# hahnicity/deepards

Measured on AMD Instinct MI355X. Metric: breath-sequences/sec (train step) cnn_linear nb20 seq224, higher is better.
Workload: dtype f32; 1 GPU; cnn_linear+resnet18, synthetic (B=64 per GPU, 20, 1, 224) fp32 train step (BASELINE configs[1]); backbone=resnet18, batch_per_gpu=64, global_batch=64, batch_rule=--batch 64 per rank (weak scaling: the global batch grows with the ranks), n_sub_batches=20, seq_len=224, optimizer=sgd-nesterov+clamp, parallelism=dp1, hipgraph=True

## Files before the change

deepards_amd/_lib.py:

```python
import ctypes
import os
import re
import subprocess

_HERE = os.path.dirname(os.path.abspath(__file__))
CSRC = os.path.join(_HERE, 'csrc')
LIB_PATH = os.environ.get('DA_LIB_PATH') or os.path.join(_HERE, 'libdeepards_hip.so')
HEADER = os.path.join(os.path.dirname(_HERE), 'include', 'deepards_hip.h')
SOURCES = ['conv_gemm.hip', 'conv_wino.hip', 'conv_bf16.hip', 'conv_x3p.hip', 'bn.hip', 'stem_pool.hip', 'head_optim.hip', 'transformer.hip',
           'filters.hip', 'se.hip', 'se_wide.hip', 'vgg.hip', 'gradcam.hip', 'protopnet.hip', 'lstm_seq.hip',
           'siamese.hip']

_P, _I, _F, _Z, _U, _D = ctypes.c_void_p, ctypes.c_int, ctypes.c_float, ctypes.c_size_t, ctypes.c_uint, ctypes.c_double
_IP = ctypes.POINTER(ctypes.c_int)


class BnRunningDesc(ctypes.Structure):
    _fields_ = [('mean', _P), ('invstd', _P), ('running_mean', _P), ('running_var', _P), ('num_batches_tracked', _P),
                ('W', _I), ('C', _I), ('Wn', _I), ('eps', _F), ('momentum', _F)]


class BnFwdDesc(ctypes.Structure):
    _fields_ = [('x', ctypes.c_void_p), ('ldx', ctypes.c_int), ('res', ctypes.c_void_p), ('ldr', ctypes.c_int),
                ('out', ctypes.c_void_p), ('ldo', ctypes.c_int), ('mean', ctypes.c_void_p), ('invstd', ctypes.c_void_p),
                ('gamma', ctypes.c_void_p), ('beta', ctypes.c_void_p), ('relu', ctypes.c_int), ('mask', ctypes.c_void_p)]


class BnBwdDesc(ctypes.Structure):
    _fields_ = [('x', ctypes.c_void_p), ('ldx', ctypes.c_int), ('dx', ctypes.c_void_p), ('lddx', ctypes.c_int),
                ('mean', ctypes.c_void_p), ('invstd', ctypes.c_void_p), ('gamma', ctypes.c_void_p), ('beta', ctypes.c_void_p),
                ('ds', ctypes.c_void_p)]


class BnPgradDesc(ctypes.Structure):
    _fields_ = [('s1', _P), ('s2', _P), ('dgamma', _P), ('dbeta', _P), ('W', _I), ('C', _I)]


class WgradReduceDesc(ctypes.Structure):
    _fields_ = [('slab', _P), ('dw', _P), ('splits', _I), ('ntaps', _I), ('N', _I), ('C', _I)]


class WgradJob(ctypes.Structure):
    _fields_ = [('dy', _P), ('x', _P), ('workspace', _P)] + [(n, _I) for n in
               ('rows', 'Lm', 'Ldy', 'lddy', 'N', 'Lx', 'ldx', 'C', 'dy_stride', 'dy_off', 'src_stride', 'ntaps')] + \
               [('src_off', _I * 3), ('winograd', _I), ('xform', _I), ('dy_half', _I), ('Wn', _I), ('ldstat', _I),
                ('mean', _P), ('invstd', _P), ('gamma', _P), ('beta', _P)]


class ConvJob(ctypes.Structure):
    _fields_ = [('x', _P), ('w', _P), ('y', _P)] + [(n, _I) for n in
               ('rows', 'Lm', 'Lsrc', 'ldx', 'C', 'Ldst', 'ldy', 'N', 'dst_stride', 'dst_off', 'src_stride', 'ntaps')] + \
               [('src_off', _I * 3), ('wtap', _I * 3), ('accumulate', _I), ('x2', _P), ('w2', _P), ('tap_split', _I)]


class RepackDesc(ctypes.Structure):
    _fields_ = [('W', _P), ('Wf', _P), ('Wd', _P), ('Uf', _P), ('Ud', _P), ('Co', _I), ('Ci', _I), ('K', _I),
                ('points', _I)]


SIGNATURES = {
    'da_version': (_I, []),
    'da_set_act_dtype': (_I, [_I]),
    'da_get_act_dtype': (_I, []),
    'da_abi_sizes': (None, [ctypes.POINTER(_I)]),
    'da_sizeof_wgrad_reduce_desc': (_I, []),
    'da_sizeof_bn_running_desc': (_I, []),
    'da_sizeof_bn_pgrad_desc': (_I, []),
    'da_hip_runtime_symbol': (_P, []),
    'da_conv_gemm': (_I, [_P, _P, _P] + [_I] * 12 + [_IP, _IP, _I, _P]),
    'da_conv_wgrad_workspace': (_Z, [_I] * 5),
    'da_conv_wgrad': (_I, [_P, _P, _P, _P] + [_I] * 12 + [_IP, _I, _P]),
    'da_debug_set': (_I, [_I, _I]),
    'da_repack_conv_weight': (_I, [_P, _P, _P, _I, _I, _I, _P]),
    'da_stem_conv_fwd': (_I, [_P, _P, _P, _I, _I, _I, _I, _P]),
    'da_stem_wgrad_workspace': (_Z, [_I, _I]),
    'da_stem_conv_wgrad': (_I, [_P, _I, _P, _P, _P, _I, _I, _I, _I, _P]),
    'da_stem_conv_fwd_g': (_I, [_P, _P, _P] + [_I] * 7 + [_P]),
    'da_stem_wgrad_workspace_g': (_Z, [_I] * 4),
    'da_stem_conv_wgrad_g': (_I, [_P, _I, _P, _P, _P] + [_I] * 7 + [_P]),
    'da_bn_chunks': (None, [_I, _I, _I, _IP, _IP]),
    'da_bn_workspace': (_Z, [_I, _I, _I]),
    'da_bn_stats_partial': (_I, [_P, _I, _I, _I, _I, _P, _P]),
    'da_stem_stats_partial': (_I, [_P, _P, _I, _I, _I, _I, _P, _P]),
    'da_stem_bn_relu_pool_fwd': (_I, [_P, _P, _P, _I, _I, _I, _I, _I, _P, _P, _P, _P, _I, _I, _P]),
    'da_stem_bwd_workspace': (_Z, [_I, _I]),
    'da_stem_bwd': (_I, [_P, _I, _P, _P, _I, _I, _I, _I, _P, _P, _P, _P, _I, _P, _P, _I, _P, _P]),
    'da_bn_stats_merge': (_I, [_P, _I, _I, _I, _F, _P, _P, _P]),
    'da_bn_running_multi': (_I, [ctypes.POINTER(BnRunningDesc), _I, _P]),
    'da_bn_apply': (_I, [_P, _I, _P, _I, _P, _I, _I, _I, _I, _P, _P, _P, _P, _I, _P, _F, _P]),
    'da_bn_fwd_x': (_I, [_P, _I, _P, _I, _P, _I, _I, _I, _I, _P, _P, _P, _P, _I, _F, _P, _I, _I, _P]),
    'da_bn_bwd_x': (_I, [_P, _I, _P, _I, _P, _I, _P, _I, _I, _I, _I, _P, _P, _P, _P, _I, _P, _P, _I, _P]),
    'da_bn_relu_pool_fwd_x': (_I, [_P, _I, _P, _I, _I, _I, _I, _P, _P, _P, _P, _I, _P]),
    'da_bn_fwd': (_I, [_P, _I, _P, _I, _P, _I, _I, _I, _I, _P, _P, _P, _P, _I, _F, _P, _P]),
    'da_bn_debug_two_stage': (_I, [_I]),
    'da_bn_debug_target_blocks': (_I, [_I]),
    'da_bn_bwd': (_I, [_P, _I, _P, _I, _P, _I, _P, _I, _P, _I, _I, _I, _I, _P, _P, _P, _P, _I, _P, _P, _P, _P, _I, _P]),
    'da_bn_mask_words': (_Z, [_I, _I, _I]),
    'da_bn_fwd_mask': (_I, [_P, _I, _P, _I, _P, _I, _I, _I, _I, _P, _P, _P, _P, _F, _P, _P, _P]),
    'da_bn_bwd_mask': (_I, [_P, _I, _P, _I, _P, _I, _P, _I, _I, _I, _I, _P, _P, _P, _P, _P, _P, _P, _P, _I, _P, _P]),
    'da_bn_pool_ok': (_I, [_I, _I, _I, _I]),
    'da_bn_fwd_pool': (_I, [_P, _I, _P, _I, _P, _I, _I, _I, _I, _P, _P, _P, _P, _F, _P, _P]),
    'da_bn_bwd_pool': (_I, [_P, _I, _P, _I, _P, _I, _P, _I, _I, _I, _I, _I, _P, _P, _P, _P, _P, _P, _P]),
    'da_bn_bwd_add': (_I, [_P, _I, _P, _I, _P, _I, _P, _I, _P, _I, _I, _I, _I, _P, _P, _P, _P, _I, _P, _P, _P, _P, _I, _P, _I, _P]),
    'da_bn_param_grad_multi': (_I, [ctypes.POINTER(BnPgradDesc), _I, _I, _P]),
    'da_bn_fwd_pair': (_I, [ctypes.POINTER(BnFwdDesc), _I, _I, _I, _F, _P]),
    'da_bn_bwd_pair': (_I, [_P, _I, ctypes.POINTER(BnBwdDesc), _I, _I, _I, _P, _P]),
    'da_bn_bwd_pair2': (_I, [_P, _I, _P, _I, ctypes.POINTER(BnBwdDesc), _I, _I, _I, _P, _P]),
    'da_bn_two_ok': (_I, [_I, _I, _I]),
    'da_bn_bwd_mask2': (_I, [_P, _I, _P, _I, _P, _I, _P, _I, _P, _I, _I, _I, _I, _P, _P, _P, _P, _P, _P, _P]),
    'da_bn_stats_fused': (_I, [_P, _I, _I, _I, _I, _P, _P, _I, _F, _P]),
    'da_bn_relu_ss': (_I, [_P, _I, _P, _I, _I, _I, _I, _P, _P, _I, _P, _P, _P]),
    'da_bn_bwd_ss': (_I, [_P, _I, _P, _I, _P, _I, _P, _I, _P, _I, _I, _I, _I, _P, _P, _I, _P, _P, _I, _I, _P, _U, _F, _I, _P, _P, _I, _P]),
    'da_conv1x1_bn': (_I, [_P, _I, _P, _P, _I, _I, _I, _I, _I, _I, _I, _P, _P, _I, _P, _P, _P, _I, ctypes.c_long, _I, _F, _P, _P]),
    'da_conv3_winograd_drop': (_I, [_P, _P, _P, _I, _I, _I, _I, _I, _I, _P, _U, _F, _P, _I, _P]),
    'da_stat_records_floats': (_Z, [ctypes.c_long, _I]),
    'da_conv3_winograd_bn': (_I, [_P, _P, _P, _I, _I, _I, _I, _I, _I, _P, _P, _P, _P, _P, _F, _P, _U, _F, _P, _P]),
    'da_conv_wgrad_splits': (_I, [_I] * 5),
    'da_conv_wgrad_padded_n': (_I, [_I, _I]),
    'da_conv_gemm_multi': (_I, [ctypes.POINTER(ConvJob), _I, _P]),
    'da_conv3_winograd': (_I, [_P, _P, _P, _I, _I, _I, _I, _I, _I, _I, _P]),
    'da_conv3_winograd4': (_I, [_P, _P, _P, _I, _I, _I, _I, _I, _I, _I, _P]),
    'da_conv3_bf16': (_I, [_P, _P, _P, _I, _I, _I, _I, _I, _I, _I, _P]),
    'da_conv3_bf16_bn': (_I, [_P, _P, _P, _I, _I, _I, _I, _I, _I, _I, _P, _P, _P, _P, _P, _F, _P, _P]),
    'da_pack_conv3_bf16': (_I, [_P, _P, _P, _I, _I, _P]),
    'da_conv3_x3p': (_I, [_P, _P, _P] + [_I] * 6 + [_P]),
    'da_conv_x3p_s2_fwd': (_I, [_P] * 5 + [_I] * 4 + [_P]),
    'da_conv_x3p_s2_dgrad': (_I, [_P] * 5 + [_I] * 4 + [_P]),
    'da_x3_split': (_I, [_P, _I, _P, _Z, _I, _P]),
    'da_x3_merge': (_I, [_P, _P, _I, _Z, _I, _P]),
    'da_conv_bf16_multi': (_I, [ctypes.POINTER(ConvJob), _I, _P]),
    'da_wino_debug_tail': (_I, [_I]),
    'da_wino_weights': (_I, [_P, _P, _I, _I, _I, _P]),
    'da_wino4_weights': (_I, [_P, _P, _I, _I, _I, _P]),
    'da_conv_wgrad_multi': (_I, [ctypes.POINTER(WgradJob), _I, _P]),
    'da_conv_wgrad_multi_reduce': (_I, [ctypes.POINTER(WgradJob), _I, ctypes.POINTER(ctypes.c_void_p), _I, _IP, _P]),
    'da_conv_wgrad_plan': (_I, [ctypes.POINTER(WgradJob), _I, _I, _IP]),
    'da_wgrad_reduce_multi': (_I, [ctypes.POINTER(WgradReduceDesc), _I, _I, _P]),
    'da_step_tail_multi': (_I, [ctypes.POINTER(WgradReduceDesc), _I, ctypes.POINTER(BnPgradDesc), _I, ctypes.POINTER(BnRunningDesc), _I, _P, _I, _I, _P, _I, _P]),
    'da_stem_bwd_partials': (_I, [_I, _I, _I, ctypes.POINTER(ctypes.c_size_t), ctypes.POINTER(_I)]),
    'da_stem_wgrad_reduce': (_I, [_P, _I, _I, _P, _I, _P]),
    'da_repack_multi': (_I, [ctypes.POINTER(RepackDesc), _I, _P]),
    'da_bn_relu_pool_fwd': (_I, [_P, _I, _P, _I, _I, _I, _I, _I, _P, _P, _P, _P, _I, _P]),
    'da_pool_bwd': (_I, [_P, _I, _P, _I, _P, _I, _I, _I, _I, _I, _P, _P, _P, _P, _I, _P]),
    'da_avgpool_fwd': (_I, [_P, _I, _P, _I, _I, _I, _I, _I, _P]),
    'da_avgpool_bwd': (_I, [_P, _I, _P, _I, _I, _I, _I, _I, _P]),
    'da_avgpool_slide_fwd': (_I, [_P, _I, _P, _I, _I, _I, _I, _P]),
    'da_avgpool_slide_bwd': (_I, [_P, _P, _I, _I, _I, _I, _I, _P]),
    'da_global_avgpool_fwd': (_I, [_P, _I, _P, _I, _I, _I, _P]),
    'da_global_avgpool_bwd': (_I, [_P, _P, _I, _I, _I, _I, _P]),
    'da_linear2_fwd': (_I, [_P, _P, _P, _P, _I, _I, _P]),
    'da_bce_logits': (_I, [_P, _P, _I, _F, _P, _P, _P]),
    'da_confidence_loss': (_I, [_P, _P, _I, _I, _F, _F, _P, _P, _P]),
    'da_vacillating_loss': (_I, [_P, _P, _I, _I, _F, _F, _P, _P, _P]),
    'da_linear2_bwd': (_I, [_P, _P, _P, _P, _P, _P, _I, _I, _I, _P]),
    'da_head_groups': (_I, [_I, _I]),
    'da_head_fwd': (_I, [_P, _I, _P, _P, _P, _P, _P, _P, _P, _I, _I, _I, _I, _I, _P]),
    'da_head_bwd': (_I, [_P, _P, _P, _P, _P, _P, _I, _P, _P, _P, _P, _P, _P, _I, _I, _I, _I, _F, _I, _P]),
    'da_head_flat_fwd': (_I, [_P, _P, _P, _P, _P, _P, _P, _P, _I, _I, _I, _I, _P]),
    'da_head_flat_bwd': (_I, [_P, _P, _P, _P, _P, _P, _P, _P, _P, _P, _P, _P, _I, _I, _I, _F, _I, _P]),
    'da_clamp_sgd_nesterov': (_I, [_P, _P, _P, _Z, _F, _F, _F, _F, _F, _I, _P]),
    'da_clamp_adam': (_I, [_P, _P, _P, _P, _Z, _F, _D, _D, _F, _I, _F, _F, _P]),
    'da_clamp_adam_dev': (_I, [_P, _P, _P, _P, _Z, _F, _D, _D, _F, _P, _F, _F, _P]),
    'da_gather_normalize': (_I, [_P, _P, ctypes.c_double, ctypes.c_double, _P, _I, _I, _P]),
    'da_gather_normalize_ch': (_I, [_P, _P, ctypes.POINTER(ctypes.c_double), ctypes.POINTER(ctypes.c_double), _P, _I, _I, _I, _I, _P]),
    'da_gather_normalize_filter': (_I, [_P, _P, ctypes.POINTER(ctypes.c_double), ctypes.POINTER(ctypes.c_double), _P, _P, _P, _I, _I, _I, _I, _P]),
    'da_gather_normalize_chain': (_I, [_P, _P, ctypes.POINTER(ctypes.c_double), ctypes.POINTER(ctypes.c_double), _I, _P, _P, _I, _P, _P,
                                       _I, _I, _I, _I, _P]),
    'da_window_median_fwd': (_I, [_P, _I, _I, _I, _I, _P, _P, _P]),
    'da_window_median_bwd': (_I, [_P, _P, _I, _I, _I, _P, _I, _P]),
    'da_lstm_fwd': (_I, [_P] * 11 + [_I, _I, _I, _P]),
    'da_lstm_bwd': (_I, [_P] * 9 + [_I, _I, _I, _P]),
    'da_lstm_seq_block_seqs': (_I, [_I]),
    'da_lstm_seq_fwd': (_I, [_P] * 5 + [_I] + [_P] * 3 + [_I, _I, _I, _P]),
    'da_lstm_seq_bwd_workspace': (_Z, [_I, _I]),
    'da_lstm_seq_bwd': (_I, [_P] * 14 + [_I] * 4 + [_P]),
    'da_lstm_seq_proj_fwd': (_I, [_P] * 4 + [_I] * 3 + [_P]),
    'da_lstm_seq_proj_bwd_workspace': (_Z, [_I] * 3),
    'da_lstm_seq_proj_bwd': (_I, [_P] * 7 + [_I] * 4 + [_P]),
    'da_tfm_block_form': (_I, [_I, _I, _I, _IP, _IP, ctypes.POINTER(_Z), ctypes.POINTER(_Z)]),
    'da_tfm_block_fwd': (_I, [_P] * 9 + [_I] * 4 + [_P, _U, _U, _F, _P]),
    'da_tfm_block_bwd': (_I, [_P] * 17 + [_I] * 4 + [_P, _U, _U, _F, _P]),
    'da_tfm_block_pgrad': (_I, [_P] * 13 + [_I] * 5 + [_P, _U, _U, _F, _P]),
    'da_reduce_rows': (_I, [_P, _I, _I, _P, _I, _P]),
    'da_se_gate_fwd': (_I, [_P] + [_I] * 5 + [_P] * 12),
    'da_se_scale_fwd': (_I, [_P] * 4 + [_I] * 4 + [_P] * 6),
    'da_se_bwd_reduce': (_I, [_P] * 5 + [_I] * 4 + [_P] * 5),
    'da_se_gate_bwd_workspace': (_Z, [_I] * 3),
    'da_se_gate_bwd': (_I, [_P] * 11 + [_I, _P, _I, _I, _I, _P]),
    'da_se_bwd_scale': (_I, [_P] * 4 + [_I] * 3 + [_P]),
    'da_se_wide_shape_ok': (_I, [_I, _I]),
    'da_se_wide_stats': (_I, [_P] + [_I] * 4 + [_F] + [_P] * 5),
    'da_se_wide_gate_fwd': (_I, [_P] + [_I] * 5 + [_P] * 12),
    'da_se_wide_scale_fwd': (_I, [_P] * 4 + [_I] * 4 + [_P] * 6),
    'da_se_wide_bwd_reduce': (_I, [_P] * 5 + [_I] * 4 + [_P] * 5),
    'da_se_wide_chunk_rows': (_I, []),
    'da_se_wide_gate_bwd_workspace': (_Z, [_I] * 3),
    'da_se_wide_gate_bwd': (_I, [_P] * 11 + [_I, _P, _I, _I, _I, _P]),
    'da_se_wide_bwd_scale': (_I, [_P] * 4 + [_I] * 3 + [_P]),
    'da_bn_relu_maxpool2_fwd': (_I, [_P, _I, _P] + [_I] * 4 + [_P] * 5),
    'da_bn_relu_maxpool2_bwd_workspace': (_Z, [_I] * 4),
    'da_bn_relu_maxpool2_bwd': (_I, [_P, _P, _I, _P, _P, _P] + [_I] * 4 + [_P] * 5),
    'da_bn_mean_bias': (_I, [_P, _P, _P, _I, _I, _P, _P]),
    'da_adaptive_avgpool_flat_fwd': (_I, [_P, _P] + [_I] * 4 + [_P]),
    'da_adaptive_avgpool_flat_bwd': (_I, [_P, _P] + [_I] * 4 + [_P]),
    'da_gather_rows': (_I, [_P, _P, _P, _I, _I, _P]),
    'da_gradcam_shape_ok': (_I, [_I] * 3),
    'da_gradcam_workspace': (_Z, [_I] * 3),
    'da_gradcam': (_I, [_P] * 4 + [_I] * 4 + [_P] * 12),
    'da_bias_act_fwd': (_I, [_P, _P, _P, _I, _I, _I, _P]),
    'da_bias_act_bwd_workspace': (_Z, [_I, _I]),
    'da_bias_act_bwd': (_I, [_P, _P, _P, _P, _I, _P, _I, _I, _I, _P]),
    'da_proto_shape_ok': (_I, [_I] * 4),
    'da_proto_row_tile': (_I, [_I, _I]),
    'da_proto_fwd': (_I, [_P] * 6 + [_I] * 4 + [_P]),
    'da_proto_bwd_workspace': (_Z, [_I] * 3),
    'da_proto_bwd': (_I, [_P] * 8 + [_I, _P] + [_I] * 4 + [_P]),
    'da_ppnet_loss': (_I, [_P] * 3 + [_I] * 3 + [_F] * 4 + [_P] * 4),
    'da_grad_add_decay': (_I, [_P, _P, _Z, _F, _P]),
    'da_vote_counts': (_I, [_P, _P, _I, _I, _P, _P, _P]),
    'da_concat2': (_I, [_P, _I, _I, _P, _I, _I, _P, _I, _Z, _P]),
    'da_slice_copy': (_I, [_P, _I, _I, _P, _I, _I, _Z, _I, _P]),
    'da_dropout': (_I, [_P, _P, _Z, _P, _U, _F, _P]),
    'da_concat2_dropout': (_I, [_P, _I, _I, _P, _I, _I, _P, _I, _Z, _P, _U, _F, _P]),
    'da_slice_dropout': (_I, [_P, _I, _I, _P, _I, _I, _Z, _P, _U, _F, _P]),
    'da_siamese_draw': (_I, [_P] * 4 + [_I, _I, _U, _U, _I, _P]),
    'da_siamese_head_rows_per_block': (_I, []),
    'da_siamese_head_fwd': (_I, [_P] * 4 + [_I] + [_P] * 7 + [_I] * 3 + [_P]),
    'da_siamese_head_bwd_workspace': (_Z, [_I] * 3),
    'da_siamese_head_bwd': (_I, [_P] * 4 + [_I] + [_P] * 8 + [_I] + [_P] * 5 + [_F] + [_I] * 4 + [_P]),
}


def header_symbols():
    txt = open(HEADER).read()
    txt = re.sub(r'/\*.*?\*/', '', txt, flags=re.S)
    return sorted(set(re.findall(r'\b(da_[a-z0-9_]+)\s*\(', txt)))


def build(force=False, verbose=False):
    srcs = [os.path.join(CSRC, s) for s in SOURCES]
    deps = srcs + [os.path.join(CSRC, h) for h in ('common.h', 'se_tail.h')]
    if not force and os.path.exists(LIB_PATH) and all(os.path.getmtime(LIB_PATH) >= os.path.getmtime(d) for d in deps):
        return LIB_PATH
    hipcc = os.environ.get('HIPCC', '/opt/rocm/bin/hipcc')
    if not os.path.exists(hipcc):
        hipcc = 'hipcc'
    cmd = [hipcc, '-O3', '--offload-arch=gfx950', '-fPIC', '-shared', '-std=c++17', '-o', LIB_PATH] + srcs
    if verbose:
        print(' '.join(cmd))
    subprocess.check_call(cmd)
    return LIB_PATH


_lib = None


def lib():
    global _lib
    if _lib is None:
        if not os.path.exists(LIB_PATH):
            raise RuntimeError('libdeepards_hip.so is not built: run `python -c "import __graft_entry__ as g; '
                               'g.build()"` (hipcc --offload-arch=gfx950).  There is no CPU fallback.')
        import torch
        l = ctypes.CDLL(LIB_PATH)
        for name, (res, args) in SIGNATURES.items():
            fn = getattr(l, name)
            fn.restype = res
            fn.argtypes = args
        _check_same_runtime(l)
        _lib = l
    return _lib


def _check_same_runtime(l):
    import sys
    torch = sys.modules.get('torch')
    if torch is None:
        return
    tlib = os.path.join(os.path.dirname(torch.__file__), 'lib', 'libamdhip64.so')
    if not os.path.exists(tlib):
        return
    theirs = ctypes.cast(ctypes.CDLL(tlib).hipGetLastError, ctypes.c_void_p).value
    ours = l.da_hip_runtime_symbol()
    if ours != theirs:
        raise RuntimeError('libdeepards_hip.so is bound to a different HIP runtime (%#x) than PyTorch (%#x): '
                           'import torch before deepards_amd' % (ours or 0, theirs or 0))
```

deepards_amd/csrc/common.h:

```cpp
#pragma once
#include <hip/hip_runtime.h>
#include <stdint.h>

typedef float f32x4 __attribute__((ext_vector_type(4)));
typedef float f32x16 __attribute__((ext_vector_type(16)));

typedef float f32x2v __attribute__((ext_vector_type(2)));
typedef __bf16 bf16x2v __attribute__((ext_vector_type(2)));

#define DA_OK 0
#define DA_EINVAL (-1)

__device__ __forceinline__ int xcd_chunked(int id, int total) {
  const int q = total >> 3, r = total & 7;
  const int xcd = id & 7, s = id >> 3;
  return (xcd < r ? xcd * (q + 1) : r * (q + 1) + (xcd - r) * q) + s;
}

__device__ __forceinline__ uint32_t mix32(uint32_t a, uint32_t b) {
  uint32_t h = a * 0x9E3779B1u ^ (b + 0x7F4A7C15u);
  h ^= h >> 16; h *= 0x85EBCA6Bu;
  h ^= h >> 13; h *= 0xC2B2AE35u;
  h ^= h >> 16;
  return h;
// ... 277 lines not shown
  const float* mean;
  const float* invstd;
  const float* gamma;
  const float* beta;
} da_wgrad_job;

struct WgradReduceDesc {
  const float* slab;
  float* dw;
  int splits, ntaps, N, C;
};

__device__ __forceinline__ void wgrad_reduce_block(const WgradReduceDesc& d, int blk, int accumulate) {
  const int total = d.ntaps * d.N * d.C;
  const int i = blk * 1024 + threadIdx.x * 4;
  if (i >= total) return;
  const float* p = d.slab + i;
  f32x4 s = {0.f, 0.f, 0.f, 0.f};
  int sp = 0;
  for (; sp + 8 <= d.splits; sp += 8) {
    f32x4 v[8];
#pragma unroll
    for (int j = 0; j < 8; ++j) v[j] = *reinterpret_cast<const f32x4*>(p + (size_t)(sp + j) * total);
#pragma unroll
    for (int e = 0; e < 4; ++e) s[e] += ((v[0][e] + v[1][e]) + (v[2][e] + v[3][e])) + ((v[4][e] + v[5][e]) + (v[6][e] + v[7][e]));
  }
  if (sp + 4 <= d.splits) {
    f32x4 v[4];
#pragma unroll
    for (int j = 0; j < 4; ++j) v[j] = *reinterpret_cast<const f32x4*>(p + (size_t)(sp + j) * total);
#pragma unroll
    for (int e = 0; e < 4; ++e) s[e] += (v[0][e] + v[1][e]) + (v[2][e] + v[3][e]);
    sp += 4;
  }
  for (; sp < d.splits; ++sp) {
    const f32x4 v = *reinterpret_cast<const f32x4*>(p + (size_t)sp * total);
#pragma unroll
    for (int e = 0; e < 4; ++e) s[e] += v[e];
  }
  const int nc = d.N * d.C;
  const int tap = i / nc, rem = i - tap * nc;
  float* o = d.dw + (size_t)rem * d.ntaps + tap;
#pragma unroll
  for (int e = 0; e < 4; ++e) {
    float* q = o + (size_t)e * d.ntaps;
    *q = accumulate ? *q + s[e] : s[e];
  }
}

#define WGRAD_PRE_MAX 14
struct WgradPreTable {
  WgradReduceDesc d[WGRAD_PRE_MAX];
  int first_block[WGRAD_PRE_MAX + 1];
  int n, nblocks, accumulate;
  int own;
};
__device__ __forceinline__ int wgrad_pre_dispatch(const WgradPreTable& p) {
  const int bid = blockIdx.x;
  if (p.nblocks == 0) return bid;
  if (p.own < 0) {
    if (bid >= p.nblocks) return bid - p.nblocks;
  } else if (bid < p.own) {
    return bid;
  }
  const int pb = p.own < 0 ? bid : bid - p.own;
  if (pb < p.first_block[p.n]) {
    int i = 0;
    while (i + 1 < p.n && pb >= p.first_block[i + 1]) ++i;
    wgrad_reduce_block(p.d[i], pb - p.first_block[i], p.accumulate);
  }
  return -1;
}
static inline int wgrad_pre_grid(WgradPreTable& pre, int blocks, bool front = false) {
  if (pre.nblocks == 0) return blocks;
  pre.own = front ? -1 : (blocks + 7) & ~7;
  return (front ? blocks : pre.own) + pre.nblocks;
}

struct WgradChain {
  WgradPreTable pre, next;
  int pre_job[WGRAD_PRE_MAX], next_job[WGRAD_PRE_MAX];
  float* const* dws;
  int* reduced;
};
static inline void wgrad_chain_init(WgradChain* c, float* const* dws, int accumulate, int* reduced) {
  c->pre.n = c->pre.nblocks = c->pre.own = 0;
  c->pre.first_block[0] = 0;
  c->pre.accumulate = accumulate;
  c->next = c->pre;
  c->dws = dws;
  c->reduced = reduced;
}
static inline void wgrad_chain_offer(WgradChain* c, int job, const da_wgrad_job& j, int splits) {
  if (!c || !c->dws || !c->dws[job] || c->next.n >= WGRAD_PRE_MAX) return;
  WgradPreTable& t = c->next;
  t.d[t.n] = {j.workspace, c->dws[job], splits, j.ntaps, j.N, j.C};
  c->next_job[t.n] = job;
  t.first_block[t.n + 1] = t.first_block[t.n] + (j.ntaps * j.N * j.C + 1023) / 1024;
  ++t.n;
  t.nblocks = (t.first_block[t.n] + 7) & ~7;
}
static inline WgradPreTable wgrad_chain_take(WgradChain* c) {
  WgradPreTable t;
  t.n = t.nblocks = t.accumulate = t.own = 0;
  t.first_block[0] = 0;
  if (!c) return t;
  t = c->pre;
  for (int i = 0; i < t.n; ++i) c->reduced[c->pre_job[i]] = 1;
  c->pre = c->next;
  for (int i = 0; i < c->next.n; ++i) c->pre_job[i] = c->next_job[i];
  c->next.n = c->next.nblocks = 0;
  return t;
}

struct WgradPlan {
  int tn, tc;
  int splits;
  int kchunk;
};
int wgrad_plan_jobs(const da_wgrad_job* jobs, int n, int chained, WgradPlan* plan);

bool wino_wgrad_eligible(const da_wgrad_job& j);
void wino_wgrad_plan_jobs(const da_wgrad_job* jobs, int n, int chained, WgradPlan* plan);
int wino_wgrad_launch(const da_wgrad_job* jobs, const WgradPlan* plan, int n, hipStream_t stream, WgradChain* chain);
void wino4_wgrad_plan(int rows, int L, int* splits, int* qchunk);
extern int g_wino4_skip5;
int wino4_wgrad_launch(const da_wgrad_job* jobs, const WgradPlan* plan, int n, hipStream_t stream, WgradChain* chain);

bool bf16_wgrad_eligible(const da_wgrad_job& j);
void bf16_wgrad_plan(int rows, int L, int* splits, int* pchunk);
int bf16_wgrad_launch(const da_wgrad_job* jobs, const WgradPlan* plan, int n, int code, hipStream_t stream);

typedef struct {
  const float* x;
  const float* w;
  float* y;
  int rows, Lm, Lsrc, ldx, C, Ldst, ldy, N, dst_stride, dst_off, src_stride, ntaps;
  int src_off[3];
  int wtap[3];
  int accumulate;
  const float* x2;
  const float* w2;
  int tap_split;
} da_conv_job;

extern "C" int da_sizeof_wgrad_reduce_desc(void);
extern "C" int da_sizeof_bn_running_desc(void);
extern "C" int da_sizeof_bn_pgrad_desc(void);
```

deepards_amd/csrc/conv_gemm.hip:

```cpp
#include "common.h"
#include <algorithm>
#include <utility>
#include <vector>

#ifndef WGRAD_GLOAD_AT
#define WGRAD_GLOAD_AT 8
#endif
#ifndef GLOAD_AT
#define GLOAD_AT 3
#endif

struct ConvGemmArgs {
  const float* x;
  const float* w;
  const float* x2;
  const float* w2;
  int tap_split;
  float* y;
  int M, Lsrc, ldx, C;
  int Ldst, ldy, N;
  int dst_stride, dst_off, src_stride;
  int ntaps, so0, so1, so2, wt0, wt1, wt2;
  int accumulate;
  FastDiv divLm;
};

template <int TM, int TN, int WGM, int WGN>
__device__ __forceinline__ void conv_gemm_body(const ConvGemmArgs& a, const int lin, float* lds) {
  constexpr int BM = TM * WGM * 32, BN = TN * WGN * 32, PITCH = 36;
  static_assert(WGM * WGN == 4, "4 waves");
  float* As = lds;
  float* Bs = lds + BM * PITCH;

  const int tid = threadIdx.x, lane = tid & 63, wave = tid >> 6;
  const int wm = wave / WGN, wn = wave % WGN;
  const int ntn = a.N / BN;
  const int m_blk = (lin / ntn) * BM, n_blk = (lin % ntn) * BN;
  const int lr = tid >> 3, lq = tid & 7;
  const int Lm = (int)a.divLm.d;

  constexpr int AP = BM / 32, BP = BN / 32;
  int a_rowoff[AP], a_j[AP];
  bool a_ok[AP];
#pragma unroll
  for (int p = 0; p < AP; ++p) {
    int m = m_blk + lr + 32 * p;
    a_ok[p] = m < a.M;
    uint32_t row = fdiv((uint32_t)(a_ok[p] ? m : 0), a.divLm);
    int j = (a_ok[p] ? m : 0) - (int)row * Lm;
    a_rowoff[p] = (int)row * a.Lsrc;
    a_j[p] = j * a.src_stride;
  }

  const int kc = a.C >> 5;
  const int nk = a.ntaps * kc;
  f32x4 ra[AP], rb[BP];

  auto gload = [&](int it) {
    int t = it / kc;
    int c0 = (it - t * kc) << 5;
    int so = t == 0 ? a.so0 : (t == 1 ? a.so1 : a.so2);
    int wt = t == 0 ? a.wt0 : (t == 1 ? a.wt1 : a.wt2);
#pragma unroll
    for (int p = 0; p < AP; ++p) {
      int ls = a_j[p] + so;
      bool ok = a_ok[p] && ls >= 0 && ls < a.Lsrc;
      const float* src = (t < a.tap_split ? a.x : a.x2) + (size_t)(a_rowoff[p] + (ok ? ls : 0)) * a.ldx + c0 + lq * 4;
      f32x4 v = {0.f, 0.f, 0.f, 0.f};
      if (ok) v = *reinterpret_cast<const f32x4*>(src);
      ra[p] = v;
    }
    const float* wtp = (t < a.tap_split ? a.w : a.w2) + (size_t)wt * a.N * a.C;
#pragma unroll
    for (int p = 0; p < BP; ++p) {
      int n = n_blk + lr + 32 * p;
      rb[p] = *reinterpret_cast<const f32x4*>(wtp + (size_t)n * a.C + c0 + lq * 4);
    }
  };

  f32x16 acc[TM][TN];
#pragma unroll
  for (int i = 0; i < TM; ++i)
#pragma unroll
// ... 1103 lines not shown
  if (key == 3) g_use_tail = value;
  else if (key == 7) g_wgrad_any = value;
  else if (key == 11) g_wino4_skip5 = value;
  else return DA_EINVAL;
  return DA_OK;
}

int da_conv_gemm(const float* x, const float* w, float* y, int rows, int Lm, int Lsrc, int ldx, int C, int Ldst,
                 int ldy, int N, int dst_stride, int dst_off, int src_stride, int ntaps, const int* src_off,
                 const int* wtap, int accumulate, hipStream_t stream) {
  DA_ENTER();
  if (g_act_bf16) return DA_EINVAL;
  if (!x || !w || !y || rows < 0 || Lm < 1 || ntaps < 1 || ntaps > 3) return DA_EINVAL;
  da_conv_job j = {};
  j.x = x; j.w = w; j.y = y;
  j.rows = rows; j.Lm = Lm; j.Lsrc = Lsrc; j.ldx = ldx; j.C = C; j.Ldst = Ldst; j.ldy = ldy; j.N = N;
  j.dst_stride = dst_stride; j.dst_off = dst_off; j.src_stride = src_stride; j.ntaps = ntaps; j.accumulate = accumulate;
  for (int t = 0; t < ntaps; ++t) {
    j.src_off[t] = src_off[t];
    j.wtap[t] = wtap[t];
  }
  ConvGemmArgs a;
  conv_gemm_fill(a, j);
  return conv_gemm_dispatch(a, stream);
}

int da_conv_gemm_multi(const da_conv_job* jobs, int n, hipStream_t stream) {
  DA_ENTER();
  if (g_act_bf16) return DA_EINVAL;
  if (n < 1 || n > 4 || !jobs) return DA_EINVAL;
  ConvGemmArgs a[4];
  for (int i = 0; i < n; ++i) {
    const da_conv_job& j = jobs[i];
    if (!j.x || !j.w || !j.y || j.rows < 0 || j.Lm < 1 || j.ntaps < 1 || j.ntaps > 3 || j.C % 32 || j.N % 64 || j.ldx % 4)
      return DA_EINVAL;
    if ((uint64_t)j.rows * j.Lm * (uint64_t)j.Lm >= 0xffffffffull) return DA_EINVAL;
    if (j.x2 && (!j.w2 || j.tap_split < 1 || j.tap_split >= j.ntaps)) return DA_EINVAL;
    conv_gemm_fill(a[i], j);
  }
  return launch_conv_multi(a, n, stream);
}

int da_conv1x1_bn(const float* x, int ldx, const float* w, float* y, int ldy, int rows, int R, int Lin, int C, int N, int pool,
                  float* mean, float* invstd, int ldstat, const float* gamma, const float* beta, const float* pend, int pend_c0,
                  long pend_units, int pend_Wu, float eps, float* out_part, hipStream_t stream) {
  DA_ENTER();
  if (g_act_bf16) return DA_EINVAL;
  if (!x || !w || !y || !mean || !invstd || !gamma || !beta || rows < 0 || R < 1 || rows % R || Lin < 1) return DA_EINVAL;
  if (C % 32 || C < 32 || C > 2048 || N % 64 || N < 64 || ldx % 4 || ldx < C || ldy < N || ldstat % 4 || ldstat < C) return DA_EINVAL;
  if (pool && (Lin & 1)) return DA_EINVAL;
  if (rows == 0) return DA_OK;
  const int Lout = pool ? Lin / 2 : Lin;
  const long M = (long)rows * Lout;
  if ((long)R * Lout < 64) return DA_EINVAL;
  if ((uint64_t)rows * Lin * (uint64_t)(ldx > ldy ? ldx : ldy) >= 0x7fffffffull) return DA_EINVAL;
  if ((uint64_t)M * (uint64_t)(R * Lout) >= 0xffffffffull) return DA_EINVAL;
  Conv1x1BnArgs a;
  a.x = x; a.w = w; a.y = y;
  a.M = (int)M; a.ldx = ldx; a.C = C; a.ldy = ldy; a.N = N; a.W = rows / R; a.Wn = R * Lout; a.ldstat = ldstat;
  a.mean = mean; a.invstd = invstd; a.gamma = gamma; a.beta = beta;
  a.divWn = make_fastdiv((uint32_t)a.Wn);
  a.pend = pend; a.pend_c0 = C; a.pend_nc = 0; a.pend_Wu = 1; a.pend_tiles = 0; a.eps = eps; a.out_part = out_part;
  if (pend) {
    if (pend_c0 < 0 || pend_c0 >= C || pend_units < 1 || pend_Wu < 64 || pend_units % pend_Wu || pend_units / pend_Wu != rows / R)
      return DA_EINVAL;
    a.pend_c0 = pend_c0; a.pend_nc = C - pend_c0; a.pend_Wu = pend_Wu; a.pend_tiles = (int)((pend_units + 63) / 64);
  }
  const unsigned blocks = (unsigned)(((M + 63) / 64) * (N / 64));
  const size_t shm = (size_t)(128 * 36 + 4 * C) * sizeof(float);
  if (out_part) {
    if (pool) hipLaunchKernelGGL((conv1x1_bn_kernel<1, 1>), dim3(blocks), dim3(256), shm, stream, a);
    else hipLaunchKernelGGL((conv1x1_bn_kernel<0, 1>), dim3(blocks), dim3(256), shm, stream, a);
  } else if (pool) hipLaunchKernelGGL((conv1x1_bn_kernel<1, 0>), dim3(blocks), dim3(256), shm, stream, a);
  else hipLaunchKernelGGL((conv1x1_bn_kernel<0, 0>), dim3(blocks), dim3(256), shm, stream, a);
  DA_CHECK_LAUNCH();
  return DA_OK;
}

size_t da_conv_wgrad_workspace(int rows, int Lm, int N, int C, int ntaps) {
  WgradPlan p = wgrad_plan(rows * Lm, N, C, ntaps);
  return (size_t)p.splits * ntaps * N * C * sizeof(float);
}

static int conv_wgrad_multi_impl(const da_wgrad_job* jobs, int n, int chained, float* const* dws, int accumulate, int* reduced,
                                 hipStream_t stream) {
  DA_ENTER();
  std::vector<WgradPlan> plan_(n > 0 ? n : 0);
  WgradPlan* const plan = plan_.data();
  int rc = wgrad_plan_jobs(jobs, n, chained, plan);
  if (rc) return rc;
  for (int i = 0; i < n; ++i)
    if (!jobs[i].workspace) return DA_EINVAL;
  WgradChain chain_, *chain = nullptr;
  if (dws) {
    if (!reduced) return DA_EINVAL;
    for (int i = 0; i < n; ++i) reduced[i] = 0;
    wgrad_chain_init(&chain_, dws, accumulate, reduced);
    chain = &chain_;
  }
  if ((rc = wino4_wgrad_launch(jobs, plan, n, stream, chain))) return rc;
  if ((rc = wino_wgrad_launch(jobs, plan, n, stream, chain))) return rc;
  if ((rc = bf16_wgrad_launch(jobs, plan, n, 49, stream))) return rc;
  if ((rc = bf16_wgrad_launch(jobs, plan, n, 16, stream))) return rc;
  if ((rc = launch_wgrad_group<2, 2, 2, 2>(jobs, plan, n, 128, 128, stream, chain))) return rc;
  if ((rc = launch_wgrad_group<2, 1, 2, 2>(jobs, plan, n, 128, 64, stream, chain))) return rc;
  if ((rc = launch_wgrad_group<1, 2, 2, 2>(jobs, plan, n, 64, 128, stream, chain))) return rc;
  if ((rc = launch_wgrad_group<1, 1, 2, 2>(jobs, plan, n, 64, 64, stream, chain))) return rc;
  if ((rc = launch_wgrad_group<1, 1, 4, 1>(jobs, plan, n, 128, 32, stream, chain))) return rc;
  if ((rc = launch_wgrad_group<1, 1, 1, 4>(jobs, plan, n, 32, 128, stream, chain))) return rc;
  if ((rc = launch_wgrad_group<2, 2, 2, 2, 1>(jobs, plan, n, 128, 128, stream, chain))) return rc;
  if (g_wgrad_any) return launch_wgrad_any<1>(jobs, plan, n, stream, chain);
  if ((rc = launch_wgrad_group<2, 1, 2, 2, 1>(jobs, plan, n, 128, 64, stream, chain))) return rc;
  if ((rc = launch_wgrad_group<1, 2, 2, 2, 1>(jobs, plan, n, 64, 128, stream, chain))) return rc;
  if ((rc = launch_wgrad_group<1, 1, 2, 2, 1>(jobs, plan, n, 64, 64, stream, chain))) return rc;
  if ((rc = launch_wgrad_group<1, 1, 4, 1, 1>(jobs, plan, n, 128, 32, stream, chain))) return rc;
  return launch_wgrad_group<1, 1, 1, 4, 1>(jobs, plan, n, 32, 128, stream, chain);
}

int da_conv_wgrad_multi(const da_wgrad_job* jobs, int n, hipStream_t stream) {
  return conv_wgrad_multi_impl(jobs, n, 0, nullptr, 0, nullptr, stream);
}

int da_conv_wgrad_multi_reduce(const da_wgrad_job* jobs, int n, float* const* dws, int accumulate, int* reduced,
                               hipStream_t stream) {
  if (n && (!dws || !reduced)) return DA_EINVAL;
  return conv_wgrad_multi_impl(jobs, n, 1, dws, accumulate, reduced, stream);
}

int da_conv_wgrad_plan(const da_wgrad_job* jobs, int n, int chained, int* slabs) {
  if (n > 0 && !slabs) return DA_EINVAL;
  std::vector<WgradPlan> plan(n > 0 ? n : 0);
  const int rc = wgrad_plan_jobs(jobs, n, chained, plan.data());
  for (int i = 0; !rc && i < n; ++i) slabs[i] = plan[i].splits;
  return rc;
}

int da_conv_wgrad_padded_n(int N, int C) {
  if (N < 32 || N % 32 || C < 32 || C % 32) return -1;
  for (int n = N; n < N + 128; n += 32)
    if (wgrad_plan(128, n, C, 1).tn) return n;
  return -1;
}

int da_conv_wgrad_splits(int rows, int Lm, int N, int C, int ntaps) {
  return wgrad_plan(rows * Lm, N, C, ntaps).splits;
}

typedef struct {
  const float* slab;
  float* dw;
  int splits, ntaps, N, C;
} da_wgrad_reduce_desc;

int da_sizeof_wgrad_reduce_desc(void) { return (int)sizeof(da_wgrad_reduce_desc); }

typedef struct {
  const float* s1;
  const float* s2;
  float* dgamma;
  float* dbeta;
  int W, C;
} da_bn_pgrad_desc;
typedef struct {
  const float* mean;
  const float* invstd;
  float* running_mean;
  float* running_var;
  long long* num_batches_tracked;
  int W, C, Wn;
  float eps, momentum;
} da_bn_running_desc;
int da_bn_param_grad_multi(const da_bn_pgrad_desc* descs, int n, int accumulate, hipStream_t stream);
int da_bn_running_multi(const da_bn_running_desc* descs, int n, hipStream_t stream);
int da_wgrad_reduce_multi(const da_wgrad_reduce_desc* descs, int n, int accumulate, hipStream_t stream);

int da_stem_wgrad_reduce(const float* partial, int nblk, int n, float* dw, int accumulate, hipStream_t stream);
int da_step_tail_multi(const da_wgrad_reduce_desc* descs, int n, const da_bn_pgrad_desc* pg, int npg,
                       const da_bn_running_desc* run, int nrun, const float* stem_partial, int stem_nblk, int stem_n,
                       float* stem_dw, int accumulate, hipStream_t stream) {
  DA_ENTER();
  if (n < 0 || npg < 0 || nrun < 0 || (n && !descs) || (npg && !pg) || (nrun && !run)) return DA_EINVAL;
  if (stem_partial && (!stem_dw || stem_nblk < 1 || stem_n < 1)) return DA_EINVAL;
  if (n == 0 || n > 32 || npg > REDUCE_MAX_BN || nrun > REDUCE_MAX_BN || (npg + nrun == 0 && !stem_partial)) {
    int rc = nrun ? da_bn_running_multi(run, nrun, stream) : DA_OK;
    if (!rc && stem_partial) rc = da_stem_wgrad_reduce(stem_partial, stem_nblk, stem_n, stem_dw, accumulate, stream);
    if (!rc && npg) rc = da_bn_param_grad_multi(pg, npg, accumulate, stream);
    if (!rc && n) rc = da_wgrad_reduce_multi(descs, n, accumulate, stream);
    return rc;
  }
  WgradReduceTable t;
  ReducePgradTable g;
  int maxc = 0, nred = 0;
  for (int i = 0; i < n; ++i) {
    const da_wgrad_reduce_desc& s = descs[i];
    if (!s.slab || !s.dw || s.splits < 1) return DA_EINVAL;
    if (s.ntaps < 1 || s.N < 1 || s.C < 1 || (s.N * s.C) % 4) return DA_EINVAL;
    t.d[i] = {s.slab, s.dw, s.splits, s.ntaps, s.N, s.C};
    t.first_block[i] = nred;
    nred += (s.ntaps * s.N * s.C + 1023) / 1024;
  }
  t.first_block[n] = nred;
  t.n = n;
  for (int i = 0; i < npg; ++i) {
    const da_bn_pgrad_desc& s = pg[i];
    if (!s.s1 || !s.s2 || !s.dgamma || !s.dbeta) return DA_EINVAL;
    g.p[i] = {s.s1, s.s2, s.dgamma, s.dbeta, s.W, s.C};
    if (s.C > maxc) maxc = s.C;
  }
  for (int i = 0; i < nrun; ++i) {
// ... 80 lines not shown
```

deepards_amd/csrc/conv_wino.hip:

```cpp
#include "common.h"
#include <type_traits>

struct WinoArgs {
  const float* x;
  const float* u;
  float* y;
  int MP, L, PL, ldx, C, ldy, N, accumulate;
  FastDiv divPL;
  const long long* drop_seed;
  uint32_t drop_salt;
  float drop_p;
  float* stat_part;
  int stat_Wu;
  const float* in_pend;
  float* in_mean;
  float* in_invstd;
  const float* in_gamma;
  const float* in_beta;
  int in_tiles, in_Wu;
  float in_eps;
};

__device__ __forceinline__ int wino_row(int i) {
  return (i >= 4 && i < 12) ? 2 * (i - 4) : (i < 4 ? 2 * i + 1 : 2 * (i - 12) + 9);
}

#define WINO_PITCH 36
#define WINO_AROWS 66
#define WINO_LDS_FLOATS (2 * WINO_AROWS * WINO_PITCH + 4 * 32 * WINO_PITCH)

#define WINO_STAT_FLOATS (4 * 2 * 2 * 32 + 8)
#define WINO_XF_FLOATS (2 * 2 * 128)
template <bool MINI, bool STATS = false, bool XFW = false, bool DROP = false>
__device__ __forceinline__ void conv3_wino_body(const WinoArgs& a, const int tile, const int sub, float* lds) {
  constexpr int PITCH = WINO_PITCH, PAIRS = MINI ? 32 : 64, AR = PAIRS + 2;
  float* Es = lds;
  float* Os = lds + AR * PITCH;
  float* Us = lds + 2 * AR * PITCH;

  const int tid = threadIdx.x, lane = tid & 63, wave = tid >> 6;
  const int ntn = a.N >> 5;
  const int P0 = (tile / ntn) * 64 + (MINI ? 32 * sub : 0), n_blk = (tile % ntn) * 32;
  const int lr = tid >> 3, lq = tid & 7;
  const int PL = a.PL;

  constexpr int NA = MINI ? 3 : 5;
  int aoff[NA], aslot[NA];
  bool aok[NA];
#pragma unroll
  for (int p = 0; p < NA; ++p) {
    const bool extra = p == NA - 1;
    const int e = extra ? PAIRS + (tid >> 4) : (MINI ? lr : lr + 32 * (p & 1));
    const int odd = extra ? ((tid >> 3) & 1) : (MINI ? p : (p >> 1));
    const int P = P0 - 1 + e;
    aslot[p] = 0;
    bool ok = P >= 0 && P < a.MP && (!extra || tid < 32);
    const uint32_t r = fdiv((uint32_t)(ok ? P : 0), a.divPL);
    const int i = (ok ? P : 0) - (int)r * PL;
    const int pos = 2 * i + odd;
    ok = ok && pos < a.L;
    aoff[p] = ((int)r * a.L + (ok ? pos : 0)) * a.ldx + lq * 4;
    aok[p] = ok;
    if (XFW) {
      const int sl = (P >= 0 ? P : 0) / a.stat_Wu - P0 / a.stat_Wu;
      aslot[p] = (sl < 0 ? 0 : (sl > 1 ? 1 : sl)) * 2 * a.C + lq * 4;
    }
  }
  const float* ub = a.u + (size_t)(n_blk + lr) * a.C + lq * 4;
  const size_t ustride = (size_t)a.N * a.C;
  float* xtab = lds + WINO_LDS_FLOATS + WINO_STAT_FLOATS;

  f32x4 ra[NA], rb[4];
  auto gload_a = [&](int ks) {
    const int c0 = ks << 5;
#pragma unroll
    for (int p = 0; p < NA; ++p) {
      f32x4 v = {0.f, 0.f, 0.f, 0.f};
      if (aok[p]) v = *reinterpret_cast<const f32x4*>(a.x + aoff[p] + c0);
      ra[p] = v;
    }
  };
  auto gload_b = [&](int ks) {
    const int c0 = ks << 5;
// ... 846 lines not shown
      ry[2 * rb] = okk ? *reinterpret_cast<const f32x4*>(a.dy + pos * a.lddy + n_blk + lq * 4) : z;
      ry[2 * rb + 1] = (okk && ok1) ? *reinterpret_cast<const f32x4*>(a.dy + (pos + 1) * a.lddy + n_blk + lq * 4) : z;
      rx[2 * rb] = ok ? *reinterpret_cast<const f32x4*>(a.x + pos * a.ldx + c_blk + lq * 4) : z;
      rx[2 * rb + 1] = ok1 ? *reinterpret_cast<const f32x4*>(a.x + (pos + 1) * a.ldx + c_blk + lq * 4) : z;
    }
    if (tid < 32) {
      const int P = tid < 16 ? k0 - 1 : k0 + KP;
      const bool ok = P >= 0 && P < a.MP;
      const uint32_t r = fdiv((uint32_t)(ok ? P : 0), a.divPL);
      const int i = (ok ? P : 0) - (int)r * PL;
      const int pp = 2 * i + (tid < 16 ? 1 : 0);
      f32x4 v = {0.f, 0.f, 0.f, 0.f};
      if (ok && pp < a.L) v = *reinterpret_cast<const f32x4*>(a.x + ((size_t)r * a.L + pp) * a.ldx + c_blk + lq * 4);
      rx[2 * NRB] = v;
    }
  };

  f32x16 acc[4];
#pragma unroll
  for (int j = 0; j < 4; ++j)
#pragma unroll
    for (int r = 0; r < 16; ++r) acc[j][r] = 0.f;

  const int frow = lane & 31, fh = lane >> 5;
  if (k_beg < k_end) gload(k_beg);
  for (int k0 = k_beg; k0 < k_end; k0 += KP) {
    __syncthreads();
#pragma unroll
    for (int rb = 0; rb < NRB; ++rb) {
      const int row = lrow + 16 * rb;
      *reinterpret_cast<f32x4*>(&YE[row * 64 + lq * 4]) = ry[2 * rb];
      *reinterpret_cast<f32x4*>(&YO[row * 64 + lq * 4]) = ry[2 * rb + 1];
      *reinterpret_cast<f32x4*>(&XE[(row + 1) * 64 + lq * 4]) = rx[2 * rb];
      *reinterpret_cast<f32x4*>(&XO[(row + 1) * 64 + lq * 4]) = rx[2 * rb + 1];
    }
    if (tid < 16) *reinterpret_cast<f32x4*>(&XO[lq * 4]) = rx[2 * NRB];
    else if (tid < 32) *reinterpret_cast<f32x4*>(&XE[(KP + 1) * 64 + lq * 4]) = rx[2 * NRB];
    const int Pm = k0 + (lane & 31);
    const int im = Pm - (int)fdiv((uint32_t)(Pm < a.MP ? Pm : 0), a.divPL) * PL;
    const uint32_t fmask = (uint32_t)__ballot(Pm < a.MP && im == 0);
    const uint32_t lmask = (uint32_t)__ballot(Pm < a.MP && im == PL - 1);
    __syncthreads();
#pragma unroll WW_UNROLL
    for (int kk = 0; kk < KP / 2; ++kk) {
      if (kk == KP / 4) {
        __builtin_amdgcn_sched_barrier(0);
        if (k0 + KP < k_end) gload(k0 + KP);
        __builtin_amdgcn_sched_barrier(0);
      }
      const int p = 2 * kk + fh;
      const float y0 = YE[p * 64 + wm * 32 + frow], y1 = YO[p * 64 + wm * 32 + frow];
      float d0 = XO[p * 64 + wn * 32 + frow];
      const float d1 = XE[(p + 1) * 64 + wn * 32 + frow], d2 = XO[(p + 1) * 64 + wn * 32 + frow];
      float d3 = XE[(p + 2) * 64 + wn * 32 + frow];
      if ((fmask >> p) & 1) d0 = 0.f;
      if ((lmask >> p) & 1) d3 = 0.f;
      acc[0] = __builtin_amdgcn_mfma_f32_32x32x2f32(y0, d0 - d2, acc[0], 0, 0, 0);
      acc[1] = __builtin_amdgcn_mfma_f32_32x32x2f32(y0 + y1, d1 + d2, acc[1], 0, 0, 0);
      acc[2] = __builtin_amdgcn_mfma_f32_32x32x2f32(y0 - y1, d2 - d1, acc[2], 0, 0, 0);
      acc[3] = __builtin_amdgcn_mfma_f32_32x32x2f32(y1, d1 - d3, acc[3], 0, 0, 0);
    }
  }

  float* out = a.slab + (size_t)split * 3 * a.N * a.C;
  const size_t plane = (size_t)a.N * a.C;
#pragma unroll
  for (int r = 0; r < 16; ++r) {
    const int n = n_blk + wm * 32 + (r & 3) + 8 * (r >> 2) + 4 * fh;
    const int c = c_blk + wn * 32 + frow;
    const float h = 0.5f * (acc[1][r] + acc[2][r]);
    float* o = out + (size_t)n * a.C + c;
    o[0] = acc[0][r] + h;
    o[plane] = 0.5f * (acc[1][r] - acc[2][r]);
    o[2 * plane] = h - acc[3][r];
  }
}

struct WinoWgradTable {
  WinoWgradArgs d[24];
  int first_block[25];
  int n;
  int skip5;
};
static_assert(sizeof(WinoWgradTable) + sizeof(WgradPreTable) <= 4096, "kernel arguments: 4 KB");

__global__ __launch_bounds__(256, WW_MIN_WAVES) void wino_wgrad_multi_kernel(WinoWgradTable t, WgradPreTable pre) {
  __shared__ float lds[WW_LDS_FLOATS];
  const int b = wgrad_pre_dispatch(pre);
  if (b < 0 || b >= t.first_block[t.n]) return;
  int i = 0;
  while (i + 1 < t.n && b >= t.first_block[i + 1]) ++i;
  wino_wgrad_body(t.d[i], b - t.first_block[i], t.first_block[i + 1] - t.first_block[i], lds);
}

bool wino_wgrad_eligible(const da_wgrad_job& j) {
  return j.ntaps == 3 && j.dy_stride == 1 && j.dy_off == 0 && j.src_stride == 1 && j.src_off[0] == -1 &&
         j.src_off[1] == 0 && j.src_off[2] == 1 && j.Lm == j.Ldy && j.Lm == j.Lx && j.N % 64 == 0 && j.C % 64 == 0 &&
         j.N >= 64 && j.C >= 64;
}

#ifndef WW_PCHUNK
#define WW_PCHUNK 640
#endif

static void wino_wgrad_plan(int rows, int L, int* splits, int* pchunk, int f) {
  const int MP = rows * ((L + 1) / 2);
  const int base = WW_PCHUNK / (f > 1 ? f : 1) >= 32 ? WW_PCHUNK / (f > 1 ? f : 1) : 32;
  int sp = (MP + base - 1) / base;
  if (sp < 1) sp = 1;
  int pc = ((MP + sp - 1) / sp + 31) / 32 * 32;
  if (pc < 32) pc = 32;
  *splits = (MP + pc - 1) / pc > 0 ? (MP + pc - 1) / pc : 1;
  *pchunk = pc;
}

void wino_wgrad_plan_jobs(const da_wgrad_job* jobs, int n, int chained, WgradPlan* plan) {
  constexpr int SLOTS = 1024;
  long total = 0;
  int njobs = 0;
  for (int i = 0; i < n; ++i) {
    if (jobs[i].winograd != 1) continue;
    plan[i].tn = plan[i].tc = 64;
    wino_wgrad_plan(jobs[i].rows, jobs[i].Lm, &plan[i].splits, &plan[i].kchunk, 1);
    total += (long)(jobs[i].N / 64) * (jobs[i].C / 64) * plan[i].splits;
    ++njobs;
  }
  if (!chained || njobs > 24 || total <= SLOTS || total % SLOTS == 0) return;
  const long full = total / SLOTS * SLOTS;
  long cum = 0;
  for (int i = 0; i < n; ++i) {
    if (jobs[i].winograd != 1) continue;
    cum += (long)(jobs[i].N / 64) * (jobs[i].C / 64) * plan[i].splits;
    if (cum > full) wino_wgrad_plan(jobs[i].rows, jobs[i].Lm, &plan[i].splits, &plan[i].kchunk, 2);
  }
}

int wino_wgrad_launch(const da_wgrad_job* jobs, const WgradPlan* plan, int n, hipStream_t s, WgradChain* chain) {
  WinoWgradTable t;
  int cnt = 0, blocks = 0;
  auto flush = [&]() -> int {
    if (!cnt) return DA_OK;
    t.n = cnt;
    t.skip5 = 0;
    t.first_block[cnt] = blocks;
    WgradPreTable pre = wgrad_chain_take(chain);
    hipLaunchKernelGGL(wino_wgrad_multi_kernel, dim3(wgrad_pre_grid(pre, blocks)), dim3(256), 0, s, t, pre);
    DA_CHECK_LAUNCH();
    cnt = 0;
    blocks = 0;
    return DA_OK;
  };
  for (int i = 0; i < n; ++i) {
    const da_wgrad_job& j = jobs[i];
    if (j.winograd != 1) continue;
    WinoWgradArgs& a = t.d[cnt];
    a.dy = j.dy; a.x = j.x; a.slab = j.workspace;
    a.L = j.Lm; a.PL = (j.Lm + 1) / 2; a.MP = j.rows * a.PL;
    a.lddy = j.lddy; a.N = j.N; a.ldx = j.ldx; a.C = j.C; a.pchunk = plan[i].kchunk;
    a.divPL = make_fastdiv((uint32_t)a.PL);
    t.first_block[cnt] = blocks;
    blocks += (j.N / 64) * (j.C / 64) * plan[i].splits;
    wgrad_chain_offer(chain, i, j, plan[i].splits);
    if (++cnt == 24) {
      int rc = flush();
      if (rc) return rc;
    }
  }
// ... 63 lines not shown
    }
  };

  f32x16 acc[6];
#pragma unroll
  for (int j = 0; j < 6; ++j)
#pragma unroll
    for (int r = 0; r < 16; ++r) acc[j][r] = 0.f;

  const int frow = lane & 31, fh = lane >> 5;
  if (k_beg < k_end) gload(k_beg);
  for (int k0 = k_beg; k0 < k_end; k0 += KQ) {
    __syncthreads();
#pragma unroll
    for (int rb = 0; rb < NRB; ++rb) {
      const int row = lrow + 16 * rb;
#pragma unroll
      for (int ph = 0; ph < 4; ++ph) *reinterpret_cast<f32x4*>(&Y[(ph * KQ + row) * 64 + lq * 4]) = ry[4 * rb + ph];
      *reinterpret_cast<f32x4*>(&X0[row * 64 + lq * 4]) = rx[4 * rb];
      *reinterpret_cast<f32x4*>(&X1[row * 64 + lq * 4]) = rx[4 * rb + 1];
      *reinterpret_cast<f32x4*>(&X2[row * 64 + lq * 4]) = rx[4 * rb + 2];
      *reinterpret_cast<f32x4*>(&X3[(row + 1) * 64 + lq * 4]) = rx[4 * rb + 3];
    }
    if (tid < 16) *reinterpret_cast<f32x4*>(&X3[lq * 4]) = rx[4 * NRB];
    else if (tid < 32) *reinterpret_cast<f32x4*>(&X0[KQ * 64 + lq * 4]) = rx[4 * NRB];
    const int Qm = k0 + (lane & (KQ - 1));
    const int im = Qm - (int)fdiv((uint32_t)(Qm < a.MP ? Qm : 0), a.divPL) * QL;
    const uint32_t fmask = (uint32_t)__ballot(Qm < a.MP && im == 0);
    const uint32_t lmask = (uint32_t)__ballot(Qm < a.MP && im == QL - 1);
    __syncthreads();
    constexpr int UNR = SKIP5 ? WW4_SKIP5_UNROLL : WW4_UNROLL, UNR2 = UNR / 2;
    static_assert(UNR % 2 == 0 && KQ % 8 == 0, "the K loop is unrolled in whole pairs of kk");
#pragma unroll UNR2
    for (int k2 = 0; k2 < KQ / 4; ++k2)
#pragma unroll
    for (int u = 0; u < 2; ++u) {
      const int kk = 2 * k2 + u;
      if (u == 0 && k2 == KQ / 8) {
        __builtin_amdgcn_sched_barrier(0);
        if (k0 + KQ < k_end) gload(k0 + KQ);
        __builtin_amdgcn_sched_barrier(0);
      }
      const int p = 2 * kk + fh;
      const int yo = p * 64 + wm * 32 + frow, xo = p * 64 + wn * 32 + frow;
      const float y0 = Y[yo], y1 = Y[KQ * 64 + yo], y2 = Y[2 * KQ * 64 + yo], y3 = Y[3 * KQ * 64 + yo];
      float d0 = X3[xo];
      const float d1 = X0[xo], d2 = X1[xo], d3 = X2[xo], d4 = X3[xo + 64];
      float d5 = X0[xo + 64];
      if ((fmask >> p) & 1) d0 = 0.f;
      if ((lmask >> p) & 1) d5 = 0.f;
      const float ya = y0 + y2, yb = y1 + y3, yc = fmaf(4.f, y2, y0), yd = 2.f * fmaf(4.f, y3, y1);
      const float e1 = fmaf(-4.f, d2, d4), e2 = fmaf(-4.f, d1, d3), f1 = d4 - d2, f2 = d3 - d1;
      acc[0] = __builtin_amdgcn_mfma_f32_32x32x2f32(y0, fmaf(4.f, d0, fmaf(-5.f, d2, d4)), acc[0], 0, 0, 0);
      acc[1] = __builtin_amdgcn_mfma_f32_32x32x2f32(ya + yb, e1 + e2, acc[1], 0, 0, 0);
      acc[2] = __builtin_amdgcn_mfma_f32_32x32x2f32(ya - yb, e1 - e2, acc[2], 0, 0, 0);
      acc[3] = __builtin_amdgcn_mfma_f32_32x32x2f32(yc + yd, fmaf(2.f, f2, f1), acc[3], 0, 0, 0);
      acc[4] = __builtin_amdgcn_mfma_f32_32x32x2f32(yc - yd, fmaf(-2.f, f2, f1), acc[4], 0, 0, 0);
      if (!SKIP5) {
        acc[5] = __builtin_amdgcn_mfma_f32_32x32x2f32(y3, fmaf(4.f, d1, fmaf(-5.f, d3, d5)), acc[5], 0, 0, 0);
      } else if (u == 0) {
        const int p5 = 2 * kk + 2 * fh;
        const int y5o = p5 * 64 + wm * 32 + frow, x5o = p5 * 64 + wn * 32 + frow;
        const float g3 = Y[3 * KQ * 64 + y5o];
        const float g1 = X0[x5o], g2 = X2[x5o], g5 = X0[x5o + 64];
        acc[5] = __builtin_amdgcn_mfma_f32_32x32x2f32(g3, fmaf(4.f, g1, fmaf(-5.f, g2, g5)), acc[5], 0, 0, 0);
      }
    }
  }

  float* out = a.slab + (size_t)split * 3 * a.N * a.C;
  const size_t plane = (size_t)a.N * a.C;
#pragma unroll
  for (int r = 0; r < 16; ++r) {
    const int n = n_blk + wm * 32 + (r & 3) + 8 * (r >> 2) + 4 * fh;
    const int c = c_blk + wn * 32 + frow;
    const float s12 = acc[1][r] + acc[2][r], s34 = acc[3][r] + acc[4][r];
    float* o = out + (size_t)n * a.C + c;
    o[0] = fmaf(0.25f, acc[0][r], fmaf(1.0f / 24.0f, s34, -(1.0f / 6.0f) * s12));
    o[plane] = fmaf(1.0f / 6.0f, acc[2][r] - acc[1][r], (1.0f / 12.0f) * (acc[3][r] - acc[4][r]));
    o[2 * plane] = fmaf(1.0f / 6.0f, s34 - s12, acc[5][r]);
  }
}

__global__ __launch_bounds__(256, WW4_MIN_WAVES) void wino4_wgrad_multi_kernel(WinoWgradTable t, WgradPreTable pre) {
  __shared__ float lds[WW4_LDS_FLOATS];
  const int b = wgrad_pre_dispatch(pre);
  if (b < 0 || b >= t.first_block[t.n]) return;
  int i = 0;
  while (i + 1 < t.n && b >= t.first_block[i + 1]) ++i;
  const bool skip5 = t.skip5 && t.d[i].PL == 2 && (t.d[i].L & 3) != 0;
  if (skip5) wino4_wgrad_body<true>(t.d[i], b - t.first_block[i], t.first_block[i + 1] - t.first_block[i], lds);
  else wino4_wgrad_body<false>(t.d[i], b - t.first_block[i], t.first_block[i + 1] - t.first_block[i], lds);
}

#ifndef WW4_QCHUNK
#define WW4_QCHUNK 320
#endif

void wino4_wgrad_plan(int rows, int L, int* splits, int* qchunk) {
  const int MQ = rows * ((L + 3) / 4);
  int sp = (MQ + WW4_QCHUNK - 1) / WW4_QCHUNK;
  if (sp < 1) sp = 1;
  int qc = ((MQ + sp - 1) / sp + WW4_KQ - 1) / WW4_KQ * WW4_KQ;
  if (qc < WW4_KQ) qc = WW4_KQ;
  *splits = (MQ + qc - 1) / qc > 0 ? (MQ + qc - 1) / qc : 1;
  *qchunk = qc;
}

int wino4_wgrad_launch(const da_wgrad_job* jobs, const WgradPlan* plan, int n, hipStream_t s, WgradChain* chain) {
  WinoWgradTable t;
  int cnt = 0, blocks = 0;
  auto flush = [&]() -> int {
    if (!cnt) return DA_OK;
    t.n = cnt;
    t.first_block[cnt] = blocks;
    WgradPreTable pre = wgrad_chain_take(chain);
    t.skip5 = g_wino4_skip5 != 0;
    hipLaunchKernelGGL(wino4_wgrad_multi_kernel, dim3(wgrad_pre_grid(pre, blocks)), dim3(256), 0, s, t, pre);
    DA_CHECK_LAUNCH();
    cnt = 0;
    blocks = 0;
    return DA_OK;
  };
  for (int i = 0; i < n; ++i) {
    const da_wgrad_job& j = jobs[i];
    if (j.winograd != 6) continue;
    WinoWgradArgs& a = t.d[cnt];
    a.dy = j.dy; a.x = j.x; a.slab = j.workspace;
    a.L = j.Lm; a.PL = (j.Lm + 3) / 4; a.MP = j.rows * a.PL;
    a.lddy = j.lddy; a.N = j.N; a.ldx = j.ldx; a.C = j.C; a.pchunk = plan[i].kchunk;
    static_assert(WW4_KQ % 8 == 0, "skip5: K steps start at even quads");
    if (a.pchunk % WW4_KQ) return DA_EINVAL;
    a.divPL = make_fastdiv((uint32_t)a.PL);
    t.first_block[cnt] = blocks;
    blocks += (j.N / 64) * (j.C / 64) * plan[i].splits;
    wgrad_chain_offer(chain, i, j, plan[i].splits);
    if (++cnt == 24) {
      int rc = flush();
      if (rc) return rc;
    }
  }
  return flush();
}

__global__ __launch_bounds__(256) void wino_weight_kernel(const float* __restrict__ w, float* __restrict__ u, int co,
                                                          int ci, int transpose) {
  const int N = transpose ? ci : co, C = transpose ? co : ci;
  const size_t total = (size_t)N * C;
  const size_t idx = (size_t)blockIdx.x * blockDim.x + threadIdx.x;
  if (idx >= total) return;
  const int n = (int)(idx / C), c = (int)(idx - (size_t)n * C);
  const float* src = transpose ? w + ((size_t)c * ci + n) * 3 : w + ((size_t)n * ci + c) * 3;
  const float g0 = transpose ? src[2] : src[0], g1 = src[1], g2 = transpose ? src[0] : src[2];
  u[idx] = g0;
  u[total + idx] = (g0 + g1 + g2) * 0.5f;
  u[2 * total + idx] = (g0 - g1 + g2) * 0.5f;
  u[3 * total + idx] = g2;
}

__global__ __launch_bounds__(256) void wino4_weight_kernel(const float* __restrict__ w, float* __restrict__ u, int co,
                                                           int ci, int transpose) {
  const int N = transpose ? ci : co, C = transpose ? co : ci;
  const size_t total = (size_t)N * C;
  const size_t idx = (size_t)blockIdx.x * blockDim.x + threadIdx.x;
  if (idx >= total) return;
  const int n = (int)(idx / C), c = (int)(idx - (size_t)n * C);
  const float* src = transpose ? w + ((size_t)c * ci + n) * 3 : w + ((size_t)n * ci + c) * 3;
  const float g0 = transpose ? src[2] : src[0], g1 = src[1], g2 = transpose ? src[0] : src[2];
  wino4_taps(g0, g1, g2, u + idx, total);
}

extern "C" {

int da_wino4_weights(const float* w, float* u, int co, int ci, int transpose, hipStream_t stream) {
  DA_ENTER();
  if (!w || !u || co < 1 || ci < 1) return DA_EINVAL;
  const size_t total = (size_t)co * ci;
  hipLaunchKernelGGL(wino4_weight_kernel, dim3((unsigned)((total + 255) / 256)), dim3(256), 0, stream, w, u, co, ci,
                     transpose);
  DA_CHECK_LAUNCH();
  return DA_OK;
}

struct WinoBnIn {
  const float* pend; float* mean; float* invstd; const float* gamma; const float* beta; float eps;
};

static int conv3_winograd_impl(const float* x, const float* u, float* y, int rows, int L, int ldx, int C, int ldy, int N,
                               int accumulate, const long long* drop_seed, unsigned drop_salt, float drop_p, float* stat_part,
                               int stat_R, hipStream_t stream, const WinoBnIn* bn = nullptr, int outs = 2) {
  DA_ENTER();
  if (g_act_bf16) return DA_EINVAL;
  if (outs == 4 && (stat_part || bn || drop_p > 0.f)) return DA_EINVAL;
  if (!x || !u || !y || rows < 0 || L < 1 || C % 32 || N % 32 || C < 32 || N < 32 || ldx % 4 || ldx < C || ldy < N)
    return DA_EINVAL;
  if (rows == 0) return DA_OK;
  if ((uint64_t)rows * L * (uint64_t)(ldx > ldy ? ldx : ldy) >= 0x7fffffffull) return DA_EINVAL;
  WinoArgs a;
  a.x = x; a.u = u; a.y = y;
  a.L = L; a.PL = (L + outs - 1) / outs; a.MP = rows * a.PL;
  a.ldx = ldx; a.C = C; a.ldy = ldy; a.N = N; a.accumulate = accumulate;
// ... 89 lines not shown
```

deepards_amd/csrc/stem_pool.hip:

```cpp
#include "common.h"

template <typename AT, int CIN, int K, int S>
__global__ __launch_bounds__(256) void stem_conv_fwd_kernel(const float* __restrict__ x, const float* __restrict__ w,
                                                            AT* __restrict__ y, int Lin, int Lout, int C0, int ldy) {
  extern __shared__ float xs[];
  constexpr int PAD = K / 2;
  const int row = blockIdx.x, LP = Lin + K - 1;
  for (int i = threadIdx.x; i < CIN * LP; i += blockDim.x) {
    const int ci = i / LP, s = i - ci * LP - PAD;
    xs[i] = (s >= 0 && s < Lin) ? x[((size_t)row * CIN + ci) * Lin + s] : 0.f;
  }
  __syncthreads();
  const int co = threadIdx.x % C0, slot = threadIdx.x / C0, nslots = blockDim.x / C0;
  if (slot >= nslots) return;
  float wk[CIN * K];
#pragma unroll
  for (int k = 0; k < CIN * K; ++k) wk[k] = w[co * CIN * K + k];
  for (int l = slot; l < Lout; l += nslots) {
    float acc = 0.f;
#pragma unroll
    for (int ci = 0; ci < CIN; ++ci)
#pragma unroll
      for (int k = 0; k < K; ++k) acc = fmaf(wk[ci * K + k], xs[ci * LP + S * l + k], acc);
    Act<AT>::st1(y + ((size_t)row * Lout + l) * ldy + co, acc);
  }
}

template <typename AT, int CIN, int K, int S>
__global__ __launch_bounds__(256) void stem_wgrad_kernel(const AT* __restrict__ dy, int lddy,
                                                         const float* __restrict__ x, float* __restrict__ partial,
                                                         int rows, int Lin, int Lout, int C0) {
  extern __shared__ float sm[];
  constexpr int PAD = K / 2, KK = CIN * K;
  const int LP = Lin + K - 1;
  float* xs = sm;
  float* red = sm + CIN * LP;
  const int co = threadIdx.x % C0, slot = threadIdx.x / C0, nslots = blockDim.x / C0;
  float acc[KK];
#pragma unroll
  for (int k = 0; k < KK; ++k) acc[k] = 0.f;
  for (int row = blockIdx.x; row < rows; row += gridDim.x) {
    __syncthreads();
    for (int i = threadIdx.x; i < CIN * LP; i += blockDim.x) {
      const int ci = i / LP, s = i - ci * LP - PAD;
      xs[i] = (s >= 0 && s < Lin) ? x[((size_t)row * CIN + ci) * Lin + s] : 0.f;
    }
    __syncthreads();
    if (slot < nslots) {
      for (int l = slot; l < Lout; l += nslots) {
        float g = Act<AT>::ld1(dy + ((size_t)row * Lout + l) * lddy + co);
#pragma unroll
        for (int ci = 0; ci < CIN; ++ci)
#pragma unroll
          for (int k = 0; k < K; ++k) acc[ci * K + k] = fmaf(g, xs[ci * LP + S * l + k], acc[ci * K + k]);
      }
    }
  }
  __syncthreads();
  if (slot < nslots) {
#pragma unroll
    for (int k = 0; k < KK; ++k) red[(slot * C0 + co) * KK + k] = acc[k];
  }
  __syncthreads();
  for (int i = threadIdx.x; i < C0 * KK; i += blockDim.x) {
    float s = 0.f;
    for (int sl = 0; sl < nslots; ++sl) s += red[sl * C0 * KK + i];
    partial[(size_t)blockIdx.x * C0 * KK + i] = s;
  }
}

__global__ __launch_bounds__(256) void stem_wgrad_reduce_kernel(const float* __restrict__ partial, int nblk, int n,
                                                                float* __restrict__ dw, int accumulate) {
  __shared__ float red[32][8];
  stem_wgrad_reduce_block(partial, nblk, n, dw, accumulate, blockIdx.x, red);
}

template <typename AT, int OX3 = 0>
__global__ __launch_bounds__(256) void bn_relu_pool_fwd_kernel(const AT* __restrict__ y, int ldy,
                                                               AT* __restrict__ out, int ldo, int rows, int R,
                                                               int Lin, int Lout, int C, const float* __restrict__ mean,
                                                               const float* __restrict__ invstd,
                                                               const float* __restrict__ gamma,
                                                               const float* __restrict__ beta, int pool_mode) {
  const int nq = C >> 2;
  size_t idx = (size_t)blockIdx.x * blockDim.x + threadIdx.x;
  size_t total = (size_t)rows * Lout * nq;
  if (idx >= total) return;
  int q = (int)(idx % nq);
  size_t po = idx / nq;
  int j = (int)(po % Lout);
  int row = (int)(po / Lout);
  int w = row / R;
  int c0 = q * 4;
  f32x4 mu = *reinterpret_cast<const f32x4*>(mean + (size_t)w * C + c0);
  f32x4 is = *reinterpret_cast<const f32x4*>(invstd + (size_t)w * C + c0);
  f32x4 ga = *reinterpret_cast<const f32x4*>(gamma + c0);
  f32x4 be = *reinterpret_cast<const f32x4*>(beta + c0);
  f32x4 o;
  if (pool_mode != 1) o = f32x4{-INFINITY, -INFINITY, -INFINITY, -INFINITY};
  else o = f32x4{0.f, 0.f, 0.f, 0.f};
  const int sh = pool_mode == 2 ? 1 : 0;
#pragma unroll
  for (int t = 0; t < 3; ++t) {
    int l = 2 * j - 1 + sh + t;
    if (l < 0 || l >= Lin) continue;
    f32x4 v = Act<AT>::ld4(y + ((size_t)row * Lin + l) * ldy + c0);
#pragma unroll
    for (int e = 0; e < 4; ++e) {
      float z = fmaxf((v[e] - mu[e]) * is[e] * ga[e] + be[e], 0.f);
      o[e] = pool_mode != 1 ? fmaxf(o[e], z) : o[e] + z;
    }
  }
  if (pool_mode == 1) {
#pragma unroll
    for (int e = 0; e < 4; ++e) o[e] *= (1.0f / 3.0f);
  }
  if constexpr (OX3) X3::st4(reinterpret_cast<__bf16*>(out) + po * (size_t)(3 * C), c0, o);
  else Act<AT>::st4(out + po * ldo + c0, o);
}

#define STEM_XPAD 8

__device__ __forceinline__ f32x4 stem_y4(const StemW4& sw, const float (&xw)[16], int o) {
  f32x4 y;
#pragma unroll
  for (int e = 0; e < 4; ++e) {
    float acc = 0.f;
#pragma unroll
    for (int k = 0; k < 7; ++k) acc = fmaf(sw.w[e][k], xw[o + k], acc);
    y[e] = acc;
  }
  return y;
}
__device__ __forceinline__ void stem_xw_fill(float (&xw)[16], const float* xs, int j) {
#pragma unroll
  for (int i = 0; i < 16; i += 4) {
    const f32x4 v = *reinterpret_cast<const f32x4*>(xs + 4 * j + i);
    xw[i] = v[0]; xw[i + 1] = v[1]; xw[i + 2] = v[2]; xw[i + 3] = v[3];
  }
}
__device__ __forceinline__ void stem_xw_next(float (&xw)[16], const float* xs, int j) {
#pragma unroll
  for (int i = 0; i < 12; ++i) xw[i] = xw[i + 4];
  const f32x4 v = *reinterpret_cast<const f32x4*>(xs + 4 * j + 12);
  xw[12] = v[0]; xw[13] = v[1]; xw[14] = v[2]; xw[15] = v[3];
}
__host__ __device__ __forceinline__ int stem_xs_floats(int Lin) { return (STEM_XPAD + Lin + 16 + 3) & ~3; }

struct StemBn4 {
  f32x4 mu, is, ga, be;
  __device__ __forceinline__ f32x4 z(const f32x4& y) const {
    f32x4 r;
#pragma unroll
    for (int e = 0; e < 4; ++e) r[e] = fmaxf((y[e] - mu[e]) * is[e] * ga[e] + be[e], 0.f);
    return r;
  }
};

template <typename AT, int OX3, int SH>
__global__ __launch_bounds__(256) void stem_bn_relu_pool_fwd_kernel(const float* __restrict__ xrows, const float* __restrict__ wt,
                                                                    AT* __restrict__ out, int ldo, int rows, int R, int Lin,
                                                                    int Lc, int Lp, int C, const float* __restrict__ mean,
                                                                    const float* __restrict__ invstd,
                                                                    const float* __restrict__ gamma,
                                                                    const float* __restrict__ beta, int pool_mode) {
  extern __shared__ __attribute__((aligned(16))) float sm[];
  const int nq = C >> 2, nruns = blockDim.x / nq, RJ = (Lp + nruns - 1) / nruns;
  const int XS = stem_xs_floats(Lin);
  float* xs = sm;
  const int q = threadIdx.x % nq, run = threadIdx.x / nq, c0 = q * 4;
  StemW4 sw;
  sw.load(wt, c0);
  StemBn4 bn;
  bn.ga = *reinterpret_cast<const f32x4*>(gamma + c0);
  bn.be = *reinterpret_cast<const f32x4*>(beta + c0);
  constexpr int sh = SH;
  const int j0 = sh + run * RJ, j1 = min(Lp + sh, j0 + RJ);
  for (int row = blockIdx.x; row < rows; row += gridDim.x) {
    const int w = row / R;
    __syncthreads();
    for (int i = threadIdx.x; i < XS; i += blockDim.x) {
      const int sx = i - STEM_XPAD - 2 * sh;
      xs[i] = (sx >= 0 && sx < Lin) ? xrows[(size_t)row * Lin + sx] : 0.f;
    }
    __syncthreads();
    if (j0 >= j1) continue;
    bn.mu = *reinterpret_cast<const f32x4*>(mean + (size_t)w * C + c0);
    bn.is = *reinterpret_cast<const f32x4*>(invstd + (size_t)w * C + c0);
    float xw[16];
    stem_xw_fill(xw, xs, j0);
    f32x4 zm = {0.f, 0.f, 0.f, 0.f};
    if (j0 > 0) zm = bn.z(stem_y4(sw, xw, 3));
    for (int j = j0; j < j1; ++j) {
      if (j > j0) stem_xw_next(xw, xs, j);
      const bool vm = j > 0, vp = 2 * j + 1 < Lc + sh;
      const f32x4 z0 = bn.z(stem_y4(sw, xw, 5)), zp = bn.z(stem_y4(sw, xw, 7));
      f32x4 o;
#pragma unroll
      for (int e = 0; e < 4; ++e) {
        if (pool_mode != 1) {
          float m = vm ? fmaxf(-INFINITY, zm[e]) : -INFINITY;
          m = fmaxf(m, z0[e]);
          o[e] = vp ? fmaxf(m, zp[e]) : m;
        } else {
          float a = vm ? 0.f + zm[e] : 0.f;
          a += z0[e];
          if (vp) a += zp[e];
          o[e] = a * (1.0f / 3.0f);
        }
      }
      const size_t po = (size_t)row * Lp + (j - sh);
      if constexpr (OX3) X3::st4(reinterpret_cast<__bf16*>(out) + po * (size_t)(3 * C), c0, o);
      else Act<AT>::st4(out + po * ldo + c0, o);
      zm = zp;
    }
  }
}

template <typename AT>
__global__ __launch_bounds__(256) void pool_bwd_kernel(const AT* __restrict__ dout, int ldd,
                                                       const AT* __restrict__ y, int ldy, AT* __restrict__ dz,
                                                       int lddz, int rows, int R, int Lin, int Lout, int C,
                                                       const float* __restrict__ mean, const float* __restrict__ invstd,
                                                       const float* __restrict__ gamma, const float* __restrict__ beta,
                                                       int pool_mode) {
  const int nq = C >> 2;
  size_t idx = (size_t)blockIdx.x * blockDim.x + threadIdx.x;
  size_t total = (size_t)rows * Lin * nq;
  if (idx >= total) return;
  int q = (int)(idx % nq);
  size_t pi = idx / nq;
  int l = (int)(pi % Lin);
  int row = (int)(pi / Lin);
  int w = row / R;
  int c0 = q * 4;
  f32x4 acc = {0.f, 0.f, 0.f, 0.f};
  const int sh = pool_mode == 2 ? 1 : 0;
  int j_lo = (l + sh) / 2 - sh;
  int j_hi = (l + sh + 1) / 2 - sh;
  if (pool_mode == 1) {
    for (int j = j_lo; j <= j_hi; ++j) {
      if (j >= Lout) continue;
      f32x4 g = Act<AT>::ld4(dout + ((size_t)row * Lout + j) * ldd + c0);
#pragma unroll
      for (int e = 0; e < 4; ++e) acc[e] += g[e] * (1.0f / 3.0f);
    }
  } else {
    f32x4 mu = *reinterpret_cast<const f32x4*>(mean + (size_t)w * C + c0);
    f32x4 is = *reinterpret_cast<const f32x4*>(invstd + (size_t)w * C + c0);
    f32x4 ga = *reinterpret_cast<const f32x4*>(gamma + c0);
    f32x4 be = *reinterpret_cast<const f32x4*>(beta + c0);
    for (int j = j_lo; j <= j_hi; ++j) {
      if (j < 0 || j >= Lout) continue;
      float best[4] = {-INFINITY, -INFINITY, -INFINITY, -INFINITY};
      int barg[4] = {-1, -1, -1, -1};
#pragma unroll
      for (int t = 0; t < 3; ++t) {
        int ll = 2 * j - 1 + sh + t;
        if (ll < 0 || ll >= Lin) continue;
        f32x4 v = Act<AT>::ld4(y + ((size_t)row * Lin + ll) * ldy + c0);
#pragma unroll
        for (int e = 0; e < 4; ++e) {
          float z = fmaxf((v[e] - mu[e]) * is[e] * ga[e] + be[e], 0.f);
          if (z > best[e]) {
            best[e] = z;
            barg[e] = ll;
          }
        }
      }
      f32x4 g = Act<AT>::ld4(dout + ((size_t)row * Lout + j) * ldd + c0);
#pragma unroll
      for (int e = 0; e < 4; ++e)
        if (barg[e] == l) acc[e] += g[e];
    }
  }
  Act<AT>::st4(dz + pi * lddz + c0, acc);
}

template <typename AT, bool APPLY, int SH>
__global__ __launch_bounds__(256) void stem_bwd_kernel(const AT* __restrict__ dout, int ldd, const float* __restrict__ xrows,
                                                       const float* __restrict__ wt, int rows, int R, int Lin, int Lc, int Lp,
                                                       int C, const float* __restrict__ mean, const float* __restrict__ invstd,
                                                       const float* __restrict__ gamma, const float* __restrict__ beta,
                                                       int pool_mode, int RPB, float* __restrict__ rowpart,
                                                       float* __restrict__ ds, float* __restrict__ partial) {
  extern __shared__ __attribute__((aligned(16))) float sm[];
  const int nq = C >> 2, slots = blockDim.x / nq, NRUN = slots < 8 ? slots : 8, RS = slots / NRUN, RJ = (Lp + NRUN - 1) / NRUN;
  const int XS = stem_xs_floats(Lin);
  float* tot = sm + RS * XS;
  float* red = tot + 2 * C;
  const int q = threadIdx.x % nq, slot = threadIdx.x / nq, rs = slot / NRUN, run = slot - rs * NRUN, c0 = q * 4;
  float* xs = sm + rs * XS;
  StemW4 sw;
  sw.load(wt, c0);
  StemBn4 bn;
  bn.ga = *reinterpret_cast<const f32x4*>(gamma + c0);
  bn.be = *reinterpret_cast<const f32x4*>(beta + c0);
  float wacc[4][7];
#pragma unroll
  for (int e = 0; e < 4; ++e)
#pragma unroll
    for (int k = 0; k < 7; ++k) wacc[e][k] = 0.f;
  const float inv_n = 1.0f / (float)(R * Lc);
  constexpr int sh = SH;
  const int jend = Lp + sh;
  const int j0 = sh + run * RJ, j1 = min(jend, j0 + RJ);
  const int row_beg = blockIdx.x * RPB, w = row_beg / R;
  if (APPLY && (int)threadIdx.x < 2 * C) {
    const int which = threadIdx.x / C, c = threadIdx.x - which * C;
    float t = 0.f;
    for (int r = 0; r < R; ++r) t += rowpart[((size_t)(w * R + r) * 2 + which) * C + c];
    tot[which * C + c] = t;
    if (ds && row_beg == w * R) ds[((size_t)which * (rows / R) + w) * C + c] = t;
  }
  bn.mu = *reinterpret_cast<const f32x4*>(mean + (size_t)w * C + c0);
  bn.is = *reinterpret_cast<const f32x4*>(invstd + (size_t)w * C + c0);
  f32x4 t1n = {0.f, 0.f, 0.f, 0.f}, t2n = t1n;
  for (int rb = row_beg; rb < row_beg + RPB; rb += RS) {
    const int row = rb + rs;
    __syncthreads();
    for (int i = threadIdx.x; i < RS * XS; i += blockDim.x) {
      const int r = i / XS, sx = i - r * XS - STEM_XPAD - 2 * sh;
      sm[i] = (sx >= 0 && sx < Lin) ? xrows[(size_t)(rb + r) * Lin + sx] : 0.f;
    }
    __syncthreads();
    if (APPLY && rb == row_beg) {
#pragma unroll
      for (int e = 0; e < 4; ++e) {
        t1n[e] = tot[c0 + e] * inv_n;
        t2n[e] = tot[C + c0 + e] * inv_n;
      }
    }
    const AT* drow = dout + (size_t)row * Lp * ldd + c0;
    float s1[4] = {0.f, 0.f, 0.f, 0.f}, s2[4] = {0.f, 0.f, 0.f, 0.f};
    float xw[16];
    auto finish = [&](const f32x4& gsum, const f32x4& y, int o) {
      f32x4 g, xh;
#pragma unroll
      for (int e = 0; e < 4; ++e) {
        xh[e] = (y[e] - bn.mu[e]) * bn.is[e];
        g[e] = (xh[e] * bn.ga[e] + bn.be[e] > 0.f) ? gsum[e] : 0.f;
      }
      if (!APPLY) {
#pragma unroll
        for (int e = 0; e < 4; ++e) {
          s1[e] += g[e];
          s2[e] += g[e] * xh[e];
        }
      } else {
#pragma unroll
        for (int e = 0; e < 4; ++e) {
          const float d = bn.ga[e] * bn.is[e] * (g[e] - t1n[e] - xh[e] * t2n[e]);
#pragma unroll
          for (int k = 0; k < 7; ++k) wacc[e][k] = fmaf(d, xw[o + k], wacc[e][k]);
        }
      }
    };
    auto choose = [&](const f32x4& zm, const f32x4& z0, const f32x4& zp, bool vm, bool vp, const f32x4& d, f32x4& gm, f32x4& g0,
                      f32x4& gp) {
      if (pool_mode == 1) {
#pragma unroll
        for (int e = 0; e < 4; ++e) {
          const float t = d[e] * (1.0f / 3.0f);
          gm[e] = vm ? t : 0.f; g0[e] = t; gp[e] = vp ? t : 0.f;
        }
        return;
      }
#pragma unroll
      for (int e = 0; e < 4; ++e) {
        float best = -INFINITY;
        int arg = -1;
        if (vm && zm[e] > best) { best = zm[e]; arg = 0; }
        if (z0[e] > best) { best = z0[e]; arg = 1; }
        if (vp && zp[e] > best) { best = zp[e]; arg = 2; }
        gm[e] = arg == 0 ? d[e] : 0.f;
        g0[e] = arg == 1 ? d[e] : 0.f;
        gp[e] = arg == 2 ? d[e] : 0.f;
      }
    };
    if (j0 < j1) {
      const int js = j0 > sh ? j0 - 1 : j0;
      stem_xw_fill(xw, xs, js);
      f32x4 carry = {0.f, 0.f, 0.f, 0.f}, ym = carry, zm = carry;
      if (js > 0) {
        ym = stem_y4(sw, xw, 3);
        zm = bn.z(ym);
      }
      for (int j = js; j < j1; ++j) {
        if (j > js) stem_xw_next(xw, xs, j);
        const bool vm = j > 0, vp = 2 * j + 1 < Lc + sh;
        const f32x4 y0 = stem_y4(sw, xw, 5), yp = stem_y4(sw, xw, 7);
        const f32x4 z0 = bn.z(y0), zp = bn.z(yp);
        const f32x4 d = Act<AT>::ld4(drow + (size_t)(j - sh) * ldd);
        f32x4 gm, g0, gp;
        choose(zm, z0, zp, vm, vp, d, gm, g0, gp);
        if (j >= j0) {
          if (vm) {
#pragma unroll
            for (int e = 0; e < 4; ++e) gm[e] += carry[e];
            finish(gm, ym, 3);
          }
          finish(g0, y0, 5);
          if (j == jend - 1 && vp) finish(gp, yp, 7);
        }
        carry = gp; ym = yp; zm = zp;
      }
    }
    if (!APPLY) {
      __syncthreads();
#pragma unroll
      for (int e = 0; e < 4; ++e) {
        red[(slot * 2 + 0) * C + c0 + e] = s1[e];
        red[(slot * 2 + 1) * C + c0 + e] = s2[e];
      }
      __syncthreads();
      for (int i = threadIdx.x; i < RS * 2 * C; i += blockDim.x) {
        const int r = i / (2 * C), t_ = i - r * 2 * C;
        float t = 0.f;
        for (int u = 0; u < NRUN; ++u) t += red[(r * NRUN + u) * 2 * C + t_];
        rowpart[(size_t)(rb + r) * 2 * C + t_] = t;
      }
    }
  }
  if (APPLY) {
    __syncthreads();
#pragma unroll
    for (int e = 0; e < 4; ++e)
#pragma unroll
      for (int k = 0; k < 7; ++k) red[(slot * C + c0 + e) * 7 + k] = wacc[e][k];
    __syncthreads();
    for (int i = threadIdx.x; i < C * 7; i += blockDim.x) {
      float t = 0.f;
      for (int r = 0; r < slots; ++r) t += red[r * C * 7 + i];
      partial[(size_t)blockIdx.x * C * 7 + i] = t;
    }
  }
}

template <typename IT, typename OT>
__global__ __launch_bounds__(256) void avgpool_fwd_kernel(const IT* __restrict__ x, int ldx, OT* __restrict__ out,
                                                          int ldo, int rows, int Lin, int Lout, int k, int C) {
  const int nq = C >> 2;
  size_t idx = (size_t)blockIdx.x * blockDim.x + threadIdx.x;
  size_t total = (size_t)rows * Lout * nq;
  if (idx >= total) return;
  int q = (int)(idx % nq);
  size_t po = idx / nq;
  int j = (int)(po % Lout);
  int row = (int)(po / Lout);
  f32x4 acc = {0.f, 0.f, 0.f, 0.f};
  for (int t = 0; t < k; ++t) {
    f32x4 v = Act<IT>::ld4(x + ((size_t)row * Lin + j * k + t) * ldx + q * 4);
#pragma unroll
    for (int e = 0; e < 4; ++e) acc[e] += v[e];
  }
  const float inv = 1.0f / (float)k;
#pragma unroll
  for (int e = 0; e < 4; ++e) acc[e] *= inv;
  Act<OT>::st4(out + po * ldo + q * 4, acc);
}

template <typename IT, typename OT>
__global__ __launch_bounds__(256) void avgpool_bwd_kernel(const IT* __restrict__ dout, int ldd, OT* __restrict__ dx,
                                                          int lddx, int rows, int Lin, int Lout, int k, int C) {
  const int nq = C >> 2;
  size_t idx = (size_t)blockIdx.x * blockDim.x + threadIdx.x;
  size_t total = (size_t)rows * Lin * nq;
  if (idx >= total) return;
  int q = (int)(idx % nq);
  size_t pi = idx / nq;
  int l = (int)(pi % Lin);
  int row = (int)(pi / Lin);
  int j = l / k;
  f32x4 g = {0.f, 0.f, 0.f, 0.f};
  if (j < Lout) {
    g = Act<IT>::ld4(dout + ((size_t)row * Lout + j) * ldd + q * 4);
    const float inv = 1.0f / (float)k;
#pragma unroll
    for (int e = 0; e < 4; ++e) g[e] *= inv;
  }
  Act<OT>::st4(dx + pi * lddx + q * 4, g);
}

template <typename AT>
__global__ __launch_bounds__(256) void avgpool_slide_fwd_kernel(const AT* __restrict__ x, int ldx,
                                                                float* __restrict__ feat, int rows, int Lin, int Lout,
                                                                int k, int C) {
  const int nq = C >> 2;
  size_t idx = (size_t)blockIdx.x * blockDim.x + threadIdx.x;
  size_t total = (size_t)rows * Lout * nq;
  if (idx >= total) return;
  int q = (int)(idx % nq);
  size_t po = idx / nq;
  int j = (int)(po % Lout);
  int row = (int)(po / Lout);
  f32x4 acc = {0.f, 0.f, 0.f, 0.f};
  for (int t = 0; t < k; ++t) {
    f32x4 v = Act<AT>::ld4(x + ((size_t)row * Lin + j + t) * ldx + q * 4);
#pragma unroll
    for (int e = 0; e < 4; ++e) acc[e] += v[e];
  }
  const float inv = 1.0f / (float)k;
  float* o = feat + (size_t)row * C * Lout + (size_t)(q * 4) * Lout + j;
#pragma unroll
  for (int e = 0; e < 4; ++e) o[(size_t)e * Lout] = acc[e] * inv;
}

template <typename AT>
__global__ __launch_bounds__(256) void avgpool_slide_bwd_kernel(const float* __restrict__ dfeat, AT* __restrict__ dx,
                                                                int lddx, int rows, int Lin, int Lout, int k, int C) {
  const int nq = C >> 2;
  size_t idx = (size_t)blockIdx.x * blockDim.x + threadIdx.x;
  size_t total = (size_t)rows * Lin * nq;
  if (idx >= total) return;
  int q = (int)(idx % nq);
  size_t pi = idx / nq;
  int l = (int)(pi % Lin);
  int row = (int)(pi / Lin);
  int j0 = l - k + 1 > 0 ? l - k + 1 : 0;
// ... 116 lines not shown
  if (256 % (C / 4)) return DA_EINVAL;
  const size_t shm = (size_t)stem_xs_floats(Lin) * sizeof(float);
  const int nblk = rows < 1024 ? rows : 1024;
#define DA_STEM_FWD(SH_)                                                                                                      \
  do {                                                                                                                        \
    if (out_x3)                                                                                                               \
      hipLaunchKernelGGL((stem_bn_relu_pool_fwd_kernel<float, 1, SH_>), dim3(nblk), dim3(256), shm, stream, xrows, wt,        \
                         (float*)out, ldo, rows, R, Lin, Lc, Lp, C, mean, invstd, gamma, beta, pool_mode);                     \
    else                                                                                                                      \
      DA_ACT_DISPATCH(hipLaunchKernelGGL((stem_bn_relu_pool_fwd_kernel<AT, 0, SH_>), dim3(nblk), dim3(256), shm, stream,      \
                                         xrows, wt, (AT*)out, ldo, rows, R, Lin, Lc, Lp, C, mean, invstd, gamma, beta,        \
                                         pool_mode));                                                                         \
  } while (0)
  if (pool_mode == 2) DA_STEM_FWD(1);
  else DA_STEM_FWD(0);
#undef DA_STEM_FWD
  DA_CHECK_LAUNCH();
  return DA_OK;
}

int da_stem_bwd_partials(int rows, int R, int C, size_t* offset, int* nblk) {
  if (!offset || !nblk || C % 4 || C < 4 || 256 % (C / 4) || R < 1 || rows % R) return DA_EINVAL;
  const int nruns = 256 / (C / 4), NRUN = nruns < 8 ? nruns : 8, RS = nruns / NRUN;
  if (R % RS) return DA_EINVAL;
  int RPB = RS;
  for (int d = RS; d <= 5; d += RS)
    if (R % d == 0) RPB = d;
  *offset = (size_t)rows * 2 * C;
  *nblk = rows / RPB;
  return DA_OK;
}

size_t da_stem_bwd_workspace(int rows, int C) {
  return ((size_t)rows * 2 * C + (size_t)rows * 7 * C) * sizeof(float);
}

int da_stem_wgrad_reduce(const float* partial, int nblk, int n, float* dw, int accumulate, hipStream_t stream) {
  DA_ENTER();
  if (!partial || !dw || nblk < 1 || n < 1) return DA_EINVAL;
  hipLaunchKernelGGL(stem_wgrad_reduce_kernel, dim3((n + 7) / 8), dim3(256), 0, stream, partial, nblk, n, dw, accumulate);
  DA_CHECK_LAUNCH();
  return DA_OK;
}

int da_stem_bwd(const void* dout, int ldd, const float* xrows, const float* wt, int rows, int R, int Lin, int C,
                const float* mean, const float* invstd, const float* gamma, const float* beta, int pool_mode, float* ds,
                float* dw, int accumulate, float* workspace, hipStream_t stream) {
  DA_ENTER();
  if (!dout || !xrows || !wt || !mean || !invstd || !gamma || !beta || !ds || !workspace || C % 4 || C < 4 ||
      256 % (C / 4) || 2 * C > 256 || ldd % 4 || R < 1 || rows % R || Lin < 2 || (Lin & 1) || pool_mode < 0 || pool_mode > 2)
    return DA_EINVAL;
  if (rows == 0) return DA_OK;
  const int Lc = Lin / 2, Lp = pool_out_len(Lc, pool_mode), nruns = 256 / (C / 4);
  float* rowpart = workspace;
  float* partial = workspace + (size_t)rows * 2 * C;
  const int NRUN = nruns < 8 ? nruns : 8, RS = nruns / NRUN;
  if (R % RS) return DA_EINVAL;
  int RPB = RS;
  for (int d = RS; d <= 5; d += RS)
    if (R % d == 0) RPB = d;
  const int nblk = rows / RPB;
  const size_t xsn = (size_t)RS * stem_xs_floats(Lin);
  const size_t shm1 = (xsn + 2 * C + (size_t)nruns * 2 * C) * sizeof(float);
  const size_t shm2 = (xsn + 2 * C + (size_t)nruns * 7 * C) * sizeof(float);
  if (shm2 > 64 * 1024) return DA_EINVAL;
#define DA_STEM_BWD(APPLY_, SH_, SHM_, DS_, PART_)                                                                             \
  DA_ACT_DISPATCH(hipLaunchKernelGGL((stem_bwd_kernel<AT, APPLY_, SH_>), dim3(nblk), dim3(256), SHM_, stream, (const AT*)dout, \
                                     ldd, xrows, wt, rows, R, Lin, Lc, Lp, C, mean, invstd, gamma, beta, pool_mode, RPB,       \
                                     rowpart, DS_, PART_))
  if (pool_mode == 2) DA_STEM_BWD(false, 1, shm1, (float*)nullptr, (float*)nullptr);
  else DA_STEM_BWD(false, 0, shm1, (float*)nullptr, (float*)nullptr);
  DA_CHECK_LAUNCH();
  if (pool_mode == 2) DA_STEM_BWD(true, 1, shm2, ds, partial);
  else DA_STEM_BWD(true, 0, shm2, ds, partial);
#undef DA_STEM_BWD
  DA_CHECK_LAUNCH();
  if (!dw) return DA_OK;
  const int n = C * 7;
  hipLaunchKernelGGL(stem_wgrad_reduce_kernel, dim3((n + 7) / 8), dim3(256), 0, stream, partial, nblk, n, dw, accumulate);
  DA_CHECK_LAUNCH();
  return DA_OK;
}

int da_pool_bwd(const void* dout, int ldd, const void* y, int ldy, void* dz, int lddz, int rows, int R, int Lin,
                int C, const float* mean, const float* invstd, const float* gamma, const float* beta, int pool_mode,
                hipStream_t stream) {
  DA_ENTER();
  if (!dout || !y || !dz || C % 4 || ldd % 4 || ldy % 4 || lddz % 4 || R < 1 || rows % R || pool_mode < 0 || pool_mode > 2)
    return DA_EINVAL;
  if (rows == 0) return DA_OK;
  int Lout = pool_out_len(Lin, pool_mode);
  size_t total = (size_t)rows * Lin * (C / 4);
  DA_ACT_DISPATCH(hipLaunchKernelGGL(pool_bwd_kernel<AT>, dim3(grid1d(total, 256)), dim3(256), 0, stream, (const AT*)dout, ldd,
                                     (const AT*)y, ldy, (AT*)dz, lddz, rows, R, Lin, Lout, C, mean, invstd, gamma, beta,
                                     pool_mode));
  DA_CHECK_LAUNCH();
  return DA_OK;
}

int da_avgpool_fwd(const float* x, int ldx, float* out, int ldo, int rows, int Lin, int k, int C,
                   hipStream_t stream) {
  DA_ENTER();
  if (!x || !out || C % 4 || ldx % 4 || ldo % 4 || k < 1 || k > Lin) return DA_EINVAL;
  if (rows == 0) return DA_OK;
  int Lout = Lin / k;
  size_t total = (size_t)rows * Lout * (C / 4);
  hipLaunchKernelGGL((avgpool_fwd_kernel<float, float>), dim3(grid1d(total, 256)), dim3(256), 0, stream, x, ldx, out, ldo,
                     rows, Lin, Lout, k, C);
  DA_CHECK_LAUNCH();
  return DA_OK;
}

int da_avgpool_slide_fwd(const void* x, int ldx, float* feat, int rows, int Lin, int k, int C, hipStream_t stream) {
  DA_ENTER();
  if (!x || !feat || C % 4 || ldx % 4 || k < 1 || k > Lin) return DA_EINVAL;
  if (rows == 0) return DA_OK;
  int Lout = Lin - k + 1;
  size_t total = (size_t)rows * Lout * (C / 4);
  DA_ACT_DISPATCH(hipLaunchKernelGGL(avgpool_slide_fwd_kernel<AT>, dim3(grid1d(total, 256)), dim3(256), 0, stream, (const AT*)x,
                                     ldx, feat, rows, Lin, Lout, k, C));
  DA_CHECK_LAUNCH();
  return DA_OK;
}

int da_avgpool_slide_bwd(const float* dfeat, void* dx, int lddx, int rows, int Lin, int k, int C,
                         hipStream_t stream) {
  DA_ENTER();
  if (!dfeat || !dx || C % 4 || lddx % 4 || k < 1 || k > Lin) return DA_EINVAL;
  if (rows == 0) return DA_OK;
  int Lout = Lin - k + 1;
  size_t total = (size_t)rows * Lin * (C / 4);
  DA_ACT_DISPATCH(hipLaunchKernelGGL(avgpool_slide_bwd_kernel<AT>, dim3(grid1d(total, 256)), dim3(256), 0, stream, dfeat,
                                     (AT*)dx, lddx, rows, Lin, Lout, k, C));
  DA_CHECK_LAUNCH();
  return DA_OK;
}

int da_avgpool_bwd(const float* dout, int ldd, float* dx, int lddx, int rows, int Lin, int k, int C,
                   hipStream_t stream) {
  DA_ENTER();
  if (!dout || !dx || C % 4 || ldd % 4 || lddx % 4 || k < 1 || k > Lin) return DA_EINVAL;
  if (rows == 0) return DA_OK;
  int Lout = Lin / k;
  size_t total = (size_t)rows * Lin * (C / 4);
  hipLaunchKernelGGL((avgpool_bwd_kernel<float, float>), dim3(grid1d(total, 256)), dim3(256), 0, stream, dout, ldd, dx, lddx,
                     rows, Lin, Lout, k, C);
  DA_CHECK_LAUNCH();
  return DA_OK;
}

int da_global_avgpool_fwd(const void* x, int ldx, float* feat, int rows, int L, int C, hipStream_t stream) {
  DA_ENTER();
  if (!x || !feat || C % 4 || ldx % 4 || L < 1) return DA_EINVAL;
  if (rows == 0) return DA_OK;
  size_t total = (size_t)rows * (C / 4);
  DA_ACT_DISPATCH(hipLaunchKernelGGL((avgpool_fwd_kernel<AT, float>), dim3(grid1d(total, 256)), dim3(256), 0, stream,
                                     (const AT*)x, ldx, feat, C, rows, L, 1, L, C));
  DA_CHECK_LAUNCH();
  return DA_OK;
}

int da_global_avgpool_bwd(const float* dfeat, void* dx, int lddx, int rows, int L, int C, hipStream_t stream) {
  DA_ENTER();
  if (!dfeat || !dx || C % 4 || lddx % 4 || L < 1) return DA_EINVAL;
  if (rows == 0) return DA_OK;
  size_t total = (size_t)rows * L * (C / 4);
// ... 8 lines not shown
```

deepards_amd/functional.py:

```python
import contextlib
import os

import torch
from torch.autograd import Function

from . import hip_ops as H

POOL_MAX, POOL_AVG = 0, 1
POOL_MAX_CEIL = 2


class BNState(object):
    __slots__ = ('running_mean', 'running_var', 'num_batches_tracked', 'momentum', 'eps')

    def __init__(self, bn):
        self.running_mean = bn.running_mean if bn.track_running_stats else None
        self.running_var = bn.running_var if bn.track_running_stats else None
        self.num_batches_tracked = bn.num_batches_tracked if bn.track_running_stats else None
        self.momentum = 0.1 if bn.momentum is None else bn.momentum
        self.eps = bn.eps


_STEP = {'on': False, 'pack': {}, 'running': [], 'running_early': [], 'groups': 1, 'pgrad': [], 'wgrad': [], 'wslab': [],
         'stemred': None}


@contextlib.contextmanager
def training_step(model=None):
    _STEP.update(on=True, pack={}, running=[], running_early=[], pgrad=[], wgrad=[], wslab=[], stemred=None, dout2={})
    try:
        if model is not None:
            precise = {id(c) for b in model.modules() if getattr(b, 'precise_convs', False) for c in b.children()}
            ms = [m for m in model.modules()
                  if isinstance(m, torch.nn.Conv1d) and m.kernel_size[0] <= 3 and m.in_channels % 32 == 0
                  and m.weight.is_cuda and (m.bias is None or m.kernel_size[0] == 3)]
            ws = [m.weight for m in ms]
            forms = [H.step_pack_form(*m.weight.shape, m.stride[0], m.padding[0], id(m) in precise or getattr(m, 'precise_conv', False))
                     for m in ms]
            for w, c, e in zip(ws, forms, H.repack_multi(ws, forms)):
                _STEP['pack'][(w.data_ptr(), int(c))] = e
        yield
    finally:
        _STEP.update(on=False, pack={}, running=[], running_early=[], pgrad=[], wgrad=[], wslab=[], stemred=None, dout2={})


def flush_forward(defer=False):
    if defer:
        return
    _flush_early_running()
    H.bn_running_multi(_STEP['running'])
    _STEP['running'] = []


@contextlib.contextmanager
def running_update_groups(groups):
    old = _STEP['groups']
    _STEP['groups'] = int(groups)
    try:
        yield
    finally:
        _STEP['groups'] = old


def _flush_early_running():
    for items in _STEP['running_early']:
        H.bn_running_multi(items)
    _STEP['running_early'] = []


def flush_backward():
    if _STEP.get('dout2'):
        raise RuntimeError('a two-term input gradient (BasicBlockFunction split_dx) was not picked up by the block in front')
    _launch_wgrads()
    _flush_early_running()
    dst = [dw.data_ptr() for _, dw in _STEP['wslab']] + [t.data_ptr() for _, tg, tb in _STEP['pgrad'] for t in (tg, tb)]
    if len(set(dst)) != len(dst):
        _plain_writer()
    H.step_tail_multi(_STEP['wslab'], _STEP['pgrad'], _STEP['running'], accumulate=_acc(), stem=_STEP.get('stemred'))
    _STEP['pgrad'], _STEP['wslab'], _STEP['running'], _STEP['stemred'] = [], [], [], None


def _launch_wgrads():
    jobs = _STEP['wgrad']
    if not jobs:
        return
    specs = [j[:5] + (j[6], j[7]) for j in jobs]
    if _WGRAD_CHAIN:
        if len({j[5].data_ptr() for j in jobs}) != len(jobs):
            _plain_writer()
        slabs, reduced = H.conv_wgrad_multi(specs, dws=[j[5] for j in jobs], accumulate=_acc())
    else:
        slabs, reduced = H.conv_wgrad_multi(specs), [False] * len(jobs)
    _STEP['wslab'] += [(sl, j[5]) for sl, j, r in zip(slabs, jobs, reduced) if not r]
    _STEP['wgrad'] = []


_WGRAD_CHAIN = True


_STEM_FUSED = os.environ.get('DA_STEM_FUSED', '1') != '0'
CONV_DTYPES = ('f32', 'bf16', 'f32x3p')


def set_conv_dtype(name):
    if name not in CONV_DTYPES:
        raise ValueError('conv dtype must be one of %s' % (CONV_DTYPES,))
    if name != 'bf16' and H.act_dtype() == 'bf16':
        H.set_act_dtype('f32')
    H.CONV_DTYPE = name
    H.WGRAD_BF16 = name == 'bf16'


def conv_dtype():
    return H.CONV_DTYPE


def set_storage_dtype(name):
    if name == 'bf16' and H.CONV_DTYPE != 'bf16':
        raise ValueError("bf16 storage needs conv dtype 'bf16' (set_conv_dtype('bf16') first)")
    H.set_act_dtype(name)


def storage_dtype():
    return H.act_dtype()


set_conv_dtype(os.environ.get('DA_CONV_DTYPE', 'f32'))


def _pack(w, code):
    key = (w.data_ptr(), int(code))
    e = _STEP['pack'].get(key) if _STEP['on'] else None
    if e is None:
        e = H.repack_multi([w], [code])[0]
        if _STEP['on']:
            _STEP['pack'][key] = e
    return e


def _conv_fwd(x, w, stride, pad, precise=False):
    kern = H.conv_kernel(*w.shape, stride, pad, H.is_x3(x), x.shape[1], precise)
    if kern == H.DIRECT:
        return H.conv_fwd(x, _pack(w, kern)[0], stride, pad)
    pk = _pack(w, kern)[2]
    if kern == H.BF16 and stride == 2:
        return H.conv_fwd_bf16_s2(x, pk)
    fn = H.conv3_x3p if kern == H.X3 else H.conv3_bf16 if kern == H.BF16 else H.conv3_winograd
    return fn(x, pk)


def _conv_dgrad(dy, w, stride, pad, l_in, out=None, accumulate=False, precise=False):
    kern = H.conv_kernel(*w.shape, stride, pad, H.is_x3(dy), l_in, precise)
    if kern == H.DIRECT:
        return H.conv_dgrad(dy, _pack(w, kern)[1], stride, pad, l_in, out=out, accumulate=accumulate)
    pk = _pack(w, kern)[3]
    if kern == H.BF16 and stride == 2:
        return H.conv_dgrad_bf16_s2(dy, pk, l_in, out=out, accumulate=accumulate)
    fn = H.conv3_x3p if kern == H.X3 else H.conv3_bf16 if kern == H.BF16 else H.conv3_winograd
    return fn(dy, pk, out=out, accumulate=accumulate)


def _entry_fwd(entry, x, x3, w1, wd, stride):
    if entry == H.X3:
        return H.conv_x3p_s2_fwd(x3, _pack(w1, H.X3)[2], _pack(wd, H.X3)[2])
    if entry == H.BF16:
        return H.conv_fwd_bf16_s2(x, _pack(w1, H.BF16)[2], _pack(wd, H.BF16)[2])
    return H.conv_fwd_multi([(x, _pack(w1, H.DIRECT)[0], stride, 1), (x, _pack(wd, H.DIRECT)[0], stride, 0)])


def _entry_dgrad(entry, dy1, w1, dyd, wd, stride, lin, precise=False):
    if entry == H.X3:
        return H.conv_x3p_s2_dgrad(dy1, _pack(w1, H.X3)[3], dyd, _pack(wd, H.X3)[3])
    if entry == H.DIRECT:
        return H.conv_dgrad_s2_pair(dy1, _pack(w1, H.DIRECT)[1], dyd, _pack(wd, H.DIRECT)[1], lin)
    if entry == H.BF16 and _BF16_DGRAD_PAIR:
        return H.conv_dgrad_bf16_s2_pair(dy1, _pack(w1, H.BF16)[3], dyd, _pack(wd, H.BF16)[3], lin)
    dx = _conv_dgrad(dy1, w1, stride, 1, lin, precise=precise)
    return _conv_dgrad(dyd, wd, stride, 0, lin, out=dx, accumulate=True)


# ... 48 lines not shown

def _tap(t):
    if DECISION_TAP is not None:
        DECISION_TAP.append(t)


class _Stats(object):
    __slots__ = ('mean', 'invstd', 'mask')


def _bn_apply(x, R, s, st, gamma, beta, relu, res=None, want_mask=False):
    if want_mask:
        out, s.mean, s.invstd, s.mask = H.bn_fwd(x, R, gamma, beta, relu=relu, res=res, eps=st.eps, want_mask=True)
    else:
        out, s.mean, s.invstd = H.bn_fwd(x, R, gamma, beta, relu=relu, res=res, eps=st.eps)
    _running(s.mean, s.invstd, R * x.shape[1], st)
    return out


def _running(mean, invstd, wn, st):
    if st.running_mean is None:
        return
    tail = (wn, st.running_mean, st.running_var, st.num_batches_tracked, st.momentum, st.eps)
    g, w = _STEP['groups'], mean.shape[0]
    if g > 1 and w % g == 0:
        k = w // g
        items = [(mean[i * k:(i + 1) * k], invstd[i * k:(i + 1) * k]) + tail for i in range(g)]
    else:
        items = [(mean, invstd) + tail]
    if _STEP['on']:
        early = _STEP['running_early']
        while len(early) < len(items) - 1:
            early.append([])
        for lst, item in zip(early, items[:-1]):
            lst.append(item)
        _STEP['running'].append(items[-1])
    else:
        for item in items:
            H.bn_running_multi([item])


class StemFunction(Function):

    @staticmethod
    def forward(ctx, x2d, w, gamma, beta, R, pool_mode, st, want_out3=False, out_cb=0):
        ctx.fused = _STEM_FUSED and H.stem_fused_ok(x2d, w, R)
        c0 = w.shape[0]
        buf = view = None
        if out_cb > c0:
            lc = (x2d.shape[-1] + 2 * (w.shape[2] // 2) - w.shape[2]) // 2 + 1
            buf = torch.empty((x2d.shape[0], (lc - 1) // 2 + 1, out_cb), device=x2d.device, dtype=torch.float32)
            view = buf[:, :, :c0]
        ctx.c0 = c0 if buf is not None else 0
        if ctx.fused:
            out, mean, invstd = H.stem_fused_fwd(x2d, w, R, gamma, beta, pool_mode, st.eps, out_x3=want_out3, out=view)
            y0 = w
            wn = R * (x2d.shape[-1] // 2)
        else:
            y0 = H.stem_conv_fwd(x2d, w)
            mean, invstd = H.bn_stats(y0, R, st.eps)
            out = H.bn_relu_pool_fwd(y0, R, mean, invstd, gamma, beta, pool_mode, out_x3=want_out3, out=view)
            wn = R * y0.shape[1]
        if buf is not None:
            out = buf
        _running(mean, invstd, wn, st)
        ctx.save_for_backward(x2d, y0, mean, invstd, gamma, beta)
        ctx.R, ctx.pool_mode = R, pool_mode
        ctx.gt = _tgt(w, gamma, beta)
        if want_out3:
            ctx.mark_non_differentiable(out)
            ctx.set_materialize_grads(False)
            return x3_handle(out), out
        return out

    @staticmethod
    def backward(ctx, dout, _d3=None):
        x2d, y0, mean, invstd, gamma, beta = ctx.saved_tensors
        tw, tg, tb = ctx.gt
        dout = dout.contiguous()
        if ctx.c0:
            dout = dout[:, :, :ctx.c0]
        if ctx.fused:
            if _STEM_TAIL and tw is not None and _STEP['on'] and _STEP.get('stemred') is None:
                (part, nblk, n), ds = H.stem_fused_bwd(dout, x2d, y0, ctx.R, mean, invstd, gamma, beta, ctx.pool_mode, defer=True)
                _STEP['stemred'] = (part, nblk, n, tw)
                dw = None
            else:
                if tw is not None:
                    _plain_writer()
                dw, ds = H.stem_fused_bwd(dout, x2d, y0, ctx.R, mean, invstd, gamma, beta, ctx.pool_mode, dw=tw,
                                          accumulate=tw is not None)
            dgamma, dbeta = _bn_pgrad(ds, gamma, beta, tg, tb)
            return None, None if tw is not None else dw, dgamma, dbeta, None, None, None, None, None
        dz = H.pool_bwd(dout, y0, ctx.R, mean, invstd, gamma, beta, ctx.pool_mode)
        dy0, dgamma, dbeta = _bn_bwd(dz, y0, ctx.R, mean, invstd, gamma, beta, 1, tg, tb, dx=dz)
        if tw is not None:
            _plain_writer()
        dw = H.stem_conv_wgrad(dy0, x2d, out=tw, accumulate=tw is not None)
        return None, None if tw is not None else dw, dgamma, dbeta, None, None, None, None, None


class DoubleStemFunction(Function):

    @staticmethod
    def forward(ctx, x2d, wa, g1, b1, w2, g2, b2, R, pool_mode, st1, st2, want_out3=False):
        if H.act_dtype() != 'f32':
            raise NotImplementedError('double_conv_first runs with fp32 activation storage only')
        ya = H.stem_conv_fwd(x2d, wa, stride=1)
        s1 = _Stats()
        h = _bn_apply(ya, R, s1, st1, g1, b1, False)
        wf, wd = H.repack_weight(w2, True, True)
        y2 = H.conv_fwd(h, wf, 2, 3)
        m2, i2 = H.bn_stats(y2, R, st2.eps)
        out = H.bn_relu_pool_fwd(y2, R, m2, i2, g2, b2, pool_mode, out_x3=want_out3)
        _running(m2, i2, R * y2.shape[1], st2)
        ctx.save_for_backward(x2d, ya, s1.mean, s1.invstd, g1, b1, h, wd, y2, m2, i2, g2, b2)
        ctx.R, ctx.pool_mode = R, pool_mode
        ctx.gt = _tgt(wa, g1, b1, w2, g2, b2)
        if want_out3:
            ctx.mark_non_differentiable(out)
            ctx.set_materialize_grads(False)
            return x3_handle(out), out
        return out

    @staticmethod
    def backward(ctx, dout, _d3=None):
        x2d, ya, m1, i1, g1, b1, h, wd, y2, m2, i2, g2, b2 = ctx.saved_tensors
        twa, tg1, tb1, tw2, tg2, tb2 = ctx.gt
        R = ctx.R
        if twa is not None or tw2 is not None:
            _plain_writer()
        dz = H.pool_bwd(dout.contiguous(), y2, R, m2, i2, g2, b2, ctx.pool_mode)
        dy2, dg2, db2 = _bn_bwd(dz, y2, R, m2, i2, g2, b2, 1, tg2, tb2, dx=dz)
        dw2 = H.conv_wgrad(dy2, h, 7, 2, 3, out=tw2, accumulate=tw2 is not None)
        dh = H.conv_dgrad(dy2, wd, 2, 3, h.shape[1])
        dya, dg1, db1 = _bn_bwd(dh, ya, R, m1, i1, g1, b1, 0, tg1, tb1, dx=dh)
        dwa = H.stem_conv_wgrad(dya, x2d, out=twa, accumulate=twa is not None, k=3, stride=1)
        return (None, None if twa is not None else dwa, dg1, db1, None if tw2 is not None else dw2, dg2, db2,
                None, None, None, None, None)


def _bn_bwd(dout, x, R, mean, invstd, gamma, beta, mode, tg, tb, out=None, dx=None, want_g=False, add=None, mask=None):
    dx, _, _, g, ds = H.bn_bwd(dout, x, R, mean, invstd, gamma, beta, mode, out=out, want_g=want_g, dx=dx,
                               defer_param_grads=True, add=add, mask=mask)
    res = (dx,) + _bn_pgrad(ds, gamma, beta, tg, tb)
    return res + (g,) if want_g else res


def _bn_pgrad(ds, gamma, beta, tg, tb):
    if tg is not None and tb is not None:
        if _STEP['on']:
            _STEP['pgrad'].append((ds, tg, tb))
        else:
            _plain_writer()
            H.bn_param_grad_multi([(ds, tg, tb)], accumulate=True)
        return None, None
    dg, db = torch.empty_like(gamma), torch.empty_like(beta)
    H.bn_param_grad_multi([(ds, dg, db)], accumulate=False)
    return dg, db


def _wgrad(dy, x, k, stride, pad, tw, extra=None, precise=False):
    if tw is not None and _STEP['on']:
        _STEP['wgrad'].append((dy, x, k, stride, pad, tw, extra, precise))
        return None
    if tw is not None:
        _plain_writer()
# ... 815 lines not shown
```

deepards_amd/hip_ops.py:

```python
import ctypes
import os

import torch

from . import _lib

_DEBUG_SYNC = os.environ.get('DEEPARDS_DEBUG_SYNC') == '1'


class HipError(RuntimeError):
    pass


def _stream():
    return ctypes.c_void_p(torch.cuda.current_stream().cuda_stream)


def _p(t):
    return None if t is None else ctypes.c_void_p(t.data_ptr())


def _chk(rc, name):
    if rc != 0:
        raise HipError('%s failed with code %d' % (name, rc))
# ... 459 lines not shown


DIRECT = 0
WINO2 = 4
WINO4 = 6
BF16 = 16
X3 = 49
WINOGRAD_WGRAD = os.environ.get('DA_WINOGRAD', '1') != '0'
CONV_DTYPE = 'f32'
WGRAD_BF16 = False
WINO4_WGRAD_MIN_C = 512


def _s2_entry(k, stride, pad):
    return stride == 2 and (k, pad) in ((3, 1), (1, 0))


def _mult(n, co, ci):
    return co % n == 0 and ci % n == 0


def _x3_flow():
    return CONV_DTYPE == 'f32x3p' and ACT == torch.float32


def _wino(co, ci, precise=False):
    return DIRECT if not WINOGRAD_WGRAD else WINO4 if min(co, ci) >= WINO4_WGRAD_MIN_C and not precise else WINO2


def conv_kernel_wanted(co, ci, k, stride, pad, precise=False):
    if CONV_DTYPE == 'bf16' and _mult(64, co, ci) and ((k, stride, pad) == (3, 1, 1) or _s2_entry(k, stride, pad)):
        return BF16
    if not ((k, stride, pad) == (3, 1, 1) and _mult(32, co, ci)):
        return DIRECT
    return X3 if CONV_DTYPE == 'f32x3p' and _mult(64, co, ci) else _wino(co, ci, precise)


def conv_kernel(co, ci, k, stride, pad, x3, l_in, precise=False):
    kern = conv_kernel_wanted(co, ci, k, stride, pad, precise)
    if kern == X3 and not x3:
        kern = _wino(co, ci, precise)
    if kern == BF16 and stride == 2 and l_in % 2:
        kern = DIRECT
    if kern not in (BF16, X3) and ACT == torch.bfloat16:
        raise NotImplementedError('bf16 activation storage: the conv %s stride %d pad %d has no bf16 kernel (channel counts '
                                  'must be multiples of 64, stride-2 inputs of even length)' % ((co, ci, k), stride, pad))
    return kern


def step_pack_form(co, ci, k, stride, pad, precise=False):
    if _x3_flow() and _s2_entry(k, stride, pad) and _mult(64, co, ci):
        return X3
    return conv_kernel_wanted(co, ci, k, stride, pad, precise)


def wgrad_kernel(co, ci, k, stride, pad, l, x3=False, operand_form=False, precise=False):
    fits = _mult(64, co, ci) and ((k, stride, pad) == (3, 1, 1) or (_s2_entry(k, stride, pad) and l % 2 == 0))
    if x3 and not fits:
        raise ValueError('conv_wgrad_multi: x3 operands belong to k3 s1 p1 / k3 s2 p1 / k1 s2 p0 (even length) jobs, channels % 64')
    if operand_form:
        return DIRECT
    if x3:
        return X3
    if WGRAD_BF16 and fits:
        return BF16
    return _wino(co, ci, precise) if fits and stride == 1 else DIRECT


def s2_entry_kernel(w1, wd, stride, l_in, x3):
    if wd is None or stride != 2:
        return None
    if x3:
        fits = l_in % 2 == 0 and w1[2] == 3 and tuple(wd) == (w1[0], w1[1], 1) and _mult(64, w1[0], w1[1])
        return X3 if _x3_flow() and fits else None
    if conv_kernel_wanted(*w1, 2, 1) != BF16:
        return DIRECT
    return BF16 if l_in % 2 == 0 and conv_kernel_wanted(*wd, 2, 0) == BF16 else None


def x3_block_ok(rows, l, c, R):
    return _x3_flow() and c % 64 == 0 and bn_x3_ok(rows, l, c, R)


def conv_wgrad_multi(jobs, dws=None, accumulate=True):
    if not jobs:
        return [] if dws is None else ([], [])
    L = _lib.lib()
    arr = (_lib.WgradJob * len(jobs))()
    shapes = []
    for d, job in zip(arr, jobs):
        dy, x, k, stride, pad = job[:5]
        extra = job[5] if len(job) > 5 and job[5] else {}
        both_x3 = is_x3(dy) and is_x3(x)
        if both_x3:
            if not (dy.is_cuda and dy.is_contiguous() and x.is_contiguous()):
                raise ValueError('conv_wgrad_multi: x3 operands must be contiguous CUDA tensors')
            rows, lo, co = dy.shape[0], dy.shape[1], dy.shape[2] * 16
            rows2, l, ci = x.shape[0], x.shape[1], x.shape[2] * 16
            lddy, ldx = co, ci
        elif ACT == torch.float32:
            lddy, ldx = _pv(dy, 'dy'), _pv(x, 'x')
            rows, lo, co = dy.shape
            rows2, l, ci = x.shape
        else:
            _rlc(dy, 'dy')
            _rlc(x, 'x')
            rows, lo, co = dy.shape
            rows2, l, ci = x.shape
            lddy, ldx = co, ci
        ldy_len = lo
        if extra.get('dy_half'):
            if k != 1 or stride != 1 or pad != 0 or l % 2 or lo * 2 != l:
                raise ValueError('conv_wgrad_multi: dy_half belongs to a 1x1 job whose dy has half the positions of x')
            lo = l
        if rows != rows2 or lo != conv_out_len(l, k, stride, pad) or k > 3 or ci % 32 or co % 32:
            raise ValueError('conv_wgrad_multi: unsupported shape')
        kern = wgrad_kernel(co, ci, k, stride, pad, l, both_x3, bool(extra), len(job) > 6 and bool(job[6]))
        d.dy, d.x = dy.data_ptr(), x.data_ptr()
        d.rows, d.Lm, d.Ldy, d.lddy, d.N, d.Lx, d.ldx, d.C = rows, lo, ldy_len, lddy, co, l, ldx, ci
        d.dy_stride, d.dy_off, d.src_stride, d.ntaps = 1, 0, stride, k
        d.winograd = 1 if kern == WINO2 else kern
        if extra:
            if stride != 1:
                raise ValueError('conv_wgrad_multi: the dense-block operand forms belong to stride-1 jobs')
            d.dy_half = 1 if extra.get('dy_half') else 0
            if extra.get('xform') is not None:
                mean_v, invstd_v, gamma, beta, R = extra['xform']
                if rows % R:
                    raise ValueError('conv_wgrad_multi: rows not a multiple of rows_per_window')
                d.xform, d.Wn = 1, R * l
                d.ldstat = _sv(mean_v, rows // R, ci, 'mean')
                if _sv(invstd_v, rows // R, ci, 'invstd') != d.ldstat:
                    raise ValueError('conv_wgrad_multi: mean / invstd must be slices of tables with one pitch')
                d.mean, d.invstd, d.gamma, d.beta = mean_v.data_ptr(), invstd_v.data_ptr(), _f32(gamma).data_ptr(), _f32(beta).data_ptr()
        for t in range(3):
            d.src_off[t] = t - pad if t < k else 0
        shapes.append((x.device, k, co, ci))
    slabs = (ctypes.c_int * len(jobs))()
    _chk(L.da_conv_wgrad_plan(arr, len(jobs), 0 if dws is None else 1, slabs), 'da_conv_wgrad_plan')
    outs = []
    for d, sp, (dev, k, co, ci) in zip(arr, slabs, shapes):
        ws = torch.empty((sp * k * co * ci,), device=dev, dtype=torch.float32)
        d.workspace = ws.data_ptr()
        outs.append((ws, sp, k, co, ci))
    if dws is not None:
        if len(dws) != len(jobs):
            raise ValueError('conv_wgrad_multi: one destination (or None) per job')
        ptrs = (ctypes.c_void_p * len(jobs))()
        for i, (dw, (_, _, k, co, ci)) in enumerate(zip(dws, outs)):
            if dw is not None:
                if tuple(dw.shape) != (co, ci, k) or not dw.is_contiguous():
                    raise ValueError('conv_wgrad_multi: bad dw shape')
                ptrs[i] = _f32(dw, 'dw').data_ptr()
        red = (ctypes.c_int * len(jobs))()
        _chk(L.da_conv_wgrad_multi_reduce(arr, len(jobs), ptrs, 1 if accumulate else 0, red, _stream()), 'da_conv_wgrad_multi_reduce')
        return outs, [bool(r) for r in red]
    _chk(L.da_conv_wgrad_multi(arr, len(jobs), _stream()), 'da_conv_wgrad_multi')
    return outs


def _reduce_descs(items, who):
    arr = (_lib.WgradReduceDesc * len(items))()
    for d, ((slab, splits, k, co, ci), dw) in zip(arr, items):
        if tuple(dw.shape) != (co, ci, k):
            raise ValueError('%s: bad dw shape' % who)
        d.slab, d.dw, d.splits, d.ntaps, d.N, d.C = slab.data_ptr(), dw.data_ptr(), splits, k, co, ci
    return arr


def wgrad_reduce_multi(items, accumulate=True):
    if not items:
        return
    arr = _reduce_descs(items, 'wgrad_reduce_multi')
    _chk(_lib.lib().da_wgrad_reduce_multi(arr, len(items), 1 if accumulate else 0, _stream()), 'da_wgrad_reduce_multi')


def _running_descs(items):
    arr = (_lib.BnRunningDesc * len(items))()
    for d, (mean, invstd, wn, rm, rv, nbt, mom, eps) in zip(arr, items):
        if nbt is not None and nbt.dtype != torch.int64:
            raise ValueError('num_batches_tracked must be int64')
        d.mean, d.invstd, d.running_mean, d.running_var = mean.data_ptr(), invstd.data_ptr(), rm.data_ptr(), rv.data_ptr()
        d.num_batches_tracked = None if nbt is None else nbt.data_ptr()
        d.W, d.C, d.Wn, d.eps, d.momentum = mean.shape[0], mean.shape[1], wn, eps, mom
    return arr


def step_tail_multi(items, pgrad, running, accumulate=True, stem=None):
    if not items:
        bn_running_multi(running)
        bn_param_grad_multi(pgrad, accumulate)
        if stem is not None:
            part, nblk, n, dw = stem
            _chk(_lib.lib().da_stem_wgrad_reduce(_p(part), nblk, n, _p(dw), 1 if accumulate else 0, _stream()), 'da_stem_wgrad_reduce')
        return
    arr = _reduce_descs(items, 'step_tail_multi')
    pg = (_lib.BnPgradDesc * max(1, len(pgrad)))()
    for d, (ds, dg, db) in zip(pg, pgrad):
        _, w, c = ds.shape
        d.s1, d.s2 = ds.data_ptr(), ds.data_ptr() + 4 * w * c
        d.dgamma, d.dbeta, d.W, d.C = dg.data_ptr(), db.data_ptr(), w, c
    run = _running_descs(running) if running else None
    sp, snb, sn, sdw = (None, 0, 0, None) if stem is None else (_p(stem[0]), stem[1], stem[2], _p(stem[3]))
    _chk(_lib.lib().da_step_tail_multi(arr, len(items), pg if pgrad else None, len(pgrad), run, len(running), sp, snb, sn, sdw,
                                       1 if accumulate else 0, _stream()), 'da_step_tail_multi')


def repack_multi(weights, winograd=None):
    outs, descs = [], []
    for n, w in enumerate(weights):
        _f32(w, 'w')
        co, ci, k = w.shape
        code = winograd[n] if winograd is not None else DIRECT
        wino = bool(code)
        if wino and k != 3 and not (code in (BF16, X3) and k == 1):
            raise ValueError('winograd taps need a 3-tap weight')
        pts = code if wino and code in (WINO4, BF16, X3) else WINO2
        mk = lambda *shape: torch.empty(shape, device=w.device, dtype=torch.float32)
        wf, wd = (None, None) if wino else (mk(k, co, ci), mk(k, ci, co))
        if pts == BF16:
            if co % 32 or ci % 32:
                raise ValueError('bf16 tap packs need channel counts that are multiples of 32')
            uf = torch.empty((k, co, ci), device=w.device, dtype=torch.bfloat16)
            ud = torch.empty((k, ci, co), device=w.device, dtype=torch.bfloat16)
        elif pts == X3:
            if co % 64 or ci % 64:
                raise ValueError('chunked split-bf16 packs need channel counts that are multiples of 64')
            uf = torch.empty((co // 64, ci // 16, 18, 64, 8), device=w.device, dtype=torch.bfloat16)
            ud = torch.empty((ci // 64, co // 16, 18, 64, 8), device=w.device, dtype=torch.bfloat16)
        else:
            uf, ud = (mk(pts, co, ci), mk(pts, ci, co)) if wino else (None, None)
        descs.append((w.data_ptr(), _p(wf), _p(wd), _p(uf), _p(ud), co, ci, k, pts))
        outs.append((wf, wd, uf, ud))
    if descs:
        arr = (_lib.RepackDesc * len(descs))()
        for d, v in zip(arr, descs):
            d.W, d.Wf, d.Wd, d.Uf, d.Ud, d.Co, d.Ci, d.K, d.points = v
        _chk(_lib.lib().da_repack_multi(arr, len(descs), _stream()), 'da_repack_multi')
    return outs
# ... 376 lines not shown
    lo = l // 2 if pool else l
    if tuple(w.shape) != (n, c, 1) or not w.is_contiguous() or tuple(out.shape) != (rows, lo, n) or rows % R or (pool and l % 2):
        raise ValueError('conv1x1_bn: unsupported shapes x%s w%s out%s' % (tuple(xv.shape), tuple(w.shape), tuple(out.shape)))
    ldy = _pv(out, 'out')
    ldstat = _sv(mean_v, rows // R, c, 'mean')
    if _sv(invstd_v, rows // R, c, 'invstd') != ldstat:
        raise ValueError('conv1x1_bn: bad statistics slices')
    rec, c_first, units, wu = pend if pend is not None else (None, 0, 0, 0)
    if rec is not None and rec.numel() != _lib.lib().da_stat_records_floats(units, c - c_first):
        raise ValueError('conv1x1_bn: the pending records do not have %d units of %d channels' % (units, c - c_first))
    part = stat_records(rows * lo, n, xv.device) if want_records else None
    _chk(_lib.lib().da_conv1x1_bn(_p(xv), ldx, _p(_f32(w)), _p(out), ldy, rows, R, l, c, n, 1 if pool else 0, _p(mean_v),
                                  _p(invstd_v), ldstat, _p(_f32(gamma)), _p(_f32(beta)), _p(rec), c_first, units, wu, eps,
                                  _p(part), _stream()), 'da_conv1x1_bn')
    return (out, part) if want_records else out


def bn_relu_pool_fwd(y, R, mean, invstd, gamma, beta, pool_mode, out_x3=False, out=None):
    _rlc(y, 'y')
    rows, lin, c = y.shape
    lout = pool_out_len(lin, pool_mode)
    if out is not None:
        if out_x3 or tuple(out.shape) != (rows, lout, c) or ACT != torch.float32:
            raise ValueError('bn_relu_pool_fwd: bad out')
        _chk(_lib.lib().da_bn_relu_pool_fwd(_p(y), c, _p(out), _pv(out, 'out'), rows, R, lin, c, _p(mean), _p(invstd), _p(gamma),
                                            _p(beta), pool_mode, _stream()), 'da_bn_relu_pool_fwd')
        return out
    if out_x3:
        _rlc32(y, 'y')
        out = x3_empty(rows, lout, c, y.device)
        _chk(_lib.lib().da_bn_relu_pool_fwd_x(_p(y), c, _p(out), rows, R, lin, c, _p(mean), _p(invstd), _p(gamma), _p(beta),
                                              pool_mode, _stream()), 'da_bn_relu_pool_fwd_x')
        return out
    out = torch.empty((rows, lout, c), device=y.device, dtype=ACT)
    _chk(_lib.lib().da_bn_relu_pool_fwd(_p(y), c, _p(out), c, rows, R, lin, c, _p(mean), _p(invstd), _p(gamma),
                                        _p(beta), pool_mode, _stream()), 'da_bn_relu_pool_fwd')
    return out


def stem_fused_ok(x2d, w, R):
    lin = x2d.shape[-1]
    ok = (x2d.dim() == 2 or x2d.shape[1] == 1) and tuple(w.shape[1:]) == (1, 7) and \
        lin % 2 == 0 and w.shape[0] in (32, 64, 128) and x2d.shape[0] % R == 0 and R % max(1, 128 // w.shape[0]) == 0
    if not ok or x2d.shape[0] == 0:
        return ok
    p_, chunk = ctypes.c_int(), ctypes.c_int()
    _lib.lib().da_bn_chunks(x2d.shape[0] // R, R * (lin // 2), w.shape[0], ctypes.byref(p_), ctypes.byref(chunk))
    if p_.value == 0:
        return False
    lc = lin // 2
    max_rows = (chunk.value + lc - 1) // lc + 1
    return (max_rows * (lin + 12) + 33 * 32) * 4 <= 64 * 1024


def stem_fused_fwd(x2d, w, R, gamma, beta, pool_mode, eps=1e-5, out_x3=False, out=None):
    _f32(x2d, 'x')
    _f32(w, 'w')
    x = x2d.reshape(x2d.shape[0], x2d.shape[-1])
    rows, lin = x.shape
    c = w.shape[0]
    wn = rows // R
    lc = lin // 2
    lp = pool_out_len(lc, pool_mode)
    L = _lib.lib()
    part = _bn_ws(wn, R * lc, c, x.device)
    _chk(L.da_stem_stats_partial(_p(x), _p(w), rows, R, lin, c, _p(part), _stream()), 'da_stem_stats_partial')
    mean = torch.empty((wn, c), device=x.device, dtype=torch.float32)
    invstd = torch.empty((wn, c), device=x.device, dtype=torch.float32)
    _chk(L.da_bn_stats_merge(_p(part), wn, R * lc, c, eps, _p(mean), _p(invstd), _stream()), 'da_bn_stats_merge')
    ldo = c
    if out is not None:
        if out_x3 or tuple(out.shape) != (rows, lp, c):
            raise ValueError('stem_fused_fwd: bad out')
        ldo = _pv(out, 'out')
    else:
        if out_x3 and ACT != torch.float32:
            raise ValueError('stem_fused_fwd: the x3 format needs float storage')
        out = x3_empty(rows, lp, c, x.device) if out_x3 else torch.empty((rows, lp, c), device=x.device, dtype=ACT)
    _chk(L.da_stem_bn_relu_pool_fwd(_p(x), _p(w), _p(out), ldo, rows, R, lin, c, _p(mean), _p(invstd), _p(gamma), _p(beta),
                                    pool_mode, 1 if out_x3 else 0, _stream()), 'da_stem_bn_relu_pool_fwd')
    return out, mean, invstd


def stem_fused_bwd(dout, x2d, w, R, mean, invstd, gamma, beta, pool_mode, dw=None, accumulate=False, defer=False):
    ldd = _pv(dout, 'dout') if ACT == torch.float32 else _rlc(dout, 'dout').shape[2]
    x = x2d.reshape(x2d.shape[0], x2d.shape[-1])
    rows, lin = x.shape
    c = w.shape[0]
    if dout.shape[2] != c or tuple(dout.shape[:2]) != (rows, pool_out_len(lin // 2, pool_mode)):
        raise ValueError('stem_fused_bwd: dout must be the pooled map\'s gradient with the stem\'s %d channels' % c)
    if dw is None and not defer:
        if accumulate:
            raise ValueError('accumulate needs dw')
        dw = torch.empty((c, 1, 7), device=x.device, dtype=torch.float32)
    L = _lib.lib()
    ds = torch.empty((2, rows // R, c), device=x.device, dtype=torch.float32)
    ws = torch.empty((L.da_stem_bwd_workspace(rows, c) // 4,), device=x.device, dtype=torch.float32)
    _chk(L.da_stem_bwd(_p(dout), ldd, _p(x), _p(w), rows, R, lin, c, _p(mean), _p(invstd), _p(gamma), _p(beta), pool_mode, _p(ds),
                       None if defer else _p(dw), 1 if accumulate else 0, _p(ws), _stream()), 'da_stem_bwd')
    if defer:
        off, nblk = ctypes.c_size_t(), ctypes.c_int()
        _chk(L.da_stem_bwd_partials(rows, R, c, ctypes.byref(off), ctypes.byref(nblk)), 'da_stem_bwd_partials')
        return (ws[off.value:], nblk.value, c * 7), ds
    return dw, ds


def pool_bwd(dout, y, R, mean, invstd, gamma, beta, pool_mode):
    ldd = _pv(dout, 'dout') if ACT == torch.float32 else _rlc(dout, 'dout').shape[2]
    _rlc(y, 'y')
    rows, lin, c = y.shape
    if tuple(dout.shape) != (rows, pool_out_len(lin, pool_mode), c):
        raise ValueError('pool_bwd: dout %s is not the pooled map\'s gradient of y %s' % (tuple(dout.shape), tuple(y.shape)))
    dz = torch.empty_like(y)
    _chk(_lib.lib().da_pool_bwd(_p(dout), ldd, _p(y), c, _p(dz), c, rows, R, lin, c, _p(mean), _p(invstd), _p(gamma),
                                _p(beta), pool_mode, _stream()), 'da_pool_bwd')
    return dz


def _rlc32(t, name='tensor'):
    if not (t.is_cuda and t.dtype == torch.float32 and t.dim() == 3 and t.is_contiguous()):
        raise ValueError('%s must be a contiguous float32 CUDA (rows, L, C) tensor, got %s %s %s' %
                         (name, tuple(t.shape), t.dtype, t.device))
    return t


def global_avgpool_fwd(x):
    _rlc(x, 'x')
    rows, lin, c = x.shape
    feat = torch.empty((rows, c), device=x.device, dtype=torch.float32)
    _chk(_lib.lib().da_global_avgpool_fwd(_p(x), c, _p(feat), rows, lin, c, _stream()), 'da_global_avgpool_fwd')
    return feat


def global_avgpool_bwd(dfeat, lin):
    _f32(dfeat, 'dfeat')
    rows, c = dfeat.shape
    dx = torch.empty((rows, lin, c), device=dfeat.device, dtype=ACT)
    _chk(_lib.lib().da_global_avgpool_bwd(_p(dfeat), _p(dx), c, rows, lin, c, _stream()), 'da_global_avgpool_bwd')
    return dx


def avgpool_fwd(x, k):
    _rlc32(x, 'x')
    rows, lin, c = x.shape
    out = torch.empty((rows, lin // k, c), device=x.device, dtype=torch.float32)
    _chk(_lib.lib().da_avgpool_fwd(_p(x), c, _p(out), c, rows, lin, k, c, _stream()), 'da_avgpool_fwd')
    return out


def avgpool_bwd(dout, lin, k):
    _rlc32(dout, 'dout')
    rows, lout, c = dout.shape
    dx = torch.empty((rows, lin, c), device=dout.device, dtype=torch.float32)
    _chk(_lib.lib().da_avgpool_bwd(_p(dout), c, _p(dx), c, rows, lin, k, c, _stream()), 'da_avgpool_bwd')
    return dx


def avgpool_slide_fwd(x, k):
    _rlc(x, 'x')
    rows, lin, c = x.shape
    feat = torch.empty((rows, c * (lin - k + 1)), device=x.device, dtype=torch.float32)
    _chk(_lib.lib().da_avgpool_slide_fwd(_p(x), c, _p(feat), rows, lin, k, c, _stream()), 'da_avgpool_slide_fwd')
    return feat


def avgpool_slide_bwd(dfeat, lin, k, c):
    _f32(dfeat, 'dfeat')
    rows = dfeat.shape[0]
    if dfeat.shape[1] != c * (lin - k + 1):
        raise ValueError('dfeat must be (rows, C * (L - k + 1))')
    dx = torch.empty((rows, lin, c), device=dfeat.device, dtype=ACT)
    _chk(_lib.lib().da_avgpool_slide_bwd(_p(dfeat), _p(dx), c, rows, lin, k, c, _stream()), 'da_avgpool_slide_bwd')
    return dx


def linear2_fwd(flat, w, bias):
    _f32(flat, 'flat')
    b, k = flat.shape
    if tuple(w.shape) != (2, k):
        raise ValueError('linear_final weight must be (2, %d), got %s' % (k, tuple(w.shape)))
# ... 260 lines not shown
```

include/deepards_hip.h:

```cpp
#ifndef DEEPARDS_HIP_H
#define DEEPARDS_HIP_H

#include <stddef.h>
#include <stdint.h>

#ifdef __cplusplus
extern "C" {
#endif

typedef struct ihipStream_t* da_stream_t;

int da_version(void);

typedef void da_act_t;
int da_set_act_dtype(int bf16);
int da_get_act_dtype(void);
void da_abi_sizes(int* out);
int da_sizeof_wgrad_reduce_desc(void);
int da_sizeof_bn_running_desc(void);
int da_sizeof_bn_pgrad_desc(void);
const void* da_hip_runtime_symbol(void);

int da_conv_gemm(const float* x, const float* w, float* y, int rows, int Lm, int Lsrc, int ldx, int C,
                 int Ldst, int ldy, int N, int dst_stride, int dst_off, int src_stride, int ntaps,
                 const int* src_off, const int* wtap, int accumulate, da_stream_t stream);

size_t da_conv_wgrad_workspace(int rows, int Lm, int N, int C, int ntaps);
int da_conv_wgrad(const float* dy, const float* x, float* dw, float* workspace, int rows, int Lm, int Ldy,
                  int lddy, int N, int Lx, int ldx, int C, int dy_stride, int dy_off, int src_stride, int ntaps,
                  const int* src_off, int accumulate, da_stream_t stream);

int da_debug_set(int key, int value);

typedef struct {
  const float* x; const float* w; float* y;
  int rows, Lm, Lsrc, ldx, C, Ldst, ldy, N, dst_stride, dst_off, src_stride, ntaps; int src_off[3]; int wtap[3];
  int accumulate;
  const float* x2; const float* w2; int tap_split;
} da_conv_job;
int da_conv_gemm_multi(const da_conv_job* jobs, int n, da_stream_t stream);
int da_conv3_winograd(const float* x, const float* u, float* y, int rows, int L, int ldx, int C, int ldy, int N,
                      int accumulate, da_stream_t stream);
int da_wino_debug_tail(int on);
int da_wino_weights(const float* w, float* u, int co, int ci, int transpose, da_stream_t stream);
int da_conv3_winograd4(const float* x, const float* u, float* y, int rows, int L, int ldx, int C, int ldy, int N,
                       int accumulate, da_stream_t stream);
int da_wino4_weights(const float* w, float* u, int co, int ci, int transpose, da_stream_t stream);

int da_conv3_bf16(const da_act_t* x, const void* wpk, da_act_t* y, int rows, int L, int ldx, int C, int ldy, int N,
                  int accumulate, da_stream_t stream);
int da_conv3_bf16_bn(const da_act_t* x, const void* wpk, da_act_t* y, int rows, int L, int ldx, int C, int ldy, int N, int R,
                     const float* in_pend, float* in_mean, float* in_invstd, const float* gamma, const float* beta, float eps,
                     float* stat_part, da_stream_t stream);
int da_pack_conv3_bf16(const float* w, void* wf, void* wd, int co, int ci, da_stream_t stream);
int da_conv_x3p_s2_fwd(const void* x3, const void* w1pk, const void* wdpk, float* y1, float* yd, int rows, int Lin, int C, int N,
                       da_stream_t stream);
int da_conv_x3p_s2_dgrad(const void* dy1_3, const void* w1pk, const void* dyd_3, const void* wdpk, float* dx, int rows, int Lout,
                         int N, int C, da_stream_t stream);
int da_conv3_x3p(const void* x, const void* wpk, float* y, int rows, int L, int C, int ldy, int N, int accumulate,
                 da_stream_t stream);
int da_x3_split(const float* x, int ld, void* out, size_t npos, int C, da_stream_t stream);
int da_x3_merge(const void* x, float* out, int ld, size_t npos, int C, da_stream_t stream);
int da_conv_bf16_multi(const da_conv_job* jobs, int n, da_stream_t stream);
typedef struct {
  const float* dy; const float* x; float* workspace;
  int rows, Lm, Ldy, lddy, N, Lx, ldx, C, dy_stride, dy_off, src_stride, ntaps; int src_off[3];
  int winograd;
  int xform, dy_half, Wn, ldstat; const float* mean; const float* invstd; const float* gamma; const float* beta;
} da_wgrad_job;
int da_conv_wgrad_multi(const da_wgrad_job* jobs, int n, da_stream_t stream);
int da_conv_wgrad_multi_reduce(const da_wgrad_job* jobs, int n, float* const* dws, int accumulate, int* reduced, da_stream_t stream);
int da_conv_wgrad_plan(const da_wgrad_job* jobs, int n, int chained, int* slabs);
int da_conv_wgrad_padded_n(int N, int C);
int da_conv_wgrad_splits(int rows, int Lm, int N, int C, int ntaps);
typedef struct { const float* slab; float* dw; int splits, ntaps, N, C; } da_wgrad_reduce_desc;
int da_wgrad_reduce_multi(const da_wgrad_reduce_desc* descs, int n, int accumulate, da_stream_t stream);
struct da_bn_pgrad_desc_;
struct da_bn_running_desc_;
int da_step_tail_multi(const da_wgrad_reduce_desc* descs, int n, const struct da_bn_pgrad_desc_* pg, int npg,
                       const struct da_bn_running_desc_* run, int nrun, const float* stem_partial, int stem_nblk, int stem_n,
                       float* stem_dw, int accumulate, da_stream_t stream);

int da_repack_conv_weight(const float* W, float* Wf, float* Wd, int Co, int Ci, int K, da_stream_t stream);
typedef struct { const float* W; float* Wf; float* Wd; float* Uf; float* Ud; int Co, Ci, K; int points; } da_repack_desc;
int da_repack_multi(const da_repack_desc* descs, int n, da_stream_t stream);

int da_stem_conv_fwd(const float* x, const float* w, da_act_t* y, int rows, int Lin, int C0, int ldy,
                     da_stream_t stream);
size_t da_stem_wgrad_workspace(int rows, int C0);
int da_stem_conv_wgrad(const da_act_t* dy, int lddy, const float* x, float* dw, float* workspace, int rows, int Lin,
                       int C0, int accumulate, da_stream_t stream);
int da_stem_conv_fwd_g(const float* x, const float* w, da_act_t* y, int rows, int Lin, int Cin, int K, int stride, int C0,
                       int ldy, da_stream_t stream);
size_t da_stem_wgrad_workspace_g(int rows, int C0, int Cin, int K);
int da_stem_conv_wgrad_g(const da_act_t* dy, int lddy, const float* x, float* dw, float* workspace, int rows, int Lin,
                         int Cin, int K, int stride, int C0, int accumulate, da_stream_t stream);

typedef struct da_bn_running_desc_ {
  const float* mean; const float* invstd; float* running_mean; float* running_var;
  long long* num_batches_tracked; int W, C, Wn; float eps, momentum;
} da_bn_running_desc;
typedef struct da_bn_pgrad_desc_ { const float* s1; const float* s2; float* dgamma; float* dbeta; int W, C; } da_bn_pgrad_desc;

void da_bn_chunks(int W, int Wn, int C, int* P, int* chunk);
size_t da_bn_workspace(int W, int Wn, int C);
int da_bn_stats_partial(const da_act_t* x, int ld, int W, int Wn, int C, float* part, da_stream_t stream);
int da_bn_stats_merge(const float* part, int W, int Wn, int C, float eps, float* mean, float* invstd,
                      da_stream_t stream);
int da_bn_running_multi(const da_bn_running_desc* descs, int n, da_stream_t stream);
int da_bn_apply(const da_act_t* x, int ldx, const da_act_t* res, int ldr, da_act_t* out, int ldo, int W, int Wn, int C,
                float* mean, float* invstd, const float* gamma, const float* beta, int relu, const float* part,
                float eps, da_stream_t stream);
int da_bn_fwd(const da_act_t* x, int ldx, const da_act_t* res, int ldr, da_act_t* out, int ldo, int W, int Wn, int C,
              float* mean, float* invstd, const float* gamma, const float* beta, int relu, float eps, float* scratch,
              da_stream_t stream);
int da_bn_debug_two_stage(int on);
int da_bn_debug_target_blocks(int blocks);
int da_bn_bwd(const da_act_t* dout, int ldd, const da_act_t* x, int ldx, const da_act_t* out, int ldo, da_act_t* dx, int lddx,
              da_act_t* gout, int ldg, int W, int Wn, int C, const float* mean, const float* invstd,
              const float* gamma, const float* beta, int mask_mode, float* scratch, float* ds, float* dgamma,
              float* dbeta, int accumulate, da_stream_t stream);
size_t da_bn_mask_words(int W, int Wn, int C);
int da_bn_fwd_mask(const da_act_t* x, int ldx, const da_act_t* res, int ldr, da_act_t* out, int ldo, int W, int Wn, int C,
                   float* mean, float* invstd, const float* gamma, const float* beta, float eps, float* scratch,
                   unsigned long long* mask, da_stream_t stream);
int da_bn_bwd_mask(const da_act_t* dout, int ldd, const da_act_t* x, int ldx, da_act_t* dx, int lddx, da_act_t* gout, int ldg, int W,
                   int Wn, int C, const float* mean, const float* invstd, const float* gamma, const float* beta,
                   float* scratch, float* ds, float* dgamma, float* dbeta, int accumulate,
                   const unsigned long long* mask, da_stream_t stream);
int da_bn_pool_ok(int W, int Wn, int C, int L);
int da_bn_fwd_pool(const da_act_t* x, int ldx, const da_act_t* res, int ldr, float* flat, int W, int Wn, int C, int L, float* mean,
                   float* invstd, const float* gamma, const float* beta, float eps, unsigned long long* mask, da_stream_t stream);
int da_bn_bwd_pool(const float* dflat, int ldd, const da_act_t* x, int ldx, da_act_t* dx, int lddx, da_act_t* gout, int ldg, int W,
                   int Wn, int C, int L, const float* mean, const float* invstd, const float* gamma, const float* beta, float* ds,
                   const unsigned long long* mask, da_stream_t stream);
int da_bn_two_ok(int W, int Wn, int C);
int da_bn_bwd_mask2(const da_act_t* dout, int ldd, const da_act_t* dout2, int ldd2, const da_act_t* x, int ldx, da_act_t* dx, int lddx,
                    da_act_t* gout, int ldg, int W, int Wn, int C, const float* mean, const float* invstd, const float* gamma,
                    const float* beta, float* ds, const unsigned long long* mask, da_stream_t stream);
int da_bn_bwd_add(const da_act_t* dout, int ldd, const da_act_t* x, int ldx, const da_act_t* out, int ldo, da_act_t* dx, int lddx,
                  da_act_t* gout, int ldg, int W, int Wn, int C, const float* mean, const float* invstd, const float* gamma,
                  const float* beta, int mask_mode, float* scratch, float* ds, float* dgamma, float* dbeta,
                  int accumulate, const da_act_t* add, int ldadd, da_stream_t stream);
int da_bn_stats_fused(const float* x, int ldx, int W, int Wn, int C, float* mean, float* invstd, int ldstat, float eps,
                      da_stream_t stream);
int da_bn_relu_ss(const float* x, int ldx, float* out, int ldo, int W, int Wn, int C, const float* mean, const float* invstd,
                  int ldstat, const float* gamma, const float* beta, da_stream_t stream);
int da_bn_bwd_ss(const da_act_t* dout, int ldd, const da_act_t* x, int ldx, const da_act_t* out, int ldo, da_act_t* dx, int lddx,
                 const da_act_t* add, int ldadd, int W, int Wn, int C, const float* mean, const float* invstd, int ldstat,
                 const float* gamma, const float* beta, int relu, int half_dout, const long long* drop_seed, unsigned drop_salt,
                 float drop_p, int drop_g, float* ds, da_act_t* hout, int ldh, da_stream_t stream);
int da_conv1x1_bn(const float* x, int ldx, const float* w, float* y, int ldy, int rows, int R, int Lin, int C, int N, int pool,
                  float* mean, float* invstd, int ldstat, const float* gamma, const float* beta, const float* pend, int pend_c0,
                  long pend_units, int pend_Wu, float eps, float* out_part, da_stream_t stream);
// ... 231 lines not shown
```

Baseline: 455,900 breath-sequences/s.

## Ride stem backward phases on the winograd-4 wgrad multi-kernel launch

```diff
diff --git a/deepards_amd/_lib.py b/deepards_amd/_lib.py
--- a/deepards_amd/_lib.py
+++ b/deepards_amd/_lib.py
@@ -56,6 +56,11 @@
 class RepackDesc(ctypes.Structure):
     _fields_ = [('W', _P), ('Wf', _P), ('Wd', _P), ('Uf', _P), ('Ud', _P), ('Co', _I), ('Ci', _I), ('K', _I),
                 ('points', _I)]
+
+
+class StemRide(ctypes.Structure):
+    _fields_ = [('dout', _P), ('ldd', _I), ('xrows', _P), ('wt', _P), ('rows', _I), ('R', _I), ('Lin', _I), ('C', _I),
+                ('mean', _P), ('invstd', _P), ('gamma', _P), ('beta', _P), ('pool_mode', _I), ('ds', _P), ('workspace', _P)]
 
 
 SIGNATURES = {
@@ -133,10 +138,12 @@
     'da_wino_weights': (_I, [_P, _P, _I, _I, _I, _P]),
     'da_wino4_weights': (_I, [_P, _P, _I, _I, _I, _P]),
     'da_conv_wgrad_multi': (_I, [ctypes.POINTER(WgradJob), _I, _P]),
-    'da_conv_wgrad_multi_reduce': (_I, [ctypes.POINTER(WgradJob), _I, ctypes.POINTER(ctypes.c_void_p), _I, _IP, _P]),
+    'da_conv_wgrad_multi_reduce': (_I, [ctypes.POINTER(WgradJob), _I, ctypes.POINTER(ctypes.c_void_p), _I, _IP, _P,
+                                        ctypes.POINTER(StemRide)]),
     'da_conv_wgrad_plan': (_I, [ctypes.POINTER(WgradJob), _I, _I, _IP]),
     'da_wgrad_reduce_multi': (_I, [ctypes.POINTER(WgradReduceDesc), _I, _I, _P]),
     'da_step_tail_multi': (_I, [ctypes.POINTER(WgradReduceDesc), _I, ctypes.POINTER(BnPgradDesc), _I, ctypes.POINTER(BnRunningDesc), _I, _P, _I, _I, _P, _I, _P]),
+    'da_conv_wgrad_stem_rides': (_I, [ctypes.POINTER(WgradJob), _I, ctypes.POINTER(StemRide)]),
     'da_stem_bwd_partials': (_I, [_I, _I, _I, ctypes.POINTER(ctypes.c_size_t), ctypes.POINTER(_I)]),
     'da_stem_wgrad_reduce': (_I, [_P, _I, _I, _P, _I, _P]),
     'da_repack_multi': (_I, [ctypes.POINTER(RepackDesc), _I, _P]),
@@ -239,7 +246,7 @@
 
 def build(force=False, verbose=False):
     srcs = [os.path.join(CSRC, s) for s in SOURCES]
-    deps = srcs + [os.path.join(CSRC, h) for h in ('common.h', 'se_tail.h')]
+    deps = srcs + [os.path.join(CSRC, h) for h in ('common.h', 'se_tail.h', 'stem_bwd.h')]
     if not force and os.path.exists(LIB_PATH) and all(os.path.getmtime(LIB_PATH) >= os.path.getmtime(d) for d in deps):
         return LIB_PATH
     hipcc = os.environ.get('HIPCC', '/opt/rocm/bin/hipcc')
diff --git a/deepards_amd/csrc/common.h b/deepards_amd/csrc/common.h
--- a/deepards_amd/csrc/common.h
+++ b/deepards_amd/csrc/common.h
@@ -383,6 +383,7 @@
   int pre_job[WGRAD_PRE_MAX], next_job[WGRAD_PRE_MAX];
   float* const* dws;
   int* reduced;
+  const struct StemRide* stem;
 };
 static inline void wgrad_chain_init(WgradChain* c, float* const* dws, int accumulate, int* reduced) {
   c->pre.n = c->pre.nblocks = c->pre.own = 0;
@@ -391,6 +392,7 @@
   c->next = c->pre;
   c->dws = dws;
   c->reduced = reduced;
+  c->stem = nullptr;
 }
 static inline void wgrad_chain_offer(WgradChain* c, int job, const da_wgrad_job& j, int splits) {
   if (!c || !c->dws || !c->dws[job] || c->next.n >= WGRAD_PRE_MAX) return;
@@ -427,6 +429,7 @@
 void wino4_wgrad_plan(int rows, int L, int* splits, int* qchunk);
 extern int g_wino4_skip5;
 int wino4_wgrad_launch(const da_wgrad_job* jobs, const WgradPlan* plan, int n, hipStream_t stream, WgradChain* chain);
+int wino4_wgrad_ride_lds_bytes();
 
 bool bf16_wgrad_eligible(const da_wgrad_job& j);
 void bf16_wgrad_plan(int rows, int L, int* splits, int* pchunk);
diff --git a/deepards_amd/csrc/conv_gemm.hip b/deepards_amd/csrc/conv_gemm.hip
--- a/deepards_amd/csrc/conv_gemm.hip
+++ b/deepards_amd/csrc/conv_gemm.hip
@@ -1,4 +1,5 @@
 #include "common.h"
+#include "stem_bwd.h"
 #include <algorithm>
 #include <utility>
 #include <vector>
@@ -1268,8 +1269,16 @@
   return (size_t)p.splits * ntaps * N * C * sizeof(float);
 }
 
+static int wgrad_launch_all(const da_wgrad_job* jobs, const WgradPlan* plan, int n, hipStream_t stream, WgradChain* chain);
+
+static bool stem_rides(const da_wgrad_job* jobs, int n, const StemRide& ride) {
+  bool w6 = false;
+  for (int i = 0; i < n; ++i) w6 = w6 || jobs[i].winograd == 6;
+  return ride.nblk && w6 && ride.shm_bytes <= wino4_wgrad_ride_lds_bytes();
+}
+
 static int conv_wgrad_multi_impl(const da_wgrad_job* jobs, int n, int chained, float* const* dws, int accumulate, int* reduced,
-                                 hipStream_t stream) {
+                                 const da_stem_ride* stem, hipStream_t stream) {
   DA_ENTER();
   std::vector<WgradPlan> plan_(n > 0 ? n : 0);
   WgradPlan* const plan = plan_.data();
@@ -1284,6 +1293,27 @@
     wgrad_chain_init(&chain_, dws, accumulate, reduced);
     chain = &chain_;
   }
+  StemRide ride;
+  if (stem) {
+    if ((rc = stem_ride_fill(stem, &ride))) return rc;
+    if (chain && stem_rides(jobs, n, ride)) {
+      chain->stem = &ride;
+    } else {
+      if ((rc = stem_bwd_launch_phase(ride, 0, stream))) return rc;
+      if ((rc = stem_bwd_launch_phase(ride, 1, stream))) return rc;
+      stem = nullptr;
+    }
+  }
+  if ((rc = wgrad_launch_all(jobs, plan, n, stream, chain))) return rc;
+  if (stem) {
+    if (chain->stem) return DA_EINVAL;
+    return stem_bwd_launch_phase(ride, 1, stream);
+  }
+  return DA_OK;
+}
+
+static int wgrad_launch_all(const da_wgrad_job* jobs, const WgradPlan* plan, int n, hipStream_t stream, WgradChain* chain) {
+  int rc;
   if ((rc = wino4_wgrad_launch(jobs, plan, n, stream, chain))) return rc;
   if ((rc = wino_wgrad_launch(jobs, plan, n, stream, chain))) return rc;
   if ((rc = bf16_wgrad_launch(jobs, plan, n, 49, stream))) return rc;
@@ -1304,13 +1334,21 @@
 }
 
 int da_conv_wgrad_multi(const da_wgrad_job* jobs, int n, hipStream_t stream) {
-  return conv_wgrad_multi_impl(jobs, n, 0, nullptr, 0, nullptr, stream);
+  return conv_wgrad_multi_impl(jobs, n, 0, nullptr, 0, nullptr, nullptr, stream);
 }
 
 int da_conv_wgrad_multi_reduce(const da_wgrad_job* jobs, int n, float* const* dws, int accumulate, int* reduced,
-                               hipStream_t stream) {
+                               hipStream_t stream, const da_stem_ride* stem) {
   if (n && (!dws || !reduced)) return DA_EINVAL;
-  return conv_wgrad_multi_impl(jobs, n, 1, dws, accumulate, reduced, stream);
+  return conv_wgrad_multi_impl(jobs, n, 1, dws, accumulate, reduced, stem, stream);
+}
+
+int da_conv_wgrad_stem_rides(const da_wgrad_job* jobs, int n, const da_stem_ride* stem) {
+  if (!stem || (n > 0 && !jobs)) return DA_EINVAL;
+  StemRide ride;
+  const int rc = stem_ride_fill(stem, &ride);
+  if (rc) return rc;
+  return stem_rides(jobs, n, ride) ? 1 : 0;
 }
 
 int da_conv_wgrad_plan(const da_wgrad_job* jobs, int n, int chained, int* slabs) {
diff --git a/deepards_amd/csrc/conv_wino.hip b/deepards_amd/csrc/conv_wino.hip
--- a/deepards_amd/csrc/conv_wino.hip
+++ b/deepards_amd/csrc/conv_wino.hip
@@ -1,4 +1,5 @@
 #include "common.h"
+#include "stem_bwd.h"
 #include <type_traits>
 
 struct WinoArgs {
@@ -1011,7 +1012,7 @@
   int n;
   int skip5;
 };
-static_assert(sizeof(WinoWgradTable) + sizeof(WgradPreTable) <= 4096, "kernel arguments: 4 KB");
+static_assert(sizeof(WinoWgradTable) + sizeof(WgradPreTable) + sizeof(StemRide) <= 4096, "kernel arguments: 4 KB");
 
 __global__ __launch_bounds__(256, WW_MIN_WAVES) void wino_wgrad_multi_kernel(WinoWgradTable t, WgradPreTable pre) {
   __shared__ float lds[WW_LDS_FLOATS];
@@ -1241,8 +1242,12 @@
   }
 }
 
-__global__ __launch_bounds__(256, WW4_MIN_WAVES) void wino4_wgrad_multi_kernel(WinoWgradTable t, WgradPreTable pre) {
-  __shared__ float lds[WW4_LDS_FLOATS];
+template <bool RIDE>
+__global__ __launch_bounds__(256, WW4_MIN_WAVES) void wino4_wgrad_multi_kernel(WinoWgradTable t, WgradPreTable pre, StemRide ride) {
+  __shared__ __attribute__((aligned(16))) float lds[WW4_LDS_FLOATS];
+  if constexpr (RIDE) {
+    if (stem_ride_dispatch(ride, lds)) return;
+  }
   const int b = wgrad_pre_dispatch(pre);
   if (b < 0 || b >= t.first_block[t.n]) return;
   int i = 0;
@@ -1251,6 +1256,8 @@
   if (skip5) wino4_wgrad_body<true>(t.d[i], b - t.first_block[i], t.first_block[i + 1] - t.first_block[i], lds);
   else wino4_wgrad_body<false>(t.d[i], b - t.first_block[i], t.first_block[i + 1] - t.first_block[i], lds);
 }
+
+int wino4_wgrad_ride_lds_bytes() { return (int)sizeof(float) * WW4_LDS_FLOATS; }
 
 #ifndef WW4_QCHUNK
 #define WW4_QCHUNK 320
@@ -1275,7 +1282,14 @@
     t.first_block[cnt] = blocks;
     WgradPreTable pre = wgrad_chain_take(chain);
     t.skip5 = g_wino4_skip5 != 0;
-    hipLaunchKernelGGL(wino4_wgrad_multi_kernel, dim3(wgrad_pre_grid(pre, blocks)), dim3(256), 0, s, t, pre);
+    StemRide ride = {};
+    if (chain && chain->stem) {
+      ride = *chain->stem;
+      chain->stem = nullptr;
+    }
+    const int grid = stem_ride_grid(ride, wgrad_pre_grid(pre, blocks));
+    if (ride.nblk) hipLaunchKernelGGL(wino4_wgrad_multi_kernel<true>, dim3(grid), dim3(256), 0, s, t, pre, ride);
+    else hipLaunchKernelGGL(wino4_wgrad_multi_kernel<false>, dim3(grid), dim3(256), 0, s, t, pre, ride);
     DA_CHECK_LAUNCH();
     cnt = 0;
     blocks = 0;
diff --git a/deepards_amd/csrc/stem_bwd.h b/deepards_amd/csrc/stem_bwd.h
--- /dev/null
+++ b/deepards_amd/csrc/stem_bwd.h
@@ -0,0 +1,235 @@
+#pragma once
+#include "common.h"
+
+#define STEM_XPAD 8
+
+__device__ __forceinline__ f32x4 stem_y4(const StemW4& sw, const float (&xw)[16], int o) {
+  f32x4 y;
+#pragma unroll
+  for (int e = 0; e < 4; ++e) {
+    float acc = 0.f;
+#pragma unroll
+    for (int k = 0; k < 7; ++k) acc = fmaf(sw.w[e][k], xw[o + k], acc);
+    y[e] = acc;
+  }
+  return y;
+}
+__device__ __forceinline__ void stem_xw_fill(float (&xw)[16], const float* xs, int j) {
+#pragma unroll
+  for (int i = 0; i < 16; i += 4) {
+    const f32x4 v = *reinterpret_cast<const f32x4*>(xs + 4 * j + i);
+    xw[i] = v[0]; xw[i + 1] = v[1]; xw[i + 2] = v[2]; xw[i + 3] = v[3];
+  }
+}
+__device__ __forceinline__ void stem_xw_next(float (&xw)[16], const float* xs, int j) {
+#pragma unroll
+  for (int i = 0; i < 12; ++i) xw[i] = xw[i + 4];
+  const f32x4 v = *reinterpret_cast<const f32x4*>(xs + 4 * j + 12);
+  xw[12] = v[0]; xw[13] = v[1]; xw[14] = v[2]; xw[15] = v[3];
+}
+__host__ __device__ __forceinline__ int stem_xs_floats(int Lin) { return (STEM_XPAD + Lin + 16 + 3) & ~3; }
+
+struct StemBn4 {
+  f32x4 mu, is, ga, be;
+  __device__ __forceinline__ f32x4 z(const f32x4& y) const {
+    f32x4 r;
+#pragma unroll
+    for (int e = 0; e < 4; ++e) r[e] = fmaxf((y[e] - mu[e]) * is[e] * ga[e] + be[e], 0.f);
+    return r;
+  }
+};
+
+template <typename AT, bool APPLY, int SH>
+__device__ __forceinline__ void stem_bwd_block(const AT* __restrict__ dout, int ldd, const float* __restrict__ xrows,
+                                               const float* __restrict__ wt, int rows, int R, int Lin, int Lc, int Lp, int C,
+                                               const float* __restrict__ mean, const float* __restrict__ invstd,
+                                               const float* __restrict__ gamma, const float* __restrict__ beta, int pool_mode,
+                                               int RPB, float* __restrict__ rowpart, float* __restrict__ ds,
+                                               float* __restrict__ partial, const int bid, float* sm) {
+  const int nq = C >> 2, slots = blockDim.x / nq, NRUN = slots < 8 ? slots : 8, RS = slots / NRUN, RJ = (Lp + NRUN - 1) / NRUN;
+  const int XS = stem_xs_floats(Lin);
+  float* tot = sm + RS * XS;
+  float* red = tot + 2 * C;
+  const int q = threadIdx.x % nq, slot = threadIdx.x / nq, rs = slot / NRUN, run = slot - rs * NRUN, c0 = q * 4;
+  float* xs = sm + rs * XS;
+  StemW4 sw;
+  sw.load(wt, c0);
+  StemBn4 bn;
+  bn.ga = *reinterpret_cast<const f32x4*>(gamma + c0);
+  bn.be = *reinterpret_cast<const f32x4*>(beta + c0);
+  float wacc[4][7];
+#pragma unroll
+  for (int e = 0; e < 4; ++e)
+#pragma unroll
+    for (int k = 0; k < 7; ++k) wacc[e][k] = 0.f;
+  const float inv_n = 1.0f / (float)(R * Lc);
+  constexpr int sh = SH;
+  const int jend = Lp + sh;
+  const int j0 = sh + run * RJ, j1 = min(jend, j0 + RJ);
+  const int row_beg = bid * RPB, w = row_beg / R;
+  if (APPLY && (int)threadIdx.x < 2 * C) {
+    const int which = threadIdx.x / C, c = threadIdx.x - which * C;
+    float t = 0.f;
+    for (int r = 0; r < R; ++r) t += rowpart[((size_t)(w * R + r) * 2 + which) * C + c];
+    tot[which * C + c] = t;
+    if (ds && row_beg == w * R) ds[((size_t)which * (rows / R) + w) * C + c] = t;
+  }
+  bn.mu = *reinterpret_cast<const f32x4*>(mean + (size_t)w * C + c0);
+  bn.is = *reinterpret_cast<const f32x4*>(invstd + (size_t)w * C + c0);
+  f32x4 t1n = {0.f, 0.f, 0.f, 0.f}, t2n = t1n;
+  for (int rb = row_beg; rb < row_beg + RPB; rb += RS) {
+    const int row = rb + rs;
+    __syncthreads();
+    for (int i = threadIdx.x; i < RS * XS; i += blockDim.x) {
+      const int r = i / XS, sx = i - r * XS - STEM_XPAD - 2 * sh;
+      sm[i] = (sx >= 0 && sx < Lin) ? xrows[(size_t)(rb + r) * Lin + sx] : 0.f;
+    }
+    __syncthreads();
+    if (APPLY && rb == row_beg) {
+#pragma unroll
+      for (int e = 0; e < 4; ++e) {
+        t1n[e] = tot[c0 + e] * inv_n;
+        t2n[e] = tot[C + c0 + e] * inv_n;
+      }
+    }
+    const AT* drow = dout + (size_t)row * Lp * ldd + c0;
+    float s1[4] = {0.f, 0.f, 0.f, 0.f}, s2[4] = {0.f, 0.f, 0.f, 0.f};
+    float xw[16];
+    auto finish = [&](const f32x4& gsum, const f32x4& y, int o) {
+      f32x4 g, xh;
+#pragma unroll
+      for (int e = 0; e < 4; ++e) {
+        xh[e] = (y[e] - bn.mu[e]) * bn.is[e];
+        g[e] = (xh[e] * bn.ga[e] + bn.be[e] > 0.f) ? gsum[e] : 0.f;
+      }
+      if (!APPLY) {
+#pragma unroll
+        for (int e = 0; e < 4; ++e) {
+          s1[e] += g[e];
+          s2[e] += g[e] * xh[e];
+        }
+      } else {
+#pragma unroll
+        for (int e = 0; e < 4; ++e) {
+          const float d = bn.ga[e] * bn.is[e] * (g[e] - t1n[e] - xh[e] * t2n[e]);
+#pragma unroll
+          for (int k = 0; k < 7; ++k) wacc[e][k] = fmaf(d, xw[o + k], wacc[e][k]);
+        }
+      }
+    };
+    auto choose = [&](const f32x4& zm, const f32x4& z0, const f32x4& zp, bool vm, bool vp, const f32x4& d, f32x4& gm, f32x4& g0,
+                      f32x4& gp) {
+      if (pool_mode == 1) {
+#pragma unroll
+        for (int e = 0; e < 4; ++e) {
+          const float t = d[e] * (1.0f / 3.0f);
+          gm[e] = vm ? t : 0.f; g0[e] = t; gp[e] = vp ? t : 0.f;
+        }
+        return;
+      }
+#pragma unroll
+      for (int e = 0; e < 4; ++e) {
+        float best = -INFINITY;
+        int arg = -1;
+        if (vm && zm[e] > best) { best = zm[e]; arg = 0; }
+        if (z0[e] > best) { best = z0[e]; arg = 1; }
+        if (vp && zp[e] > best) { best = zp[e]; arg = 2; }
+        gm[e] = arg == 0 ? d[e] : 0.f;
+        g0[e] = arg == 1 ? d[e] : 0.f;
+        gp[e] = arg == 2 ? d[e] : 0.f;
+      }
+    };
+    if (j0 < j1) {
+      const int js = j0 > sh ? j0 - 1 : j0;
+      stem_xw_fill(xw, xs, js);
+      f32x4 carry = {0.f, 0.f, 0.f, 0.f}, ym = carry, zm = carry;
+      if (js > 0) {
+        ym = stem_y4(sw, xw, 3);
+        zm = bn.z(ym);
+      }
+      for (int j = js; j < j1; ++j) {
+        if (j > js) stem_xw_next(xw, xs, j);
+        const bool vm = j > 0, vp = 2 * j + 1 < Lc + sh;
+        const f32x4 y0 = stem_y4(sw, xw, 5), yp = stem_y4(sw, xw, 7);
+        const f32x4 z0 = bn.z(y0), zp = bn.z(yp);
+        const f32x4 d = Act<AT>::ld4(drow + (size_t)(j - sh) * ldd);
+        f32x4 gm, g0, gp;
+        choose(zm, z0, zp, vm, vp, d, gm, g0, gp);
+        if (j >= j0) {
+          if (vm) {
+#pragma unroll
+            for (int e = 0; e < 4; ++e) gm[e] += carry[e];
+            finish(gm, ym, 3);
+          }
+          finish(g0, y0, 5);
+          if (j == jend - 1 && vp) finish(gp, yp, 7);
+        }
+        carry = gp; ym = yp; zm = zp;
+      }
+    }
+    if (!APPLY) {
+      __syncthreads();
+#pragma unroll
+      for (int e = 0; e < 4; ++e) {
+        red[(slot * 2 + 0) * C + c0 + e] = s1[e];
+        red[(slot * 2 + 1) * C + c0 + e] = s2[e];
+      }
+      __syncthreads();
+      for (int i = threadIdx.x; i < RS * 2 * C; i += blockDim.x) {
+        const int r = i / (2 * C), t_ = i - r * 2 * C;
+        float t = 0.f;
+        for (int u = 0; u < NRUN; ++u) t += red[(r * NRUN + u) * 2 * C + t_];
+        rowpart[(size_t)(rb + r) * 2 * C + t_] = t;
+      }
+    }
+  }
+  if (APPLY) {
+    __syncthreads();
+#pragma unroll
+    for (int e = 0; e < 4; ++e)
+#pragma unroll
+      for (int k = 0; k < 7; ++k) red[(slot * C + c0 + e) * 7 + k] = wacc[e][k];
+    __syncthreads();
+    for (int i = threadIdx.x; i < C * 7; i += blockDim.x) {
+      float t = 0.f;
+      for (int r = 0; r < slots; ++r) t += red[r * C * 7 + i];
+      partial[(size_t)bid * C * 7 + i] = t;
+    }
+  }
+}
+
+struct StemRide {
+  const float* dout; const float* xrows; const float* wt;
+  const float* mean; const float* invstd; const float* gamma; const float* beta;
+  float* rowpart; float* ds; float* partial;
+  int ldd, rows, R, Lin, Lc, Lp, C, pool_mode, RPB;
+  int nblk;
+  int base;
+  int shm_bytes;
+};
+
+__device__ __forceinline__ bool stem_ride_dispatch(const StemRide& s, float* lds) {
+  const int sb = (int)blockIdx.x - s.base;
+  if (sb < 0) return false;
+  if (sb >= s.nblk) return true;
+  if (s.pool_mode == 2)
+    stem_bwd_block<float, false, 1>(s.dout, s.ldd, s.xrows, s.wt, s.rows, s.R, s.Lin, s.Lc, s.Lp, s.C, s.mean, s.invstd, s.gamma,
+                                    s.beta, s.pool_mode, s.RPB, s.rowpart, nullptr, nullptr, sb, lds);
+  else
+    stem_bwd_block<float, false, 0>(s.dout, s.ldd, s.xrows, s.wt, s.rows, s.R, s.Lin, s.Lc, s.Lp, s.C, s.mean, s.invstd, s.gamma,
+                                    s.beta, s.pool_mode, s.RPB, s.rowpart, nullptr, nullptr, sb, lds);
+  return true;
+}
+static inline int stem_ride_grid(StemRide& s, int grid) {
+  if (s.nblk == 0) return grid;
+  s.base = (grid + 7) & ~7;
+  return s.base + s.nblk;
+}
+
+typedef struct {
+  const float* dout; int ldd; const float* xrows; const float* wt; int rows, R, Lin, C;
+  const float* mean; const float* invstd; const float* gamma; const float* beta; int pool_mode;
+  float* ds; float* workspace;
+} da_stem_ride;
+extern "C" int stem_ride_fill(const da_stem_ride* a, StemRide* s);
+extern "C" int stem_bwd_launch_phase(const StemRide& s, int phase, hipStream_t stream);
diff --git a/deepards_amd/csrc/stem_pool.hip b/deepards_amd/csrc/stem_pool.hip
--- a/deepards_amd/csrc/stem_pool.hip
+++ b/deepards_amd/csrc/stem_pool.hip
@@ -1,4 +1,5 @@
 #include "common.h"
+#include "stem_bwd.h"
 
 template <typename AT, int CIN, int K, int S>
 __global__ __launch_bounds__(256) void stem_conv_fwd_kernel(const float* __restrict__ x, const float* __restrict__ w,
@@ -119,43 +120,6 @@
   else Act<AT>::st4(out + po * ldo + c0, o);
 }
 
-#define STEM_XPAD 8
-
-__device__ __forceinline__ f32x4 stem_y4(const StemW4& sw, const float (&xw)[16], int o) {
-  f32x4 y;
-#pragma unroll
-  for (int e = 0; e < 4; ++e) {
-    float acc = 0.f;
-#pragma unroll
-    for (int k = 0; k < 7; ++k) acc = fmaf(sw.w[e][k], xw[o + k], acc);
-    y[e] = acc;
-  }
-  return y;
-}
-__device__ __forceinline__ void stem_xw_fill(float (&xw)[16], const float* xs, int j) {
-#pragma unroll
-  for (int i = 0; i < 16; i += 4) {
-    const f32x4 v = *reinterpret_cast<const f32x4*>(xs + 4 * j + i);
-    xw[i] = v[0]; xw[i + 1] = v[1]; xw[i + 2] = v[2]; xw[i + 3] = v[3];
-  }
-}
-__device__ __forceinline__ void stem_xw_next(float (&xw)[16], const float* xs, int j) {
-#pragma unroll
-  for (int i = 0; i < 12; ++i) xw[i] = xw[i + 4];
-  const f32x4 v = *reinterpret_cast<const f32x4*>(xs + 4 * j + 12);
-  xw[12] = v[0]; xw[13] = v[1]; xw[14] = v[2]; xw[15] = v[3];
-}
-__host__ __device__ __forceinline__ int stem_xs_floats(int Lin) { return (STEM_XPAD + Lin + 16 + 3) & ~3; }
-
-struct StemBn4 {
-  f32x4 mu, is, ga, be;
-  __device__ __forceinline__ f32x4 z(const f32x4& y) const {
-    f32x4 r;
-#pragma unroll
-    for (int e = 0; e < 4; ++e) r[e] = fmaxf((y[e] - mu[e]) * is[e] * ga[e] + be[e], 0.f);
-    return r;
-  }
-};
 
 template <typename AT, int OX3, int SH>
 __global__ __launch_bounds__(256) void stem_bn_relu_pool_fwd_kernel(const float* __restrict__ xrows, const float* __restrict__ wt,
@@ -285,156 +249,8 @@
                                                        int pool_mode, int RPB, float* __restrict__ rowpart,
                                                        float* __restrict__ ds, float* __restrict__ partial) {
   extern __shared__ __attribute__((aligned(16))) float sm[];
-  const int nq = C >> 2, slots = blockDim.x / nq, NRUN = slots < 8 ? slots : 8, RS = slots / NRUN, RJ = (Lp + NRUN - 1) / NRUN;
-  const int XS = stem_xs_floats(Lin);
-  float* tot = sm + RS * XS;
-  float* red = tot + 2 * C;
-  const int q = threadIdx.x % nq, slot = threadIdx.x / nq, rs = slot / NRUN, run = slot - rs * NRUN, c0 = q * 4;
-  float* xs = sm + rs * XS;
-  StemW4 sw;
-  sw.load(wt, c0);
-  StemBn4 bn;
-  bn.ga = *reinterpret_cast<const f32x4*>(gamma + c0);
-  bn.be = *reinterpret_cast<const f32x4*>(beta + c0);
-  float wacc[4][7];
-#pragma unroll
-  for (int e = 0; e < 4; ++e)
-#pragma unroll
-    for (int k = 0; k < 7; ++k) wacc[e][k] = 0.f;
-  const float inv_n = 1.0f / (float)(R * Lc);
-  constexpr int sh = SH;
-  const int jend = Lp + sh;
-  const int j0 = sh + run * RJ, j1 = min(jend, j0 + RJ);
-  const int row_beg = blockIdx.x * RPB, w = row_beg / R;
-  if (APPLY && (int)threadIdx.x < 2 * C) {
-    const int which = threadIdx.x / C, c = threadIdx.x - which * C;
-    float t = 0.f;
-    for (int r = 0; r < R; ++r) t += rowpart[((size_t)(w * R + r) * 2 + which) * C + c];
-    tot[which * C + c] = t;
-    if (ds && row_beg == w * R) ds[((size_t)which * (rows / R) + w) * C + c] = t;
-  }
-  bn.mu = *reinterpret_cast<const f32x4*>(mean + (size_t)w * C + c0);
-  bn.is = *reinterpret_cast<const f32x4*>(invstd + (size_t)w * C + c0);
-  f32x4 t1n = {0.f, 0.f, 0.f, 0.f}, t2n = t1n;
-  for (int rb = row_beg; rb < row_beg + RPB; rb += RS) {
-    const int row = rb + rs;
-    __syncthreads();
-    for (int i = threadIdx.x; i < RS * XS; i += blockDim.x) {
-      const int r = i / XS, sx = i - r * XS - STEM_XPAD - 2 * sh;
-      sm[i] = (sx >= 0 && sx < Lin) ? xrows[(size_t)(rb + r) * Lin + sx] : 0.f;
-    }
-    __syncthreads();
-    if (APPLY && rb == row_beg) {
-#pragma unroll
-      for (int e = 0; e < 4; ++e) {
-        t1n[e] = tot[c0 + e] * inv_n;
-        t2n[e] = tot[C + c0 + e] * inv_n;
-      }
-    }
-    const AT* drow = dout + (size_t)row * Lp * ldd + c0;
-    float s1[4] = {0.f, 0.f, 0.f, 0.f}, s2[4] = {0.f, 0.f, 0.f, 0.f};
-    float xw[16];
-    auto finish = [&](const f32x4& gsum, const f32x4& y, int o) {
-      f32x4 g, xh;
-#pragma unroll
-      for (int e = 0; e < 4; ++e) {
-        xh[e] = (y[e] - bn.mu[e]) * bn.is[e];
-        g[e] = (xh[e] * bn.ga[e] + bn.be[e] > 0.f) ? gsum[e] : 0.f;
-      }
-      if (!APPLY) {
-#pragma unroll
-        for (int e = 0; e < 4; ++e) {
-          s1[e] += g[e];
-          s2[e] += g[e] * xh[e];
-        }
-      } else {
-#pragma unroll
-        for (int e = 0; e < 4; ++e) {
-          const float d = bn.ga[e] * bn.is[e] * (g[e] - t1n[e] - xh[e] * t2n[e]);
-#pragma unroll
-          for (int k = 0; k < 7; ++k) wacc[e][k] = fmaf(d, xw[o + k], wacc[e][k]);
-        }
-      }
-    };
-    auto choose = [&](const f32x4& zm, const f32x4& z0, const f32x4& zp, bool vm, bool vp, const f32x4& d, f32x4& gm, f32x4& g0,
-                      f32x4& gp) {
-      if (pool_mode == 1) {
-#pragma unroll
-        for (int e = 0; e < 4; ++e) {
-          const float t = d[e] * (1.0f / 3.0f);
-          gm[e] = vm ? t : 0.f; g0[e] = t; gp[e] = vp ? t : 0.f;
-        }
-        return;
-      }
-#pragma unroll
-      for (int e = 0; e < 4; ++e) {
-        float best = -INFINITY;
-        int arg = -1;
-        if (vm && zm[e] > best) { best = zm[e]; arg = 0; }
-        if (z0[e] > best) { best = z0[e]; arg = 1; }
-        if (vp && zp[e] > best) { best = zp[e]; arg = 2; }
-        gm[e] = arg == 0 ? d[e] : 0.f;
-        g0[e] = arg == 1 ? d[e] : 0.f;
-        gp[e] = arg == 2 ? d[e] : 0.f;
-      }
-    };
-    if (j0 < j1) {
-      const int js = j0 > sh ? j0 - 1 : j0;
-      stem_xw_fill(xw, xs, js);
-      f32x4 carry = {0.f, 0.f, 0.f, 0.f}, ym = carry, zm = carry;
-      if (js > 0) {
-        ym = stem_y4(sw, xw, 3);
-        zm = bn.z(ym);
-      }
-      for (int j = js; j < j1; ++j) {
-        if (j > js) stem_xw_next(xw, xs, j);
-        const bool vm = j > 0, vp = 2 * j + 1 < Lc + sh;
-        const f32x4 y0 = stem_y4(sw, xw, 5), yp = stem_y4(sw, xw, 7);
-        const f32x4 z0 = bn.z(y0), zp = bn.z(yp);
-        const f32x4 d = Act<AT>::ld4(drow + (size_t)(j - sh) * ldd);
-        f32x4 gm, g0, gp;
-        choose(zm, z0, zp, vm, vp, d, gm, g0, gp);
-        if (j >= j0) {
-          if (vm) {
-#pragma unroll
-            for (int e = 0; e < 4; ++e) gm[e] += carry[e];
-            finish(gm, ym, 3);
-          }
-          finish(g0, y0, 5);
-          if (j == jend - 1 && vp) finish(gp, yp, 7);
-        }
-        carry = gp; ym = yp; zm = zp;
-      }
-    }
-    if (!APPLY) {
-      __syncthreads();
-#pragma unroll
-      for (int e = 0; e < 4; ++e) {
-        red[(slot * 2 + 0) * C + c0 + e] = s1[e];
-        red[(slot * 2 + 1) * C + c0 + e] = s2[e];
-      }
-      __syncthreads();
-      for (int i = threadIdx.x; i < RS * 2 * C; i += blockDim.x) {
-        const int r = i / (2 * C), t_ = i - r * 2 * C;
-        float t = 0.f;
-        for (int u = 0; u < NRUN; ++u) t += red[(r * NRUN + u) * 2 * C + t_];
-        rowpart[(size_t)(rb + r) * 2 * C + t_] = t;
-      }
-    }
-  }
-  if (APPLY) {
-    __syncthreads();
-#pragma unroll
-    for (int e = 0; e < 4; ++e)
-#pragma unroll
-      for (int k = 0; k < 7; ++k) red[(slot * C + c0 + e) * 7 + k] = wacc[e][k];
-    __syncthreads();
-    for (int i = threadIdx.x; i < C * 7; i += blockDim.x) {
-      float t = 0.f;
-      for (int r = 0; r < slots; ++r) t += red[r * C * 7 + i];
-      partial[(size_t)blockIdx.x * C * 7 + i] = t;
-    }
-  }
+  stem_bwd_block<AT, APPLY, SH>(dout, ldd, xrows, wt, rows, R, Lin, Lc, Lp, C, mean, invstd, gamma, beta, pool_mode, RPB, rowpart,
+                                ds, partial, (int)blockIdx.x, sm);
 }
 
 template <typename IT, typename OT>
@@ -717,6 +533,52 @@
   return DA_OK;
 }
 
+int stem_ride_fill(const da_stem_ride* a, StemRide* s) {
+  const int C = a->C, R = a->R, rows = a->rows, Lin = a->Lin;
+  if (g_act_bf16) return DA_EINVAL;
+  if (!a->dout || !a->xrows || !a->wt || !a->mean || !a->invstd || !a->gamma || !a->beta || !a->ds || !a->workspace || C % 4 ||
+      C < 4 || 256 % (C / 4) || 2 * C > 256 || a->ldd % 4 || R < 1 || rows < 0 || rows % R || Lin < 2 || (Lin & 1) ||
+      a->pool_mode < 0 || a->pool_mode > 2)
+    return DA_EINVAL;
+  const int nruns = 256 / (C / 4), NRUN = nruns < 8 ? nruns : 8, RS = nruns / NRUN;
+  if (R % RS) return DA_EINVAL;
+  int RPB = RS;
+  for (int d = RS; d <= 5; d += RS)
+    if (R % d == 0) RPB = d;
+  s->dout = a->dout; s->xrows = a->xrows; s->wt = a->wt;
+  s->mean = a->mean; s->invstd = a->invstd; s->gamma = a->gamma; s->beta = a->beta;
+  s->rowpart = a->workspace; s->ds = a->ds; s->partial = a->workspace + (size_t)rows * 2 * C;
+  s->ldd = a->ldd; s->rows = rows; s->R = R; s->Lin = Lin; s->Lc = Lin / 2; s->Lp = pool_out_len(s->Lc, a->pool_mode); s->C = C;
+  s->pool_mode = a->pool_mode; s->RPB = RPB;
+  s->nblk = rows / RPB;
+  s->base = 0;
+  const size_t shm1 = ((size_t)RS * stem_xs_floats(Lin) + 2 * C + (size_t)nruns * 2 * C) * sizeof(float);
+  const size_t shm2 = ((size_t)RS * stem_xs_floats(Lin) + 2 * C + (size_t)nruns * 7 * C) * sizeof(float);
+  if (shm2 > 64 * 1024) return DA_EINVAL;
+  s->shm_bytes = (int)shm1;
+  return DA_OK;
+}
+
+int stem_bwd_launch_phase(const StemRide& s, int phase, hipStream_t stream) {
+  if (s.nblk == 0) return DA_OK;
+  const int nruns = 256 / (s.C / 4), NRUN = nruns < 8 ? nruns : 8, RS = nruns / NRUN;
+  const size_t shm = ((size_t)RS * stem_xs_floats(s.Lin) + 2 * s.C + (size_t)nruns * (phase ? 7 : 2) * s.C) * sizeof(float);
+#define DA_STEM_BWD(APPLY_, SH_, DS_, PART_)                                                                                    \
+  hipLaunchKernelGGL((stem_bwd_kernel<float, APPLY_, SH_>), dim3(s.nblk), dim3(256), shm, stream, s.dout, s.ldd, s.xrows, s.wt, \
+                     s.rows, s.R, s.Lin, s.Lc, s.Lp, s.C, s.mean, s.invstd, s.gamma, s.beta, s.pool_mode, s.RPB, s.rowpart, DS_, \
+                     PART_)
+  if (!phase) {
+    if (s.pool_mode == 2) DA_STEM_BWD(false, 1, (float*)nullptr, (float*)nullptr);
+    else DA_STEM_BWD(false, 0, (float*)nullptr, (float*)nullptr);
+  } else {
+    if (s.pool_mode == 2) DA_STEM_BWD(true, 1, s.ds, s.partial);
+    else DA_STEM_BWD(true, 0, s.ds, s.partial);
+  }
+#undef DA_STEM_BWD
+  DA_CHECK_LAUNCH();
+  return DA_OK;
+}
+
 int da_pool_bwd(const void* dout, int ldd, const void* y, int ldy, void* dz, int lddz, int rows, int R, int Lin,
                 int C, const float* mean, const float* invstd, const float* gamma, const float* beta, int pool_mode,
                 hipStream_t stream) {
diff --git a/deepards_amd/functional.py b/deepards_amd/functional.py
--- a/deepards_amd/functional.py
+++ b/deepards_amd/functional.py
@@ -22,12 +22,12 @@
 
 
 _STEP = {'on': False, 'pack': {}, 'running': [], 'running_early': [], 'groups': 1, 'pgrad': [], 'wgrad': [], 'wslab': [],
-         'stemred': None}
+         'stemred': None, 'stemride': None}
 
 
 @contextlib.contextmanager
 def training_step(model=None):
-    _STEP.update(on=True, pack={}, running=[], running_early=[], pgrad=[], wgrad=[], wslab=[], stemred=None, dout2={})
+    _STEP.update(on=True, pack={}, running=[], running_early=[], pgrad=[], wgrad=[], wslab=[], stemred=None, stemride=None, dout2={})
     try:
         if model is not None:
             precise = {id(c) for b in model.modules() if getattr(b, 'precise_convs', False) for c in b.children()}
@@ -41,7 +41,7 @@
                 _STEP['pack'][(w.data_ptr(), int(c))] = e
         yield
     finally:
-        _STEP.update(on=False, pack={}, running=[], running_early=[], pgrad=[], wgrad=[], wslab=[], stemred=None, dout2={})
+        _STEP.update(on=False, pack={}, running=[], running_early=[], pgrad=[], wgrad=[], wslab=[], stemred=None, stemride=None, dout2={})
 
 
 def flush_forward(defer=False):
@@ -82,13 +82,17 @@
 
 def _launch_wgrads():
     jobs = _STEP['wgrad']
+    stem, _STEP['stemride'] = _STEP.get('stemride'), None
+    if stem is not None and not (jobs and _WGRAD_CHAIN):
+        H.conv_wgrad_multi([], dws=[], accumulate=_acc(), stem=stem)
+        stem = None
     if not jobs:
         return
     specs = [j[:5] + (j[6], j[7]) for j in jobs]
     if _WGRAD_CHAIN:
         if len({j[5].data_ptr() for j in jobs}) != len(jobs):
             _plain_writer()
-        slabs, reduced = H.conv_wgrad_multi(specs, dws=[j[5] for j in jobs], accumulate=_acc())
+        slabs, reduced = H.conv_wgrad_multi(specs, dws=[j[5] for j in jobs], accumulate=_acc(), stem=stem)
     else:
         slabs, reduced = H.conv_wgrad_multi(specs), [False] * len(jobs)
     _STEP['wslab'] += [(sl, j[5]) for sl, j, r in zip(slabs, jobs, reduced) if not r]
@@ -96,6 +100,7 @@
 
 
 _WGRAD_CHAIN = True
+_STEM_RIDE = True
 
 
 _STEM_FUSED = os.environ.get('DA_STEM_FUSED', '1') != '0'
@@ -310,7 +315,12 @@
             dout = dout[:, :, :ctx.c0]
         if ctx.fused:
             if _STEM_TAIL and tw is not None and _STEP['on'] and _STEP.get('stemred') is None:
-                (part, nblk, n), ds = H.stem_fused_bwd(dout, x2d, y0, ctx.R, mean, invstd, gamma, beta, ctx.pool_mode, defer=True)
+                if _STEM_RIDE and _WGRAD_CHAIN and H.act_dtype() == 'f32' and _STEP.get('stemride') is None:
+                    (part, nblk, n), ds, _STEP['stemride'] = H.stem_fused_bwd(dout, x2d, y0, ctx.R, mean, invstd, gamma, beta,
+                                                                              ctx.pool_mode, defer=True, ride=True)
+                else:
+                    (part, nblk, n), ds = H.stem_fused_bwd(dout, x2d, y0, ctx.R, mean, invstd, gamma, beta, ctx.pool_mode,
+                                                           defer=True)
                 _STEP['stemred'] = (part, nblk, n, tw)
                 dw = None
             else:
diff --git a/deepards_amd/hip_ops.py b/deepards_amd/hip_ops.py
--- a/deepards_amd/hip_ops.py
+++ b/deepards_amd/hip_ops.py
@@ -565,8 +565,11 @@
     return _x3_flow() and c % 64 == 0 and bn_x3_ok(rows, l, c, R)
 
 
-def conv_wgrad_multi(jobs, dws=None, accumulate=True):
+def conv_wgrad_multi(jobs, dws=None, accumulate=True, stem=None):
     if not jobs:
+        if stem is not None:
+            _chk(_lib.lib().da_conv_wgrad_multi_reduce(None, 0, None, 1 if accumulate else 0, None, _stream(),
+                                                       ctypes.byref(stem[0])), 'da_conv_wgrad_multi_reduce')
         return [] if dws is None else ([], [])
     L = _lib.lib()
     arr = (_lib.WgradJob * len(jobs))()
@@ -636,8 +639,11 @@
                     raise ValueError('conv_wgrad_multi: bad dw shape')
                 ptrs[i] = _f32(dw, 'dw').data_ptr()
         red = (ctypes.c_int * len(jobs))()
-        _chk(L.da_conv_wgrad_multi_reduce(arr, len(jobs), ptrs, 1 if accumulate else 0, red, _stream()), 'da_conv_wgrad_multi_reduce')
+        _chk(L.da_conv_wgrad_multi_reduce(arr, len(jobs), ptrs, 1 if accumulate else 0, red, _stream(),
+                                          ctypes.byref(stem[0]) if stem is not None else None), 'da_conv_wgrad_multi_reduce')
         return outs, [bool(r) for r in red]
+    if stem is not None:
+        raise ValueError('conv_wgrad_multi: the stem backward rides on the chained call (dws)')
     _chk(L.da_conv_wgrad_multi(arr, len(jobs), _stream()), 'da_conv_wgrad_multi')
     return outs
 
@@ -1180,7 +1186,7 @@
     return out, mean, invstd
 
 
-def stem_fused_bwd(dout, x2d, w, R, mean, invstd, gamma, beta, pool_mode, dw=None, accumulate=False, defer=False):
+def stem_fused_bwd(dout, x2d, w, R, mean, invstd, gamma, beta, pool_mode, dw=None, accumulate=False, defer=False, ride=False):
     ldd = _pv(dout, 'dout') if ACT == torch.float32 else _rlc(dout, 'dout').shape[2]
     x = x2d.reshape(x2d.shape[0], x2d.shape[-1])
     rows, lin = x.shape
@@ -1194,6 +1200,14 @@
     L = _lib.lib()
     ds = torch.empty((2, rows // R, c), device=x.device, dtype=torch.float32)
     ws = torch.empty((L.da_stem_bwd_workspace(rows, c) // 4,), device=x.device, dtype=torch.float32)
+    if ride:
+        if not defer or ACT != torch.float32:
+            raise ValueError('stem_fused_bwd: ride needs defer and float storage')
+        off, nblk = ctypes.c_size_t(), ctypes.c_int()
+        _chk(L.da_stem_bwd_partials(rows, R, c, ctypes.byref(off), ctypes.byref(nblk)), 'da_stem_bwd_partials')
+        d = _lib.StemRide(dout.data_ptr(), ldd, x.data_ptr(), _f32(w, 'w').data_ptr(), rows, R, lin, c, mean.data_ptr(),
+                          invstd.data_ptr(), gamma.data_ptr(), beta.data_ptr(), pool_mode, ds.data_ptr(), ws.data_ptr())
+        return (ws[off.value:], nblk.value, c * 7), ds, (d, (dout, x, w, mean, invstd, gamma, beta, ds, ws))
     _chk(L.da_stem_bwd(_p(dout), ldd, _p(x), _p(w), rows, R, lin, c, _p(mean), _p(invstd), _p(gamma), _p(beta), pool_mode, _p(ds),
                        None if defer else _p(dw), 1 if accumulate else 0, _p(ws), _stream()), 'da_stem_bwd')
     if defer:
diff --git a/include/deepards_hip.h b/include/deepards_hip.h
--- a/include/deepards_hip.h
+++ b/include/deepards_hip.h
@@ -69,7 +69,14 @@
   int xform, dy_half, Wn, ldstat; const float* mean; const float* invstd; const float* gamma; const float* beta;
 } da_wgrad_job;
 int da_conv_wgrad_multi(const da_wgrad_job* jobs, int n, da_stream_t stream);
-int da_conv_wgrad_multi_reduce(const da_wgrad_job* jobs, int n, float* const* dws, int accumulate, int* reduced, da_stream_t stream);
+typedef struct {
+  const float* dout; int ldd; const float* xrows; const float* wt; int rows, R, Lin, C;
+  const float* mean; const float* invstd; const float* gamma; const float* beta; int pool_mode;
+  float* ds; float* workspace;
+} da_stem_ride;
+int da_conv_wgrad_multi_reduce(const da_wgrad_job* jobs, int n, float* const* dws, int accumulate, int* reduced, da_stream_t stream,
+                               const da_stem_ride* stem);
+int da_conv_wgrad_stem_rides(const da_wgrad_job* jobs, int n, const da_stem_ride* stem);
 int da_conv_wgrad_plan(const da_wgrad_job* jobs, int n, int chained, int* slabs);
 int da_conv_wgrad_padded_n(int N, int C);
 int da_conv_wgrad_splits(int rows, int Lm, int N, int C, int ntaps);
```

Result: no change. 458,500 breath-sequences/s (median of 6 runs) (+0.6%).
